# erthward/geonomics

Measured on AMD Instinct MI355X. Metric: individual-timesteps/sec, higher is better.
Workload: dtype u64

## Files before the change

### geonomics_amd/_native.py

```python
import ctypes as C
import os

import numpy as np

_HERE = os.path.dirname(os.path.abspath(__file__))
LIB_PATH = os.environ.get('GNX_LIB') or os.path.join(_HERE, 'libgnxhip.so')

DIST = {'lognormal': 0, 'wald': 1, 'levy': 2}
MATE_UNIFORM, MATE_NEAREST, MATE_INVERSE = 0, 1, 2
SURF_NONE, SURF_MIXTURE, SURF_UNIMODAL = 0, 1, 2
(F_X, F_Y, F_AGE, F_SEX, F_ID, F_E, F_Z, F_FIT, F_GROW, F_GENO) = range(10)
(R_N, R_NPAIRS, R_K, R_D, R_COUNTS) = range(5)
KERNELS = ['move', 'sort', 'permute', 'find_mates', 'pairs', 'offspring',
           'crossover', 'phenotype', 'density', 'death', 'compact', 'crossover_tail']

EXPORTS = [
    'gnx_create', 'gnx_destroy', 'gnx_last_error', 'gnx_words_per_hom', 'gnx_blocks_per_hom',
    'gnx_set_stream', 'gnx_synchronize', 'gnx_upload_rasters',
    'gnx_upload_layer', 'gnx_set_species_params', 'gnx_upload_population',
    'gnx_init_population', 'gnx_set_recomb_paths', 'gnx_set_trait',
    'gnx_set_dominance', 'gnx_set_deleterious', 'gnx_upload_genomes',
    'gnx_assign_genomes', 'gnx_set_z', 'gnx_age', 'gnx_move',
    'gnx_pop_dynamics', 'gnx_pop_dynamics_mate', 'gnx_pop_dynamics_die',
    'gnx_set_z_range', 'gnx_step', 'gnx_counts', 'gnx_step_index',
# ... 253 lines not shown
    def assign_genomes(self, n_per_site):
        n = _arr(n_per_site, np.int32)
        assert n.size == self.L
        self._chk(self.lib.gnx_assign_genomes(self.h, _ptr(n, C.c_int32)))

    def set_z(self):
        self._chk(self.lib.gnx_set_z(self.h))

    def age(self):
        self._chk(self.lib.gnx_age(self.h))

    def move(self):
        self._chk(self.lib.gnx_move(self.h))

    def pop_dynamics(self, burn, with_selection):
        self._chk(self.lib.gnx_pop_dynamics(self.h, int(bool(burn)),
                                            int(bool(with_selection))))

    def pop_dynamics_mate(self, burn):
        self._chk(self.lib.gnx_pop_dynamics_mate(self.h, int(bool(burn))))

    def pop_dynamics_die(self, burn, with_selection):
        self._chk(self.lib.gnx_pop_dynamics_die(self.h, int(bool(burn)),
                                                int(bool(with_selection))))

    def set_z_range(self, first, n):
        self._chk(self.lib.gnx_set_z_range(self.h, C.c_int64(first), C.c_int64(n)))

    def step(self, burn, with_selection):
        self._chk(self.lib.gnx_step(self.h, int(bool(burn)),
                                    int(bool(with_selection))))

    def walk(self, T, burn, with_selection):
        self._chk(self.lib.gnx_walk(self.h, C.c_int64(int(T)), int(bool(burn)),
                                    int(bool(with_selection))))

    def walk_history(self, max_steps=1 << 16):
        n = np.zeros(max_steps, np.int64)
        b = np.zeros(max_steps, np.int64)
        d = np.zeros(max_steps, np.int64)
        k = self.lib.gnx_walk_history(self.h, C.c_int64(max_steps), _ptr(n, C.c_int64),
                                      _ptr(b, C.c_int64), _ptr(d, C.c_int64))
        return n[:k], b[:k], d[:k]

    def comm_init_rccl(self, unique_id, rank, world):
        buf = (C.c_uint8 * 128).from_buffer_copy(bytes(unique_id))
        self._chk(self.lib.gnx_comm_init_rccl(self.h, buf, int(rank), int(world)))

    def comm_init_single(self):
        self._chk(self.lib.gnx_comm_init_single(self.h))

    def comm_local_join(self, group, rank):
        self._chk(self.lib.gnx_comm_local_join(self.h, group, int(rank)))

    def set_id_order(self, mode):
        self._chk(self.lib.gnx_set_id_order(self.h, int(mode)))
        self._id_order = int(mode)

    @property
    def id_order(self):
        return getattr(self, '_id_order', 0)

    def comm_selftest(self):
        self._chk(self.lib.gnx_comm_selftest(self.h))

    def comm_free(self):
        self._chk(self.lib.gnx_comm_free(self.h))

    @property
    def comm_bytes_sent(self):
        return int(self.lib.gnx_comm_bytes_sent(self.h))

    def comm_info(self):
        out = np.zeros(16, np.int64)
        self._chk(self.lib.gnx_comm_info(self.h, _ptr(out, C.c_int64)))
        steps = max(int(out[7]), 1)
        names = ('route_and_count_exchange', 'migrant_ghost_exchange_import',
                 'sort_pairs_second_count_exchange', 'births_gamete_service',
                 'allreduce_deaths')
        return {'transport': ('single', 'rccl', 'local')[int(out[0])], 'rank': int(out[1]),
                'world': int(out[2]), 'nccl_comm_count': int(out[3]),
                'nccl_comm_user_rank': int(out[4]), 'nccl_comm_device': int(out[5]),
                'hip_device': int(out[6]), 'tile_steps': int(out[7]),
                'phase_ms_per_step': {n: float(out[8 + k]) / 1e3 / steps
                                      for k, n in enumerate(names)},
                'bytes_sent': int(out[13]), 'gc_runs': int(out[14])}

    def tile_step_abort(self):
        self._chk(self.lib.gnx_tile_step_abort(self.h))

    def tile_step(self, burn, with_selection, exact=True):
        out = np.zeros(3, np.int64)
        self._chk(self.lib.gnx_tile_step(self.h, int(bool(burn)), int(bool(with_selection)),
                                         int(bool(exact)), _ptr(out, C.c_int64)))
        self._id_order = 1
        return int(out[0]), int(out[1]), int(out[2])

    def tile_walk(self, T, burn, with_selection, exact=True):
        out = np.zeros(5, np.int64)
        self._chk(self.lib.gnx_tile_walk(self.h, C.c_int64(int(T)), int(bool(burn)),
                                         int(bool(with_selection)), int(bool(exact)),
                                         _ptr(out, C.c_int64)))
        self._id_order = 1
        return (int(out[0]), int(out[1]), int(out[2])), int(out[3]), int(out[4])

    def tile_step_begin(self, burn):
        self._chk(self.lib.gnx_tile_step_begin(self.h, int(bool(burn))))
        self._id_order = 1
        a, b = C.c_int64(), C.c_int64()
        self._chk(self.lib.gnx_tile_step_births(self.h, C.byref(a), C.byref(b)))
        return int(a.value), int(b.value)

    def tile_step_end(self, burn, with_selection, exact=True):
        out = np.zeros(3, np.int64)
        self._chk(self.lib.gnx_tile_step_end(self.h, int(bool(burn)), int(bool(with_selection)),
                                             int(bool(exact)), _ptr(out, C.c_int64)))
        return int(out[0]), int(out[1]), int(out[2])

    def tile2_vt_counts(self):
        cnt = np.zeros(64, np.int64)
        self._chk(self.lib.gnx_tile2_vt_counts(self.h, _ptr(cnt, C.c_int64)))
        return cnt

    def tile2_vt_bases(self, bases):
        b = _arr(bases, np.int64)
        assert b.size == 64
        self._chk(self.lib.gnx_tile2_vt_bases(self.h, _ptr(b, C.c_int64)))

    def step_begin(self, burn):
        self._chk(self.lib.gnx_step_begin(self.h, int(bool(burn))))

    def step_mid(self, burn, with_selection):
        self._chk(self.lib.gnx_step_mid(self.h, int(bool(burn)), int(bool(with_selection))))

    def step_end(self, burn):
        self._chk(self.lib.gnx_step_end(self.h, int(bool(burn))))

    def counts(self):
        n, b, d = C.c_int64(), C.c_int64(), C.c_int64()
        self._chk(self.lib.gnx_counts(self.h, C.byref(n), C.byref(b), C.byref(d)))
        return n.value, b.value, d.value

    def totals(self):
        out = np.zeros(6, np.int64)
        self._chk(self.lib.gnx_totals(self.h, _ptr(out, C.c_int64)))
        return dict(zip(('steps', 'ind_steps', 'births', 'deaths', 'xo_births', 'dd_steps'),
                        (int(v) for v in out)))

    def reset_totals(self):
        self._chk(self.lib.gnx_reset_totals(self.h))

    PATH_COUNTS = ('lazy_mortalities', 'xo_launch_p2', 'xo_flush', 'jobs_lanes_256',
                   'jobs_lanes_512', 'sort_hist_gather', 'gc_with_pending_xo', 'make_dense',
                   'moves_ahead')

    def path_counts(self):
        out = np.zeros(len(self.PATH_COUNTS), np.int64)
        n = self.lib.gnx_path_counts(self.h, _ptr(out, C.c_int64), len(out))
        assert n == len(out), 'gnx_path_counts: the library has %d counters' % n
        return dict(zip(self.PATH_COUNTS, (int(v) for v in out)))

    def reset_path_counts(self):
        self._chk(self.lib.gnx_reset_path_counts(self.h))

    @property
    def N(self):
        return self.counts()[0]

    @property
    def step_index(self):
        return self.lib.gnx_step_index(self.h)

    @step_index.setter
    def step_index(self, v):
        self._chk(self.lib.gnx_set_step_index(self.h, C.c_int64(int(v))))

    def synchronize(self):
        self._chk(self.lib.gnx_synchronize(self.h))

    def set_defer_crossover(self, on):
        self._chk(self.lib.gnx_set_defer_crossover(self.h, int(bool(on))))

    def set_crossover_overlap(self, mode):
        self._chk(self.lib.gnx_set_crossover_overlap(self.h, int(mode)))

    def debug_halves(self):
        out = np.zeros(6, np.int64)
        self._chk(self.lib.gnx_debug_halves(self.h, _ptr(out, C.c_int64)))
        return out

    def genome_info(self):
        out = np.zeros(8, np.int64)
        self._chk(self.lib.gnx_genome_info(self.h, _ptr(out, C.c_int64)))
        return dict(zip(('NB', 'BW', 'gc_runs', 'row_spread', 'sparse', 'free_blocks_est',
                         'free_rows', 'deferred'), (int(v) for v in out)))

    def set_crossover_split(self, wide_per_1024):
        self._chk(self.lib.gnx_set_crossover_split(self.h, int(wide_per_1024)))

    def last_crossover_jobs(self):
        n = C.c_int64()
        self._chk(self.lib.gnx_last_crossover_jobs(self.h, None, 0, C.byref(n)))
        out = np.zeros((n.value, 4), np.int32)
        if n.value:
            self._chk(self.lib.gnx_last_crossover_jobs(self.h, _ptr(out, C.c_int32), n.value,
                                                       C.byref(n)))
        return out

    @property
    def last_crossover_births(self):
        return self.lib.gnx_last_crossover_births(self.h)

    def set_stream(self, stream_ptr):
        self._chk(self.lib.gnx_set_stream(self.h, C.c_void_p(stream_ptr)))

    def mutate(self, slots, loci, homs):
        slots = _arr(slots, np.int64)
        loci = _arr(loci, np.int32)
        homs = _arr(homs, np.uint8)
        self._chk(self.lib.gnx_mutate(self.h, int(slots.size),
                                      _ptr(slots, C.c_int64),
                                      _ptr(loci, C.c_int32),
                                      _ptr(homs, C.c_uint8)))

    _FIELD_DT = {F_X: np.float32, F_Y: np.float32, F_AGE: np.int32,
                 F_SEX: np.uint8, F_ID: np.int64, F_FIT: np.float32,
                 F_GROW: np.int32}

    def download(self, field):
        n = int(self.lib.gnx_n_slots(self.h))
        if field == F_E:
            out = np.empty((self.n_layers, n), dtype=np.float32)
        elif field == F_Z:
            out = np.empty((self.n_traits, n), dtype=np.float32)
        elif field == F_GENO:
            out = np.empty((n, 2, self.W64), dtype=np.uint64)
        else:
            out = np.empty(n, dtype=self._FIELD_DT[field])
        if out.size:
            self._chk(self.lib.gnx_download(self.h, field,
                                            out.ctypes.data_as(C.c_void_p),
                                            C.c_int64(out.nbytes)))
        return out

    def download_genomes(self, slots):
        slots = _arr(slots, np.int64)
        out = np.empty((slots.size, 2, self.W64), dtype=np.uint64)
        if slots.size:
            self._chk(self.lib.gnx_download_genomes(
                self.h, C.c_int64(slots.size), _ptr(slots, C.c_int64),
                _ptr(out, C.c_uint64)))
        return out

    def download_raster(self, which):
        out = np.empty((self.H, self.W), dtype=np.float64)
        self._chk(self.lib.gnx_download_raster(self.h, which, _ptr(out, C.c_double)))
        return out

    def spatial_diff_stats(self):
        m, s = C.c_double(), C.c_double()
        self._chk(self.lib.gnx_spatial_diff_stats(self.h, C.byref(m), C.byref(s)))
        return m.value, s.value

    def spatial_diff_sums(self):
        a, b = C.c_double(), C.c_double()
        self._chk(self.lib.gnx_spatial_diff_sums(self.h, C.byref(a), C.byref(b)))
        return a.value, b.value

    def op_move(self, theta, dist):
        t = _arr(theta, np.float32)
        d = _arr(dist, np.float32)
        assert t.size == self.N and d.size == self.N
        self._chk(self.lib.gnx_op_move(self.h, _ptr(t, C.c_float), _ptr(d, C.c_float)))

    def op_move_draws(self):
        n = self.N
        t = np.empty(n, np.float32)
        d = np.empty(n, np.float32)
        self._chk(self.lib.gnx_op_move_draws(self.h, _ptr(t, C.c_float),
                                             _ptr(d, C.c_float)))
        return t, d

    def op_find_pairs(self, keep=None):
        n = self.N
        k = None if keep is None else _arr(keep, np.uint8)
        mate = np.empty(n, np.int32)
        pairs = np.empty((max(n, 1), 2), np.int32)
        npairs = C.c_int64()
        self._chk(self.lib.gnx_op_find_pairs(self.h, _ptr(k, C.c_uint8),
                                             _ptr(mate, C.c_int32),
                                             _ptr(pairs, C.c_int32),
                                             C.byref(npairs)))
        return mate, pairs[:npairs.value].copy()

    def op_crossover(self, parent_slots, keys, start_homs):
        p = _arr(parent_slots, np.int32)
        k = _arr(keys, np.int32)
        s = _arr(start_homs, np.uint8)
        B = p.shape[0]
        assert p.shape == (B, 2) and k.shape == (B, 2) and s.shape == (B, 2)
        self._chk(self.lib.gnx_op_crossover(self.h, C.c_int64(B),
                                            _ptr(p, C.c_int32),
                                            _ptr(k, C.c_int32),
                                            _ptr(s, C.c_uint8)))

    def op_dispersal(self, mid_x, mid_y, theta, dist):
        mx = _arr(mid_x, np.float32)
# ... 963 lines not shown
```

### geonomics_amd/csrc/gnx_api.hip

```cpp
#include <cmath>
#include <cstdarg>
#include <algorithm>
#include <atomic>
#include <chrono>
#include "gnx_internal.h"
#include "gnx_rng.h"
#include "gnx_compact.h"

static thread_local char g_err[1024] = "";

void gnx_set_error(const char* fmt, ...) {
  va_list ap;
  va_start(ap, fmt);
  vsnprintf(g_err, sizeof(g_err), fmt, ap);
  va_end(ap);
}

extern "C" const char* gnx_last_error(void) { return g_err; }

extern "C" int gnx_words_per_hom(int32_t L) {
  int w = (L + 63) / 64;
  return ((w + 15) / 16) * 16;
}

// ... 255 lines not shown
      while (want > 1 && (lines % want || (!asked && lines / want < 2) ||
                          (double)h->cfg.cap_rows * 4 * 2.0 * want >= 2.0e9))
        --want;
      h->NB = want;
      h->BW = h->W64 / want;
      int bl = gnx_env_int("GNX_BLOCK_LINES", -1);
      if (bl < 0) bl = (!asked && lines >= 40) ? std::max(5, (lines + GNX_MAX_NB - 1) / GNX_MAX_NB) : 0;
      if (bl > 0 && (double)h->cfg.cap_rows * 4 * 2.0 * ((lines + bl - 1) / bl) >= 2.0e9) bl = 0;
      if (bl > 0 && (lines + bl - 1) / bl <= GNX_MAX_NB && (lines + bl - 1) / bl >= 1) {
        h->NB = (lines + bl - 1) / bl;
        h->BW = 16 * bl;
      }
      h->NB_alloc = h->NB;
      h->BW_alloc = h->BW;
    }
    {
      const size_t need = (size_t)h->cfg.cap_rows * 2 * std::max(h->W64, h->NB * h->BW) * 8;
      size_t free_b = 0, total_b = 0;
      (void)hipMemGetInfo(&free_b, &total_b);
      int want = gnx_env_int("GNX_ROW_SPREAD", 4);
      want = std::max(1, std::min(want, 8));
      while (want > 1 && ((double)need * want > 0.75 * (double)free_b ||
                          (double)h->cfg.cap_rows * want > 1.0e9))
        --want;
      for (; want >= 1; --want) {
        h->G = nullptr;
        const hipError_t e = hipMalloc((void**)&h->G, need * (size_t)want);
        if (e == hipSuccess) break;
        (void)hipGetLastError();
        if (want == 1) {
          gnx_set_error("hipMalloc of the genome table (%zu bytes) failed: %s", need,
                        hipGetErrorString(e));
          return 1;
        }
      }
      h->row_spread = want;
    }
    GNXCHK(dalloc(&h->free_rows, (size_t)h->cfg.cap_rows));
    const size_t halves = (size_t)h->cfg.cap_rows * h->row_spread * 2 * h->NB;
    GNXCHK(dalloc(&h->hmap, halves));
    GNXCHK(dalloc(&h->half_mark, halves));
    GNXCHK(dalloc(&h->half_free, (size_t)h->cfg.cap_rows * 2 * h->NB));
    GNXCHK(dalloc(&h->half_top, 1));
    HIPCHK(hipMalloc(&h->xo_plan, (size_t)cap * 40));
    GNXCHK(dalloc(&h->gc_cnt, (size_t)h->cfg.cap_rows * 2 * h->NB / GNX_CB + 2));
    GNXCHK(dalloc(&h->gc_off, (size_t)h->cfg.cap_rows * 2 * h->NB / GNX_CB + 2));
    HIPCHK(hipMemset(h->half_mark, 0, halves));
    HIPCHK(hipMalloc((void**)&h->xo_jobs_acc, 2 * sizeof(unsigned long long)));
    HIPCHK(hipMemset(h->xo_jobs_acc, 0, 2 * sizeof(unsigned long long)));
    HIPCHK(hipMemset(h->hmap, 0xff, halves * sizeof(int32_t)));
    HIPCHK(hipMemset(h->half_top, 0, sizeof(int32_t)));
    h->alias_xo = gnx_env_int("GNX_XO_ALIAS", 1) != 0;
  }
  for (int k = 0; k < 2; ++k) {
    GNXCHK(dalloc(&h->key[k], cap));
    GNXCHK(dalloc(&h->perm[k], cap));
  }
  GNXCHK(dalloc(&h->mate, cap));
  for (int k = 0; k < 2; ++k) {
    GNXCHK(dalloc(&h->ord[k], cap));
    GNXCHK(dalloc(&h->keyk[k], cap));
    GNXCHK(dalloc(&h->valk[k], cap));
  }
  GNXCHK(dalloc(&h->newslot, cap));
  GNXCHK(dalloc(&h->fill_cnt, 4));
  HIPCHK(hipEventCreateWithFlags(&h->ev_fill, gnx_order_event_flags()));
  HIPCHK(hipEventCreateWithFlags(&h->ev_alive, gnx_order_event_flags()));
  HIPCHK(hipEventCreateWithFlags(&h->ev_moved, gnx_order_event_flags()));
  HIPCHK(hipEventCreateWithFlags(&h->ev_perm_rest, gnx_order_event_flags()));
  {
    const size_t nb = std::max(gnx_os_scratch_bytes((size_t)cap, 24),
                               gnx_os_words_used64((size_t)cap, 64) * sizeof(unsigned int)) + 16;
    HIPCHK(hipMalloc(&h->os_scratch, nb));
    HIPCHK(hipMemset(h->os_scratch, 0, nb));
  }
  GNXCHK(dalloc(&h->os_ktmp, cap));
  GNXCHK(dalloc(&h->os_vtmp, cap));
  GNXCHK(dalloc(&h->cell32, cap));
  GNXCHK(dalloc(&h->ord_cnt, cap / GNX_CB + 2));
  GNXCHK(dalloc(&h->ord_off, cap / GNX_CB + 2));
  HIPCHK(hipEventCreateWithFlags(&h->ev_ord, gnx_order_event_flags()));
  HIPCHK(hipStreamCreate(&h->stream3));
  HIPCHK(hipEventCreateWithFlags(&h->ev_compact, gnx_order_event_flags()));
  h->ord_mode = gnx_env_int("GNX_ORD_SORT", 1) != 0;
  GNXCHK(dalloc(&h->tag, cap));
  HIPCHK(hipMalloc(&h->cand, (size_t)cap * 16));
  GNXCHK(dalloc(&h->flag, cap + 1));
  GNXCHK(dalloc(&h->flag2, cap + 1));
  GNXCHK(dalloc(&h->scan, cap + 1));
  GNXCHK(dalloc(&h->pairs, cap * 2));
  GNXCHK(dalloc(&h->nbirths, cap + 1));
  GNXCHK(dalloc(&h->boff, cap + 1));
  GNXCHK(dalloc(&h->off_pair, cap));
  GNXCHK(dalloc(&h->off_parent, cap * 2));
  GNXCHK(dalloc(&h->off_keys, cap * 2));
  GNXCHK(dalloc(&h->off_start, cap * 2));
  GNXCHK(dalloc(&h->keep_in, cap));
  GNXCHK(dalloc(&h->inj_a, cap * GNX_DISP_ATTEMPTS));
  GNXCHK(dalloc(&h->inj_b, cap * GNX_DISP_ATTEMPTS));
  GNXCHK(dalloc(&h->mid_x, cap));
  GNXCHK(dalloc(&h->mid_y, cap));
  GNXCHK(dalloc(&h->p_death, cap));
  GNXCHK(dalloc(&h->d_cell, cap));
  GNXCHK(dalloc(&h->dead_in, cap));
  GNXCHK(dalloc(&h->nmax_bits, 1));
  GNXCHK(dalloc(&h->red, 8));
  GNXCHK(gnx_prim_sort_bytes((size_t)cap, 32, &h->sort_tmp_bytes));
  HIPCHK(hipMalloc(&h->sort_tmp, std::max<size_t>(h->sort_tmp_bytes, 16)));
  GNXCHK(gnx_prim_scan_bytes((size_t)cap + 1, &h->scan_tmp_bytes));
  HIPCHK(hipMalloc(&h->scan_tmp, std::max<size_t>(h->scan_tmp_bytes, 16)));
  GNXCHK(gnx_prim_sort64_bytes((size_t)cap, &h->sort64_tmp_bytes));
  HIPCHK(hipMalloc(&h->sort64_tmp, std::max<size_t>(h->sort64_tmp_bytes, 16)));
  GNXCHK(dalloc(&h->key64[0], cap));
  GNXCHK(dalloc(&h->key64[1], cap));
  GNXCHK(dalloc(&h->pairs2, cap * 2));
  GNXCHK(dalloc(&h->pair_goff, cap));
  GNXCHK(dalloc(&h->req_pid, cap));
  GNXCHK(dalloc(&h->req_k, cap));
  GNXCHK(dalloc(&h->req_key, cap));
  GNXCHK(dalloc(&h->req_start, cap));
  GNXCHK(dalloc(&h->req_px, cap));
  GNXCHK(dalloc(&h->req_py, cap));
  GNXCHK(dalloc(&h->req_count, 1));
  h->blk_stride = (int)((cap + 1023) / 1024) + 2;
  GNXCHK(dalloc(&h->blk_cnt, (size_t)3 * h->blk_stride));
  GNXCHK(dalloc(&h->blk_off, (size_t)3 * h->blk_stride));
  GNXCHK(dalloc(&h->cnt_dev, 8));
  GNXCHK(dalloc(&h->tickets, 8));
  GNXCHK(dalloc(&h->nmax2, 2));
  HIPCHK(hipMemset(h->nmax2, 0, 2 * sizeof(unsigned long long)));
  HIPCHK(hipEventCreateWithFlags(&h->ev_pairs, gnx_order_event_flags()));
  HIPCHK(hipEventCreateWithFlags(&h->ev_latP, gnx_order_event_flags()));
  HIPCHK(hipEventCreateWithFlags(&h->ev_perm, gnx_order_event_flags()));
  HIPCHK(hipEventCreateWithFlags(&h->ev_binsN, gnx_order_event_flags()));
  HIPCHK(hipMemset(h->tickets, 0, 8 * sizeof(unsigned int)));
  HIPCHK(hipHostMalloc((void**)&h->h_pin, 32 * sizeof(int64_t),
                       hipHostMallocCoherent | hipHostMallocMapped));
  memset(h->h_pin, 0, 32 * sizeof(int64_t));
  HIPCHK(hipHostGetDevicePointer((void**)&h->h_pin_dev, h->h_pin, 0));
  if (cfg->L > 0) {
    for (int k = 0; k < 2; ++k) {
      HIPCHK(hipMalloc(&h->jobs[k], (size_t)cap * 2 * h->NB * 16));
      HIPCHK(hipMalloc(&h->jobs_bp[k], (size_t)cap * 2 * h->NB * 8));
      GNXCHK(dalloc(&h->n_jobs_dev[k], 1));
      HIPCHK(hipEventCreateWithFlags(&h->ev_xo_done[k], gnx_order_event_flags()));
      HIPCHK(hipEventCreateWithFlags(&h->ev_xo_wide[k], gnx_order_event_flags()));
    }
    HIPCHK(hipEventCreateWithFlags(&h->ev_jobs, gnx_order_event_flags()));
  }
  HIPCHK(hipEventCreateWithFlags(&h->ev_counts, hipEventDisableTiming));
  h->xo_launch_late = h->xo_launch_late_default = cap > gnx_dd_max_cap();
  h->compact_fill = gnx_env_int("GNX_COMPACT_FILL", 1) != 0;
  h->permute_split = gnx_env_int("GNX_PERMUTE_SPLIT", 1) != 0;
  *out = h;
  return 0;
}

extern "C" void gnx_destroy(gnx_state* h) {
  if (!h) return;
  host_marks_report();
  if (gnx_host_times() && g_host_steps > 0)
    fprintf(stderr, "[gnx host times] %lld steps: %.1f us/step in gnx_step, %.1f us of it waiting for counts\n",
            g_host_steps, 1e6 * g_host_step_s / g_host_steps, 1e6 * g_host_wait_s / g_host_steps);
  (void)gnx_xo_launch_pending(h);
  (void)hipStreamSynchronize(h->stream);
  gnx_dd_destroy(h);
  (void)gnx_comm_free(h);
  {
    void* vt[] = {h->vt_cls, h->vt_scls, h->vt_blk_nz, h->vt_rank, h->vt_pblk, h->vt_blk_cnt, h->vt_blk_off, h->vt_count, h->vt_base};
    for (void* q : vt)
      if (q) (void)hipFree(q);
  }
  if (h->stream2) (void)hipStreamSynchronize(h->stream2);
  if (h->stream3) (void)hipStreamSynchronize(h->stream3);
  for (int k = 0; k < 2; ++k) {
    (void)hipFree(h->jobs[k]);
    (void)hipFree(h->jobs_bp[k]);
    (void)hipFree(h->n_jobs_dev[k]);
    if (h->ev_xo_done[k]) (void)hipEventDestroy(h->ev_xo_done[k]);
    if (h->ev_xo_wide[k]) (void)hipEventDestroy(h->ev_xo_wide[k]);
  }
  if (h->ev_jobs) (void)hipEventDestroy(h->ev_jobs);
  if (h->ev_counts) (void)hipEventDestroy(h->ev_counts);
  for (int k = 0; k < 2; ++k) {
    free_soa(&h->soa[k]);
    (void)hipFree(h->key[k]);
    (void)hipFree(h->perm[k]);
    (void)hipFree(h->counts_rast[k]);
  }
  void* ptrs[] = {h->os_scratch, h->os_ktmp, h->os_vtmp, h->fill_cnt, h->ord[0], h->ord[1], h->keyk[0], h->keyk[1], h->valk[0], h->valk[1], h->newslot, h->cell32, h->ord_cnt, h->ord_off, h->route_geo_dev, h->xo_plan, h->gc_cnt, h->gc_off, h->half_mark, h->hmap, h->half_free, h->half_top, h->xo_jobs_acc, h->rast, h->G, h->free_rows, h->paths, h->bp_off, h->bp_loci, h->dom,
                  h->delet_loci, h->delet_s, h->cell_start, h->tag, h->cand, h->sort64_tmp, h->key64[0], h->key64[1], h->pairs2,
                  h->pair_goff, h->st_rec, h->st_z, h->st_geno, h->st_slots, h->req_pid, h->req_k, h->req_key, h->req_start, h->req_px, h->req_py,
                  h->req_count, h->sort_tmp, h->scan_tmp, h->mate,
                  h->flag, h->flag2, h->scan, h->pairs, h->nbirths, h->boff, h->off_pair,
                  h->off_parent, h->off_keys, h->off_start, h->keep_in, h->inj_a, h->inj_b,
                  h->mid_x, h->mid_y, h->p_death, h->d_cell, h->dead_in, h->nmax_bits, h->red,
                  h->sel_loci, h->path_sel, h->lat.areas, h->lat.cprime, h->spl_N.c, h->spl_P.c, h->bin_partials, h->nodes,
                  h->K_over, h->blk_cnt, h->blk_off, h->cnt_dev, h->tickets, h->nmax2, h->fb[0], h->gp_rec, h->gp_z, h->gp_slots, h->tile_counts, h->rq_sorted, h->rq_k, h->gam_out, h->gam_slot, h->chk,
                  h->lin_tab, h->lin_bt};
  for (void* p : ptrs) (void)hipFree(p);
  for (int t = 0; t < GNX_MAX_TRAITS; ++t) {
    (void)hipFree(h->traits[t].loci);
    (void)hipFree(h->traits[t].alpha);
    (void)hipFree(h->traits[t].phi_rast);
  }
  (void)hipHostFree(h->h_pin);
  if (h->h_route_pin) (void)hipHostFree(h->h_route_pin);
  (void)hipFree(h->gh_rec);
  (void)hipFree(h->route_cnt);
  if (h->h_stage) (void)hipHostFree(h->h_stage);
  for (int k = 0; k < GNX_K_COUNT; ++k) timers_resolve(h, k);
  for (hipEvent_t e : h->ev_free) (void)hipEventDestroy(e);
  if (h->own_stream) (void)hipStreamDestroy(h->stream);
  if (h->stream2) (void)hipStreamDestroy(h->stream2);
  h->stream2 = nullptr;
  if (h->stream3) {
    (void)hipStreamSynchronize(h->stream3);
    (void)hipStreamDestroy(h->stream3);
  }
  if (h->ev_ord) (void)hipEventDestroy(h->ev_ord);
  if (h->ev_compact) (void)hipEventDestroy(h->ev_compact);
  if (h->ev_fill) (void)hipEventDestroy(h->ev_fill);
  if (h->ev_alive) (void)hipEventDestroy(h->ev_alive);
  if (h->ev_moved) (void)hipEventDestroy(h->ev_moved);
  if (h->ev_perm_rest) (void)hipEventDestroy(h->ev_perm_rest);
  if (h->ev_pairs) (void)hipEventDestroy(h->ev_pairs);
  if (h->ev_latP) (void)hipEventDestroy(h->ev_latP);
  if (h->ev_perm) (void)hipEventDestroy(h->ev_perm);
  if (h->ev_binsN) (void)hipEventDestroy(h->ev_binsN);
  delete h;
}

extern "C" int gnx_set_stream(gnx_state* h, void* hip_stream) {
  GNXCHK(gnx_xo_join(h));
  HIPCHK(hipStreamSynchronize(h->stream));
  if (h->stream2) HIPCHK(hipStreamSynchronize(h->stream2));
  if (h->own_stream) (void)hipStreamDestroy(h->stream);
  if (h->stream2) (void)hipStreamDestroy(h->stream2);
  h->stream2 = nullptr;
  h->stream = (hipStream_t)hip_stream;
  h->own_stream = false;
  return 0;
}

extern "C" int gnx_synchronize(gnx_state* h) {
  GNXCHK(gnx_xo_launch_pending(h));
  if (h->stream3) HIPCHK(hipStreamSynchronize(h->stream3));
  HIPCHK(hipStreamSynchronize(h->stream));
  if (h->stream2) HIPCHK(hipStreamSynchronize(h->stream2));
  return 0;
}

extern "C" int gnx_upload_rasters(gnx_state* h, const float* rasts) {
  size_t n = (size_t)h->cfg.n_layers * h->cfg.W * h->cfg.H;
  HIPCHK(hipMemcpyAsync(h->rast, rasts, n * sizeof(float), hipMemcpyHostToDevice, h->stream));
  HIPCHK(hipStreamSynchronize(h->stream));
  return 0;
}

extern "C" int gnx_upload_layer(gnx_state* h, int32_t layer, const float* rast) {
  if (layer < 0 || layer >= h->cfg.n_layers) {
    gnx_set_error("gnx_upload_layer: bad layer %d", layer);
    return 1;
  }
  size_t n = (size_t)h->cfg.W * h->cfg.H;
  HIPCHK(hipMemcpyAsync(h->rast + layer * n, rast, n * sizeof(float), hipMemcpyHostToDevice,
                        h->stream));
  HIPCHK(hipStreamSynchronize(h->stream));
  return 0;
}

extern "C" int gnx_set_k_raster(gnx_state* h, const double* K) {
  h->cfg_epoch += 1;
  size_t n = (size_t)h->cfg.W * h->cfg.H;
  HIPCHK(hipStreamSynchronize(h->stream));
  if (!K) {
    (void)hipFree(h->K_over);
    h->K_over = nullptr;
    return 0;
  }
  if (!h->K_over) HIPCHK(hipMalloc((void**)&h->K_over, n * sizeof(double)));
  GNXCHK(gnx_h2d(h, h->K_over, K, n * sizeof(double)));
  return 0;
}

static int lattice_nodes(int dim, double ww) {
  double hww = ww / 2.0;
  double last_edge = 0, last_inner = 0;
  int ne = (int)ceil((dim + ww) / ww);
  last_edge = (ne - 1) * ww;
  int ni = (int)ceil(((dim + hww) - hww) / ww);
  last_inner = hww + (ni - 1) * ww;
  double last = std::max(last_edge, last_inner);
  return (int)llround(last / hww) + 1;
}

static int setup_lattice(gnx_state* h) {
  const gnx_config& c = h->cfg;
  double ww = h->sp.window_width;
  if (!(ww > 0)) ww = std::nearbyint(0.1 * std::max(c.W, c.H));
  if (!(ww > 0)) ww = 1;
  GnxLattice& L = h->lat;
  (void)hipFree(L.areas);
  (void)hipFree(L.cprime);
  (void)hipFree(h->spl_N.c);
  (void)hipFree(h->spl_P.c);
  (void)hipFree(h->bin_partials);
  (void)hipFree(h->nodes);
  L.hww = ww / 2.0;
  L.Jx = lattice_nodes(c.W, ww);
  L.Jy = lattice_nodes(c.H, ww);
  L.nbx = L.Jx;
  L.nby = L.Jy;
  const int64_t nn = (int64_t)L.Jx * L.Jy;
  std::vector<double> areas(nn);
  for (int i = 0; i < L.Jy; ++i)
    for (int j = 0; j < L.Jx; ++j) {
      double cx = j * L.hww, cy = i * L.hww;
      double ax = std::min(cx + L.hww, (double)c.W) - std::max(cx - L.hww, 0.0);
      double ay = std::min(cy + L.hww, (double)c.H) - std::max(cy - L.hww, 0.0);
      double a = std::max(ax, 0.0) * std::max(ay, 0.0);
      if (a == 0) a = 0.0001;
      areas[(int64_t)i * L.Jx + j] = a;
    }
  int Jm = std::max(L.Jx, L.Jy);
  std::vector<double> cp(Jm + 1, 0.0);
  if (Jm > 1) cp[1] = 0.25;
  for (int k = 2; k < Jm; ++k) cp[k] = 1.0 / (4.0 - cp[k - 1]);
  GNXCHK(dalloc(&L.areas, nn));
  GNXCHK(dalloc(&L.cprime, Jm + 1));
  GNXCHK(dalloc(&h->spl_N.c, 4 * nn));
  GNXCHK(dalloc(&h->spl_P.c, 4 * nn));
  GNXCHK(dalloc(&h->nodes, nn));
  size_t nb = (size_t)L.nbx * L.nby;
  GNXCHK(dalloc(&h->bin_partials, 2 * nb + 4));
  h->bins_P = h->bin_partials + nb;
  (void)hipFree(h->fb[0]);
  GNXCHK(dalloc(&h->fb[0], 3 * nb));
  h->fb[1] = h->fb[0] + nb;
  h->fb[2] = h->fb[0] + 2 * nb;
  HIPCHK(hipMemset(h->fb[0], 0, 3 * nb * sizeof(int32_t)));
  h->fb_zero[0] = h->fb_zero[1] = h->fb_zero[2] = true;
  h->fb_adults = false;
  h->nmax_ready = false;
  HIPCHK(hipMemcpy(L.areas, areas.data(), nn * sizeof(double), hipMemcpyHostToDevice));
  HIPCHK(hipMemcpy(L.cprime, cp.data(), (Jm + 1) * sizeof(double), hipMemcpyHostToDevice));
  h->spl_N.valid = h->spl_P.valid = false;
// ... 1003 lines not shown
```

### geonomics_amd/csrc/gnx_internal.h

```cpp
#pragma once
#include <cstring>
#include <cstdint>
#include <cstdio>
#include <cstdlib>
#include <string>
#include <vector>
#include <utility>
#include <hip/hip_runtime.h>
#include "../../include/gnx_hip.h"
#include "gnx_half.h"

#define GNX_MAX_TRAITS 16
#define GNX_MAX_LAYERS 16
#define GNX_DISP_ATTEMPTS 8
#define GNX_SPARSE_MAX_BP 24

void gnx_set_error(const char* fmt, ...);

static inline int gnx_env_int(const char* name, int dflt) {
  const char* v = getenv(name);
  return v ? atoi(v) : dflt;
}
static inline int64_t gnx_dd_max_cap() {
  static const int64_t v = getenv("GNX_DD_MAX_CAP") ? atoll(getenv("GNX_DD_MAX_CAP")) : 600000;
// ... 61 lines not shown
  float e[4], z[4];
  uint64_t tb[4];
};
#ifdef __HIPCC__
__device__ __forceinline__ GnxRec gnx_rec_load(const GnxSoA& a, int64_t i, int64_t cap, int nl,
                                               int nt, int tbw) {
  GnxRec r;
  r.x = a.x[i];
  r.y = a.y[i];
  r.age = a.age[i];
  r.sex = a.sex[i];
  r.id = a.id[i];
  r.fit = a.fit[i];
  r.grow = a.grow[i];
  r.ghost = a.ghost[i];
#pragma unroll
  for (int l = 0; l < 4; ++l) r.e[l] = l < nl ? a.e[(int64_t)l * cap + i] : 0.0f;
#pragma unroll
  for (int t = 0; t < 4; ++t) r.z[t] = t < nt ? a.z[(int64_t)t * cap + i] : 0.0f;
#pragma unroll
  for (int w = 0; w < 4; ++w) r.tb[w] = w < tbw ? a.tb[i * tbw + w] : 0ull;
  return r;
}
__device__ __forceinline__ void gnx_rec_store(const GnxSoA& b, int64_t k, int64_t cap, int nl, int nt,
                                              int tbw, const GnxRec& r) {
  b.x[k] = r.x;
  b.y[k] = r.y;
  b.age[k] = r.age;
  b.sex[k] = r.sex;
  b.id[k] = r.id;
  b.fit[k] = r.fit;
  b.grow[k] = r.grow;
  b.ghost[k] = r.ghost;
#pragma unroll
  for (int l = 0; l < 4; ++l)
    if (l < nl) b.e[(int64_t)l * cap + k] = r.e[l];
#pragma unroll
  for (int t = 0; t < 4; ++t)
    if (t < nt) b.z[(int64_t)t * cap + k] = r.z[t];
#pragma unroll
  for (int w = 0; w < 4; ++w)
    if (w < tbw) b.tb[k * tbw + w] = r.tb[w];
}
__device__ __forceinline__ void gnx_rec_rest(const GnxSoA& a, int64_t i, const GnxSoA& b, int64_t k,
                                             int64_t cap, int nl, int nt, int tbw) {
  for (int l = 4; l < nl; ++l) b.e[(int64_t)l * cap + k] = a.e[(int64_t)l * cap + i];
  for (int t = 4; t < nt; ++t) b.z[(int64_t)t * cap + k] = a.z[(int64_t)t * cap + i];
  for (int w = 4; w < tbw; ++w) b.tb[k * tbw + w] = a.tb[i * tbw + w];
}
#endif

struct GnxLattice {
  int Jx = 0, Jy = 0;
  int nbx = 0, nby = 0;
  double hww = 0;
  double* areas = nullptr;
  double* cprime = nullptr;
};

struct GnxSpline {
  double* c = nullptr;
  bool valid = false;
};

struct GnxKernelTimer {
  double ms = 0;
  int64_t launches = 0;
  double bytes = 0;
};

struct GnxDD {
  int32_t N;
  int32_t P;
  int32_t B;
  int32_t n_free;
  int32_t ord_n;
  int32_t err;
  int32_t seq;
  int32_t pad;
  int64_t max_id;
  int64_t step;
};
#define GNX_DD_ERR_SLOTS 1
#define GNX_DD_ERR_ROWS 2
#define GNX_DD_ERR_BLOCKS 4
struct GnxDDRec {
  int64_t seq;
  int32_t N0, P, B, S;
  int32_t xo, n_free, half_top, err;
  int64_t max_id, step;
  int64_t pad[2];
};
#define GNX_DD_RING 4096
#ifdef __HIPCC__
__device__ __forceinline__ int64_t gnx_dd_n(const GnxDD* dd, int64_t n) { return dd ? (int64_t)dd->N : n; }
__device__ __forceinline__ int64_t gnx_dd_nb(const GnxDD* dd, int64_t n) {
  return dd ? (int64_t)dd->N + dd->B : n;
}
__device__ __forceinline__ long long gnx_dd_step(const GnxDD* dd, long long s) {
  return dd ? (long long)dd->step : s;
}
__device__ __forceinline__ int gnx_tile_index(float v, int tw, int n) {
  int c = (int)(v / (float)tw);
  c = max(0, min(n - 1, c));
  while (c + 1 < n && (float)((c + 1) * tw) <= v) ++c;
  while (c > 0 && (float)(c * tw) > v) --c;
  return c;
}
#endif

#define GNX_MAX_TILES 4096
#define GNX_TILE_DIM 64
struct RouteGeo {
  int R, C, tw, th, me, ncx, ncy;
  double inv_cs;
  int cx0[GNX_TILE_DIM], cx1[GNX_TILE_DIM], cy0[GNX_TILE_DIM], cy1[GNX_TILE_DIM];
};
#ifdef __HIPCC__
__device__ __forceinline__ int gnx_route_append(int32_t* __restrict__ counts, int dest) {
  unsigned long long todo = __ballot(dest >= 0);
  const int lane = threadIdx.x & 63;
  int idx = -1;
  while (todo) {
    const int leader = __ffsll((long long)todo) - 1;
    const int d = __shfl(dest, leader);
    const unsigned long long same = __ballot(dest == d);
    int base = 0;
    if (lane == leader) base = atomicAdd(&counts[d], (int)__popcll(same));
    base = __shfl(base, leader);
    if (dest == d) idx = base + (int)__popcll(same & ((1ull << lane) - 1ull));
    todo &= ~same;
  }
  return idx;
}
__device__ __forceinline__ int gnx_route_dest(const RouteGeo& g, int k, int orow, int oc, int cx, int cy) {
  if (k == 4) return (orow * g.C + oc) != g.me ? orow * g.C + oc : -1;
  const int rr = orow + k / 3 - 1, cc = oc + k % 3 - 1;
  if (rr >= 0 && rr < g.R && cc >= 0 && cc < g.C && cx >= g.cx0[cc] && cx <= g.cx1[cc] &&
      cy >= g.cy0[rr] && cy <= g.cy1[rr])
    return rr * g.C + cc;
  return -1;
}
#endif
enum {
  GNX_PC_LAZY_MORT = 0,
  GNX_PC_XO_P2,
  GNX_PC_XO_FLUSH,
  GNX_PC_JOBS_256,
  GNX_PC_JOBS_512,
  GNX_PC_SORT_GATHER,
  GNX_PC_GC_PENDING_XO,
  GNX_PC_MAKE_DENSE,
  GNX_PC_MOVE_AHEAD,
  GNX_PC_COUNT
};

struct gnx_state {
  gnx_config cfg{};
  gnx_species_params sp{};
  bool have_sp = false;
  hipStream_t stream = nullptr;
  hipStream_t stream2 = nullptr;
  bool xo_pending = false;
  bool own_stream = false;
  int W64 = 0;
  int64_t N = 0;
  int64_t max_id = -1;
  int64_t step = 0;
  int64_t last_births = 0, last_deaths = 0;
  int64_t tot[6]{};
  int64_t pc[GNX_PC_COUNT]{};
  int64_t n_ghost = 0;

  GnxSoA soa[2]{};
  int cur = 0;

  uint64_t* G = nullptr;
  int row_spread = 1;
  int32_t* free_rows = nullptr;
  int64_t n_free = 0;
  int32_t* hmap = nullptr;
  uint8_t* half_mark = nullptr;
  int32_t* half_free = nullptr;
  int32_t* half_top = nullptr;
  int64_t half_free_est = 0;
  int64_t gc_runs = 0;
  void* xo_plan = nullptr;
  int32_t* gc_cnt = nullptr;
  int32_t* gc_off = nullptr;
  int NB = 1;
  int NB_alloc = 1;
  int BW = 0, BW_alloc = 0;
  hipStream_t stream3 = nullptr;
  hipEvent_t ev_compact = nullptr;
  bool alias_xo = true;
  unsigned long long* xo_jobs_acc = nullptr;
  bool genomes_assigned = false;

  float* rast = nullptr;

  int n_paths = 0;
  uint64_t* paths = nullptr;
  int32_t* bp_off = nullptr;
  int32_t* bp_loci = nullptr;
  bool sparse_paths = false;

  int32_t* lin_tab = nullptr;
  int32_t* lin_bt = nullptr;
  int64_t lin_rows = 0;
  uint64_t lin_sum = 0;
  int64_t lin_budget = 0;
  double lin_ms = 0.0;
  int64_t lin_launches = 0, lin_uploaded = 0;

  int64_t ld_budget = 0;
  double ld_ms = 0.0;
  int64_t ld_launches = 0, ld_blocks = 0;

  double tr_ms = 0.0;
  int64_t tr_launches = 0, tr_bytes = 0;

  double sw_ms = 0.0;
  int64_t sw_launches = 0, sw_steps = 0;

  int64_t cost_budget = 0;
  double cost_ms = 0.0;
  int64_t cost_launches = 0, cost_rounds = 0, cost_batches = 0;

  double admix_ms = 0.0;
  int64_t admix_launches = 0, admix_chunks = 0;
  int32_t admix_instance = 0;

  int64_t dm_tiles = 0, dm_chunks = 0, dm_launches = 0;

  GnxTrait traits[GNX_MAX_TRAITS];
  std::vector<int32_t> h_trait_loci[GNX_MAX_TRAITS];
  std::vector<int32_t> h_delet_loci;
  int n_tl = 0;
  int n_sel = 0, TW = 0;
  int32_t* sel_loci = nullptr;
  uint64_t* path_sel = nullptr;
  uint8_t* dom = nullptr;
  int n_delet = 0;
  int32_t* delet_loci = nullptr;
  double* delet_s = nullptr;

  bool defer_xo = true;
  bool xo_deferred = false;
  int64_t xo_first = 0, xo_B = 0;
  void* jobs[2]{};
  int32_t* n_jobs_dev[2]{};
  void* jobs_bp[2]{};
  bool jobs_inline[2]{};
  int jobs_cur = 0;
  hipEvent_t ev_jobs = nullptr, ev_xo_done[2]{};
  hipEvent_t ev_counts = nullptr;
  bool xo_inflight[2]{};
  hipEvent_t ev_xo_wide[2]{};
  bool xo_wide_inflight[2]{};
  int xo_split = 0;
  int xo_last_split = 0;
  bool xo_running = false;
  bool xo_launch_late = false;
  bool xo_launch_late_default = false;
  bool xo_sort_waits = true;
  int xo_wait_at = 1;
  int xo_ready_buf = -1;
  int64_t xo_ready_jobs = 0;
  int64_t last_xo_births = 0;

  double cs = 1, inv_cs = 1;
  int ncx = 1, ncy = 1, key_bits = 1;
  int cell_ref = 1;
  uint32_t* key[2]{};
  int32_t* perm[2]{};
  int32_t* cell_start = nullptr;
  void* cand = nullptr;
  uint32_t* tag = nullptr;
  void* sort_tmp = nullptr;
  size_t sort_tmp_bytes = 0;
  void* scan_tmp = nullptr;
  size_t scan_tmp_bytes = 0;
  void* sort64_tmp = nullptr;
  size_t sort64_tmp_bytes = 0;
  uint64_t* key64[2]{};
  int32_t* pairs2 = nullptr;
  int64_t* pair_goff = nullptr;
  bool pair_goff_local = false;
  int id_order = 0;
  bool pair_goff_ready = false;
  bool pair_goff_local_base = false;
  bool vt_fused = false;
  int64_t vt_mul = 1;
  bool vt_weighted = false;
  uint8_t* vt_cls = nullptr;
  uint8_t* vt_scls = nullptr;
  unsigned long long* vt_blk_nz = nullptr;
  int32_t *vt_rank = nullptr, *vt_pblk = nullptr, *vt_blk_cnt = nullptr, *vt_blk_off = nullptr,
          *vt_count = nullptr;
  int64_t* vt_base = nullptr;
  int64_t n_births_pending = 0;
  bool step_burn = false;
  int64_t* req_pid = nullptr;
  int32_t* req_k = nullptr;
  int32_t* req_key = nullptr;
  uint8_t* req_start = nullptr;
  float* req_px = nullptr;
  float* req_py = nullptr;
  int32_t* req_count = nullptr;
  bool tiled = false;
  int tile_R = 1, tile_C = 1, tile_r = 0, tile_c = 0;
  gnx_ind_rec* st_rec = nullptr;
  float* st_z = nullptr;
  uint64_t* st_geno = nullptr;
  int64_t* st_slots = nullptr;
  int64_t st_n = 0, st_cap = 0, st_geno_cap = 0;
  bool st_has_geno = false;
  int64_t birth_first_slot = 0;
  int64_t n_req = 0;
  gnx_ind_rec* gp_rec = nullptr;
  float* gp_z = nullptr;
  int64_t* gp_slots = nullptr;
  int64_t gp_n = 0, gp_cap = 0;
  int32_t* tile_counts = nullptr;
  void* rq_sorted = nullptr;
  int32_t* rq_k = nullptr;
  int64_t rq_cap = 0;
  uint64_t* gam_out = nullptr;
  int32_t* gam_slot = nullptr;
  int64_t gam_cap = 0;
  int64_t* chk = nullptr;
  int64_t tile_evict = 0;
  float evict_box[4]{};
  int64_t n_req_known = -1;
  gnx_ind_rec* gh_rec = nullptr;
  int64_t gh_cap = 0;
  int32_t* route_cnt = nullptr;
  int64_t route_n_mig = 0, route_n_gh = 0;
  int64_t prev_deaths = 0;
  int32_t* h_route_pin = nullptr;
  int32_t* h_route_pin_dev = nullptr;
  std::vector<int64_t> req_by_rank;
  bool rq_is2 = false;
  bool tile_req_on_device = false;
  bool tile2_mode = false;
  bool req_cnt_zeroed = false;
  bool tile_pairs_nowait = false;
  bool tile_births_settled = false;

  int32_t* mate = nullptr;
  int32_t* flag = nullptr;
  int32_t* flag2 = nullptr;
  int32_t* scan = nullptr;
  int32_t* pairs = nullptr;
  int32_t* nbirths = nullptr;
  int32_t* boff = nullptr;
  int32_t* off_pair = nullptr;
  int32_t* off_parent = nullptr;
  int32_t* off_keys = nullptr;
  uint8_t* off_start = nullptr;
  uint8_t* keep_in = nullptr;
  float* inj_a = nullptr;
  float* inj_b = nullptr;
  float* mid_x = nullptr;
  float* mid_y = nullptr;
  int64_t n_pairs = 0;
  bool pairs_wait = false;
  int64_t pairs_seq = 0;
  bool pairs_with_top = false, pairs_with_density = false;
  bool mort_wait = false;
  bool mort_xo = false, mort_fill = false, mort_ord_keep = false;
  int mort_has_rows = 0;
  int64_t mort_N = 0;

  GnxLattice lat;
  GnxSpline spl_N, spl_P;
  int32_t* bin_partials = nullptr;
  int32_t* bins_P = nullptr;
  bool bins_zeroed[2]{};
  bool nmax_zeroed = false;
  bool req_zeroed = false;
  int32_t* fb[3]{};
  bool fb_zero[3]{};
  int fb_cur = 0;
  bool fb_adults = false;
  int64_t fb_count = 0;
  unsigned long long* nmax2 = nullptr;
  const unsigned long long* nmax_cur = nullptr;
  bool nmax_ready = false;
  bool last_N_fused = false;
  hipEvent_t ev_pairs = nullptr, ev_latP = nullptr, ev_perm = nullptr, ev_binsN = nullptr;
  bool binsN_inflight = false;
  bool latP_inflight = false;
  bool ord_mode = true;
  bool ord_valid = false;
  int64_t ord_n = 0;
  int ord_cur = 0;
  int32_t* ord[2]{};
  int32_t* newslot = nullptr;
  bool compact_fill = true;
  bool jobs_self_scan = false;
  bool ord_covers_xo = false;
  bool permute_split = true;
  bool perm_rest_inflight = false;
  bool perm_rest_pending = false;
  GnxSoA perm_rest_a{}, perm_rest_b{};
  int64_t perm_rest_N = 0;
  hipEvent_t ev_perm_rest = nullptr;
  bool fb_pending = false;
  const float *fbp_x = nullptr, *fbp_y = nullptr;
  int64_t fbp_N = 0;
  hipEvent_t ev_alive = nullptr;
  int32_t* fill_cnt = nullptr;
  hipEvent_t ev_fill = nullptr;
  int64_t fill_guess = 0;
  uint32_t* cell32 = nullptr;
  uint32_t* keyk[2]{};
  int32_t* valk[2]{};
  void* os_scratch = nullptr;
  uint32_t* os_ktmp = nullptr;
  int32_t* os_vtmp = nullptr;
  int32_t* ord_cnt = nullptr;
  int32_t* ord_off = nullptr;
  hipEvent_t ev_ord = nullptr;
  bool ord_inflight = false;
  bool keys_ordmode = false;
  bool keys_fresh = false;
  bool hist_fresh = false;
  bool holes = false;
  int64_t holes_N = 0;
  RouteGeo* route_geo_dev = nullptr;
  uint64_t route_geo_epoch = 0;
  bool move_counts_routes = false;
  bool move_counted_routes = false;
  bool tile_lazy_ok = false;
  int64_t holes_flagged = 0;
  bool eager_move = false;
  bool move_ahead_ok = false;
  bool moved_ahead = false;
  hipEvent_t ev_moved = nullptr;
  bool move_writes_keys = false;
  int n_bin_blocks = 0;
  double* nodes = nullptr;
  double* K_over = nullptr;
  unsigned long long* nmax_bits = nullptr;
  double* p_death = nullptr;
  double* d_cell = nullptr;
  uint8_t* dead_in = nullptr;
  int32_t* counts_rast[2]{};
  int counts_cur = 0;
  bool counts_init = false;
  double* red = nullptr;

  int32_t* blk_cnt = nullptr;
  int32_t* blk_off = nullptr;
  int blk_stride = 0;
  int32_t* cnt_dev = nullptr;
  unsigned int* tickets = nullptr;

  int64_t* h_pin = nullptr;
  int64_t* h_pin_dev = nullptr;
  int64_t pin_seq = 0;
  void* h_stage = nullptr;
  size_t h_stage_bytes = 0;

  void* tile_comm = nullptr;
  GnxDD* dd = nullptr;
  GnxDDRec* dd_ring = nullptr;
  GnxDDRec* dd_ring_dev = nullptr;
  bool dd_active = false;
  int64_t dd_seq = 0;
  int64_t dd_seen = 0;
  int64_t dd_half_est = 0;
  int64_t dd_b_hi = 0;
  int64_t dd_use_hi = 0;
  int64_t dd_gc_seq = 0;
  int64_t dd_top_last = 0, dd_top_seq = 0;
  int64_t dd_est_seq = 0;
  int64_t dd_post_gc = 0;
  bool dd_gc_wait = false;
  void* dd_graph[1]{};
  int32_t dd_err = 0;
  std::vector<int64_t> dd_hist;
  bool dd_hist_closed = false;
  uint64_t cfg_epoch = 1;

  bool profiling = false;
  int profile_only = -1;
  GnxKernelTimer timers[GNX_K_COUNT];
  hipEvent_t ev_open = nullptr;
  std::vector<hipEvent_t> ev_free;
  std::vector<std::pair<hipEvent_t, hipEvent_t>> ev_pending[GNX_K_COUNT];
};

GnxTraitTab gnx_trait_tab(const gnx_state* h);

static inline GnxHalves gnx_halves(const gnx_state* h) {
  return GnxHalves{h->hmap, h->half_free, h->half_top, h->NB, h->BW > 0 ? h->BW : h->W64 / h->NB};
}
int gnx_half_reserve(gnx_state* h, int64_t blocks);
int gnx_gc(gnx_state* h);
static inline const int32_t* gnx_alias_bp(const gnx_state* h) {
  return (h->alias_xo && h->sparse_paths) ? h->bp_off : nullptr;
}
static inline const int32_t* gnx_alias_loci(const gnx_state* h) {
  return (h->alias_xo && h->sparse_paths) ? h->bp_loci : nullptr;
}

int gnx_publish(gnx_state* h, int slot, const int32_t* a, const int32_t* b = nullptr,
                const int32_t* c = nullptr, const int32_t* d = nullptr);

void gnx_time_begin(gnx_state* h, int kernel = -1);
void gnx_time_end(gnx_state* h, int kernel, double bytes);

int gnx_h2d(gnx_state* h, void* dst, const void* src, size_t bytes);
int gnx_d2h(gnx_state* h, void* dst, const void* src, size_t bytes);

int gnx_l_init_population(gnx_state* h, int64_t N);
int gnx_l_gather_e(gnx_state* h, int64_t first, int64_t n);
int gnx_l_age(gnx_state* h);
int gnx_l_move(gnx_state* h, bool inc_age, const float* inj_theta, const float* inj_dist,
               float* out_theta, float* out_dist, bool apply);
int gnx_l_move_ahead(gnx_state* h, int64_t N);
int gnx_move_ahead_join(gnx_state* h);
int gnx_l_sort_by_cell(gnx_state* h, bool split_rest = false);
int gnx_wait_permute_rest(gnx_state* h);
int gnx_permute_rest_launch(gnx_state* h);
int gnx_l_find_pairs(gnx_state* h, const uint8_t* d_keep, int64_t* n_pairs_out,
                     bool with_density = false);
int gnx_l_find_pairs_enqueue(gnx_state* h, const uint8_t* d_keep, bool with_density);
int gnx_l_find_pairs_finish(gnx_state* h, int64_t* n_pairs_out);
int gnx_l_births(gnx_state* h, int64_t* births_out);
int gnx_l_pair_cls(gnx_state* h, int64_t P, bool local);
int gnx_vt_buffers(gnx_state* h);
int gnx_l_mate(gnx_state* h, bool burn, bool inject, int64_t B_inject, int64_t* births_out,
               int64_t id_base = -1, bool tiled = false);
int gnx_l_dispersal_inject(gnx_state* h, int64_t B, int A, const float* d_mx, const float* d_my,
                           const float* d_theta, const float* d_dist, float* d_ox, float* d_oy,
                           int32_t* d_used);
int gnx_l_crossover_all(gnx_state* h, int64_t first_slot, int64_t B);
int gnx_l_crossover_requests(gnx_state* h, int64_t first_slot, int64_t n_req);
int gnx_l_crossover_pending(gnx_state* h, int64_t first_slot, int64_t B);
int gnx_l_crossover_survivors(gnx_state* h, int64_t first_slot, int64_t B, const int32_t* d_alive,
                              const int32_t* d_scan);
int gnx_xo_join(gnx_state* h);
int gnx_xo_flush_deferred(gnx_state* h);
int gnx_xo_launch_pending(gnx_state* h, int site = GNX_PC_XO_FLUSH);
int gnx_xo_wait_inflight(gnx_state* h);
int gnx_xo_prepare_jobs(gnx_state* h, int32_t** zero);
int gnx_xo_wait_wide(gnx_state* h);
double gnx_xo_bytes_per_birth(const gnx_state* h);
int gnx_l_rebuild_sel(gnx_state* h);
int gnx_l_path_sel(gnx_state* h);
int gnx_l_tb_from_rows(gnx_state* h, int64_t first, int64_t n, const int32_t* d_list,
                       const int64_t* d_slots, bool join = true);
// ... 165 lines not shown
```

### geonomics_amd/csrc/gnx_kernels_pop.hip

```cpp
#include "gnx_internal.h"
#include "gnx_rng.h"
#include "gnx_compact.h"
#include "gnx_tb.h"
#include "gnx_bins.h"

static int gnx_id_bits(const gnx_state* h) {
  int b = 1;
  while (b < 40 && (h->max_id >> b) != 0) ++b;
  return b;
}
static bool gnx_ord_sort(const gnx_state* h) {
  return h->ord_mode && h->ord_valid && !h->tiled;
}

__device__ __forceinline__ int wave_min_i(int v) {
#pragma unroll
  for (int m = 32; m >= 1; m >>= 1) v = min(v, __shfl_xor(v, m));
  return v;
}
__device__ __forceinline__ int wave_max_i(int v) {
#pragma unroll
  for (int m = 32; m >= 1; m >>= 1) v = max(v, __shfl_xor(v, m));
  return v;
}
// ... 432 lines not shown
  P.step = h->step;
  P.seed = c.seed;
  const bool with_keys = h->move_writes_keys && apply && !inj_theta;
  const bool ordm = with_keys && gnx_ord_sort(h);
  P.key = (with_keys && !ordm) ? h->key64[0] : nullptr;
  P.cell32 = ordm ? h->cell32 : nullptr;
  P.idx = h->perm[0];
  P.inv_cs = h->inv_cs;
  P.ncx = h->ncx;
  P.ncy = h->ncy;
  P.idbits = gnx_id_bits(h);
  GNXCHK(gnx_os_hist_discard(h));
  P.hist = nullptr;
  P.hist_rb = P.hist_places = 0;
  if (ordm && !ddm && gnx_move_hist(h, &P.hist_places, &P.hist_rb)) {
    P.hist = (uint32_t*)h->os_scratch;
    h->hist_fresh = true;
  }
  P.rg = nullptr;
  P.rcnt = nullptr;
  if (h->move_counts_routes && apply && !ddm && !inj_theta && h->route_geo_dev && h->route_cnt) {
    P.rg = h->route_geo_dev;
    P.rcnt = h->route_cnt;
    h->move_counted_routes = true;
  }
  h->keys_fresh = with_keys;
  if (with_keys) h->keys_ordmode = ordm;
  constexpr int GNX_MOVE_TILE_FLOATS = 2 * 2048;
  P.tile_floats = sp.move_surf != GNX_SURF_NONE ? GNX_MOVE_TILE_FLOATS : 0;
  gnx_time_begin(h);
  const int64_t n_grid = ddm ? (int64_t)c.cap_inds : (holes ? h->holes_N : h->N);
  hipLaunchKernelGGL(k_move<2>, dim3(gnx_grid(n_grid, 512)), dim3(256),
                     (size_t)P.tile_floats * sizeof(float), h->stream, P,
                     h->soa[h->cur], h->rast, inj_theta, inj_dist, out_theta, out_dist);
  gnx_time_end(h, GNX_K_MOVE,
               (double)h->N * (32.0 + 8.0 * c.n_layers + (sp.move_surf ? 36.0 : 0.0)));
  HIPCHK(hipGetLastError());
  return 0;
}

int gnx_l_move_ahead(gnx_state* h, int64_t N) {
  HIPCHK(hipStreamWaitEvent(h->stream2, h->ev_alive, 0));
  h->holes = true;
  h->holes_N = N;
  h->holes_flagged = N;
  hipStream_t main = h->stream;
  h->stream = h->stream2;
  h->step += 1;
  h->move_writes_keys = true;
  const int rc = gnx_l_move(h, true, nullptr, nullptr, nullptr, nullptr, true);
  h->move_writes_keys = false;
  h->step -= 1;
  h->stream = main;
  GNXCHK(rc);
  HIPCHK(hipEventRecord(h->ev_moved, h->stream2));
  h->moved_ahead = true;
  ++h->pc[GNX_PC_MOVE_AHEAD];
  return 0;
}

int gnx_move_ahead_join(gnx_state* h) {
  if (!h->moved_ahead) return 0;
  h->moved_ahead = false;
  HIPCHK(hipStreamWaitEvent(h->stream, h->ev_moved, 0));
  return 0;
}

__device__ __forceinline__ int gnx_cell_of(float x, float y, double inv_cs, int ncx, int ncy) {
  int cx = min(ncx - 1, (int)((double)x * inv_cs));
  int cy = min(ncy - 1, (int)((double)y * inv_cs));
  return cy * ncx + cx;
}

__global__ void k_keys(int64_t N, const float* x, const float* y, const int64_t* id,
                       double inv_cs, int ncx, int ncy, int idbits, uint64_t* key, int32_t* idx) {
  int64_t i = (int64_t)blockIdx.x * blockDim.x + threadIdx.x;
  if (i >= N) return;
  key[i] = ((uint64_t)gnx_cell_of(x[i], y[i], inv_cs, ncx, ncy) << idbits) | (uint64_t)id[i];
  idx[i] = (int32_t)i;
}

__global__ void k_keys_evict(int64_t N, const float* x, const float* y, const int64_t* id,
                             const uint8_t* ghost, float x0, float x1, float y0, float y1,
                             double inv_cs, int ncx, int ncy, int idbits, uint64_t* key,
                             int32_t* idx, const int32_t* __restrict__ alive, int64_t n_flagged) {
  int64_t i = (int64_t)blockIdx.x * blockDim.x + threadIdx.x;
  if (i >= N) return;
  const float xi = x[i], yi = y[i];
  const bool dead = alive != nullptr && i < n_flagged && (alive[i] & 1) == 0;
  const bool out = !ghost[i] && (xi < x0 || xi >= x1 || yi < y0 || yi >= y1);
  const uint64_t cell = dead ? (uint64_t)(ncx * ncy) + 1ull
                             : (out ? (uint64_t)(ncx * ncy) : (uint64_t)gnx_cell_of(xi, yi, inv_cs, ncx, ncy));
  key[i] = (cell << idbits) | (uint64_t)id[i];
  idx[i] = (int32_t)i;
}

__global__ void k_free_tail(int64_t N, int64_t n, const int32_t* grow, int32_t* free_rows,
                            int64_t n_free) {
  int64_t k = (int64_t)blockIdx.x * blockDim.x + threadIdx.x;
  if (k < n) free_rows[n_free + k] = grow[N + k];
}

__global__ void k_permute(int64_t N, int64_t cap, const int32_t* perm, GnxSoA a, GnxSoA b,
                          int n_layers, int n_traits, int tbw, unsigned long long pair_seed,
                          uint32_t* tag, uint4* cand, uint64_t* key, int idbits,
                          int32_t* cell_start, int ncells, const uint32_t* __restrict__ cellk,
                          const int32_t* __restrict__ ord, int64_t ord_n,
                          int32_t* __restrict__ ord_new, int32_t* __restrict__ perm_out,
                          uint4* __restrict__ wipe, int64_t wipe_n, int hot_only,
                          const GnxDD* __restrict__ dd, GnxBinP bins, int32_t* __restrict__ vt_zero) {
  int64_t i = (int64_t)blockIdx.x * blockDim.x + threadIdx.x;
  if (vt_zero && i < 64) vt_zero[i] = 0;
  if (dd) {
    N = dd->N;
    ord_n = dd->ord_n;
    pair_seed = gnx_pair_seed(pair_seed, dd->step);
  }
  for (int64_t w = i; w < wipe_n; w += (int64_t)gridDim.x * blockDim.x)
    wipe[w] = make_uint4(0u, 0u, 0u, 0u);
  if (i >= N) return;
  {
    const int k = cellk ? (int)cellk[i] : (int)(key[i] >> idbits);
    const int prev = (i == 0) ? -1 : (cellk ? (int)cellk[i - 1] : (int)(key[i - 1] >> idbits));
    for (int c = prev + 1; c <= k; ++c) cell_start[c] = (int32_t)i;
    if (i == N - 1)
      for (int c = k + 1; c <= ncells; ++c) cell_start[c] = (int32_t)N;
  }
  int64_t j = perm[i];
  if (cellk) {
    const int64_t kk = j;
    j = kk < ord_n ? ord[kk] : kk;
    ord_new[kk] = (int32_t)i;
    perm_out[i] = (int32_t)j;
  }
  const uint32_t ck = cellk ? cellk[i] : 0u;
  GnxRec r;
  if (hot_only) {
    r.x = a.x[j];
    r.y = a.y[j];
    r.age = a.age[j];
    r.sex = a.sex[j];
    r.id = a.id[j];
    r.ghost = a.ghost[j];
    b.x[i] = r.x;
    b.y[i] = r.y;
    b.age[i] = r.age;
    b.sex[i] = r.sex;
    b.id[i] = r.id;
    b.ghost[i] = r.ghost;
  } else {
    r = gnx_rec_load(a, j, cap, n_layers, n_traits, tbw);
    gnx_rec_store(b, i, cap, n_layers, n_traits, tbw, r);
  }
  if (cellk) key[i] = ((uint64_t)ck << idbits) | (uint64_t)r.id;
  const uint32_t tg = gnx_ind_tag(pair_seed, (unsigned long long)r.id);
  cand[i] = make_uint4(__float_as_uint(r.x), __float_as_uint(r.y), tg, (uint32_t)r.id);
  if (!hot_only) gnx_rec_rest(a, j, b, i, cap, n_layers, n_traits, tbw);
  if (bins.bins) gnx_bin_add(bins.bins, gnx_bin_of(bins, r.x, r.y), true);
}

__global__ void k_permute_rest(int64_t N, int64_t cap, const int32_t* __restrict__ perm, GnxSoA a,
                               GnxSoA b, int n_layers, int n_traits, int tbw) {
  const int64_t i = (int64_t)blockIdx.x * blockDim.x + threadIdx.x;
  if (i >= N) return;
  const int64_t j = perm[i];
  const float fit = a.fit[j];
  const int32_t grow = a.grow[j];
  float e[4], z[4];
  uint64_t tb[4];
#pragma unroll
  for (int l = 0; l < 4; ++l) e[l] = l < n_layers ? a.e[(int64_t)l * cap + j] : 0.0f;
#pragma unroll
  for (int t = 0; t < 4; ++t) z[t] = t < n_traits ? a.z[(int64_t)t * cap + j] : 0.0f;
#pragma unroll
  for (int w = 0; w < 4; ++w) tb[w] = w < tbw ? a.tb[j * tbw + w] : 0ull;
  b.fit[i] = fit;
  b.grow[i] = grow;
#pragma unroll
  for (int l = 0; l < 4; ++l)
    if (l < n_layers) b.e[(int64_t)l * cap + i] = e[l];
#pragma unroll
  for (int t = 0; t < 4; ++t)
    if (t < n_traits) b.z[(int64_t)t * cap + i] = z[t];
#pragma unroll
  for (int w = 0; w < 4; ++w)
    if (w < tbw) b.tb[i * tbw + w] = tb[w];
  gnx_rec_rest(a, j, b, i, cap, n_layers, n_traits, tbw);
}

__global__ void k_cells(int64_t N, const float* x, const float* y, double inv_cs, int ncx, int ncy,
                        uint32_t* cell32) {
  int64_t i = (int64_t)blockIdx.x * blockDim.x + threadIdx.x;
  if (i < N) cell32[i] = (uint32_t)gnx_cell_of(x[i], y[i], inv_cs, ncx, ncy);
}

__global__ void k_keys_ord(int64_t N, int64_t ord_n, const int32_t* __restrict__ ord,
                           const uint32_t* __restrict__ cell32, uint32_t* __restrict__ key,
                           int32_t* __restrict__ val) {
  int64_t k = (int64_t)blockIdx.x * blockDim.x + threadIdx.x;
  if (k >= N) return;
  const int64_t slot = k < ord_n ? ord[k] : k;
  key[k] = cell32[slot];
  val[k] = (int32_t)k;
}

__global__ void k_iota(int64_t N, int32_t* v) {
  int64_t i = (int64_t)blockIdx.x * blockDim.x + threadIdx.x;
  if (i < N) v[i] = (int32_t)i;
}

int gnx_permute_rest_launch(gnx_state* h) {
  if (!h->perm_rest_pending) return 0;
  h->perm_rest_pending = false;
  const gnx_config& c = h->cfg;
  HIPCHK(hipEventRecord(h->ev_perm, h->stream));
  HIPCHK(hipStreamWaitEvent(h->stream3, h->ev_perm, 0));
  hipLaunchKernelGGL(k_permute_rest, dim3(gnx_grid(h->perm_rest_N, 256)), dim3(256), 0, h->stream3,
                     h->perm_rest_N, c.cap_inds, h->perm[1], h->perm_rest_a, h->perm_rest_b,
                     c.n_layers, c.n_traits, h->perm_rest_a.tb ? 2 * h->TW : 0);
  HIPCHK(hipEventRecord(h->ev_perm_rest, h->stream3));
  HIPCHK(hipGetLastError());
  h->perm_rest_inflight = true;
  return 0;
}

int gnx_wait_permute_rest(gnx_state* h) {
  GNXCHK(gnx_permute_rest_launch(h));
  if (h->perm_rest_inflight) {
    HIPCHK(hipStreamWaitEvent(h->stream, h->ev_perm_rest, 0));
    h->perm_rest_inflight = false;
  }
  return 0;
}

__global__ void k_gather_ord(int64_t N, int64_t cap, const int32_t* __restrict__ ord, GnxSoA a,
                             GnxSoA b, int n_layers, int n_traits, int tbw,
                             int32_t* __restrict__ ord_new) {
  const int64_t i = (int64_t)blockIdx.x * blockDim.x + threadIdx.x;
  if (i >= N) return;
  const int64_t j = ord[i];
  const GnxRec r = gnx_rec_load(a, j, cap, n_layers, n_traits, tbw);
  gnx_rec_store(b, i, cap, n_layers, n_traits, tbw, r);
  gnx_rec_rest(a, j, b, i, cap, n_layers, n_traits, tbw);
  ord_new[i] = (int32_t)i;
}

int gnx_l_make_dense(gnx_state* h) {
  if (!h->holes) return 0;
  if (h->tile2_mode || h->mort_wait || h->pairs_wait || !h->ord_valid || h->ord_n != h->N) {
    gnx_set_error("internal: an uncompacted population that cannot be gathered (tile %d, step "
                  "open %d, index %d with %lld of %lld)", (int)h->tile2_mode,
                  (int)(h->mort_wait || h->pairs_wait), (int)h->ord_valid, (long long)h->ord_n,
                  (long long)h->N);
    return 1;
  }
  const int64_t N = h->N;
  gnx_bins_adults_drop(h);
  GNXCHK(gnx_wait_permute_rest(h));
  GNXCHK(gnx_xo_flush_deferred(h));
  GNXCHK(gnx_move_ahead_join(h));
  GNXCHK(gnx_os_hist_discard(h));
  h->keys_fresh = false;
  if (h->ord_inflight) {
    HIPCHK(hipStreamWaitEvent(h->stream, h->ev_ord, 0));
    h->ord_inflight = false;
  }
  const gnx_config& c = h->cfg;
  GnxSoA a = h->soa[h->cur], b = h->soa[h->cur ^ 1];
  hipLaunchKernelGGL(k_gather_ord, dim3(gnx_grid(N, 256)), dim3(256), 0, h->stream, N, c.cap_inds,
                     (const int32_t*)h->ord[h->ord_cur], a, b, c.n_layers, c.n_traits,
                     a.tb ? 2 * h->TW : 0, h->ord[h->ord_cur ^ 1]);
  HIPCHK(hipGetLastError());
  h->cur ^= 1;
  h->ord_cur ^= 1;
  h->holes = false;
  h->holes_N = 0;
  h->holes_flagged = 0;
  ++h->pc[GNX_PC_MAKE_DENSE];
  return 0;
}

int gnx_l_sort_by_cell(gnx_state* h, bool split_rest) {
  int64_t N = h->N;
  gnx_bins_adults_drop(h);
  GNXCHK(gnx_wait_permute_rest(h));
  if (N == 0) {
    h->holes = false;
    return gnx_move_ahead_join(h);
  }
  GNXCHK(gnx_xo_flush_deferred(h));
  const bool xo_covered = h->xo_sort_waits && h->ord_covers_xo && h->ord_inflight && h->tile_evict == 0 &&
                          (h->keys_fresh ? h->keys_ordmode : gnx_ord_sort(h));
  if (xo_covered) {
    for (int k = 0; k < 2; ++k) h->xo_inflight[k] = h->xo_wide_inflight[k] = false;
    h->ord_covers_xo = false;
  } else if (h->xo_sort_waits) {
    GNXCHK(gnx_xo_wait_wide(h));
  }
  const gnx_config& c = h->cfg;
  GnxSoA a = h->soa[h->cur], b = h->soa[h->cur ^ 1];
  const int idbits = gnx_id_bits(h);
  const bool alone = h->xo_sort_waits || !h->xo_running;
  const bool tile_holes = h->holes && h->tile2_mode;
  const int64_t n_sort = tile_holes ? h->holes_N : N;
  const bool ordm = (h->tile_evict > 0 || tile_holes) ? false
                                                      : (h->keys_fresh ? h->keys_ordmode : gnx_ord_sort(h));
  if (h->holes && !tile_holes && !(ordm && h->keys_fresh)) {
    gnx_set_error("internal: the cell sort of an uncompacted population needs the id-ordered index "
                  "and the movement's keys");
    return 1;
  }
  h->holes = false;
  gnx_time_begin(h);
  int64_t wipe_words = 0;
  if (ordm) {
    if (!h->keys_fresh)
      hipLaunchKernelGGL(k_cells, dim3(gnx_grid(N, 256)), dim3(256), 0, h->stream, N, a.x, a.y,
                         h->inv_cs, h->ncx, h->ncy, h->cell32);
    if (h->ord_inflight) {
      HIPCHK(hipStreamWaitEvent(h->stream, h->ev_ord, 0));
      h->ord_inflight = false;
    }
    if (h->keys_fresh && h->hist_fresh) {
      h->hist_fresh = false;
      ++h->pc[GNX_PC_SORT_GATHER];
      GNXCHK(gnx_os_sort32_gather(h->os_scratch, h->os_ktmp, h->os_vtmp, h->keyk[1], h->valk[1],
                                  (size_t)N, h->key_bits, h->ord[h->ord_cur], h->ord_n, h->cell32,
                                  h->stream));
      wipe_words = (int64_t)gnx_os_words_used((size_t)N, h->key_bits);
    } else if (h->key_bits <= 24) {
      GNXCHK(gnx_os_hist_discard(h));
      GNXCHK(gnx_os_keys_hist(h->os_scratch, h->tickets + 3, N, h->ord_n, h->ord[h->ord_cur],
                              h->cell32, h->keyk[0], h->valk[0], h->key_bits, h->stream));
      GNXCHK(gnx_os_sort32_ranked(h->os_scratch, h->os_ktmp, h->os_vtmp, h->keyk[0], h->keyk[1],
                                  h->valk[0], h->valk[1], (size_t)N, h->key_bits, h->stream));
      wipe_words = (int64_t)gnx_os_words_used((size_t)N, h->key_bits);
    } else {
      GNXCHK(gnx_os_hist_discard(h));
      hipLaunchKernelGGL(k_keys_ord, dim3(gnx_grid(N, 256)), dim3(256), 0, h->stream, N, h->ord_n,
                         h->ord[h->ord_cur], h->cell32, h->keyk[0], h->valk[0]);
      GNXCHK(gnx_prim_sort32_bits(h->sort64_tmp, h->sort64_tmp_bytes, h->keyk[0], h->keyk[1],
                                  h->valk[0], h->valk[1], (size_t)N, h->key_bits, h->stream, alone));
    }
  } else {
    GNXCHK(gnx_os_hist_discard(h));
    int cell_bits = h->key_bits;
    if (h->tile_evict > 0 || tile_holes) {
      while ((1ll << cell_bits) <= (int64_t)h->ncx * h->ncy + (tile_holes ? 1 : 0)) ++cell_bits;
      if (h->tile_evict == 0) {
        h->evict_box[0] = h->evict_box[2] = -1.0f;
        h->evict_box[1] = (float)c.W + 1.0f;
        h->evict_box[3] = (float)c.H + 1.0f;
      }
      hipLaunchKernelGGL(k_keys_evict, dim3(gnx_grid(n_sort, 256)), dim3(256), 0, h->stream, n_sort,
                         a.x, a.y, a.id, a.ghost, h->evict_box[0], h->evict_box[1], h->evict_box[2],
                         h->evict_box[3], h->inv_cs, h->ncx, h->ncy, idbits, h->key64[0],
                         h->perm[0], tile_holes ? (const int32_t*)h->flag : (const int32_t*)nullptr,
                         h->holes_flagged);
    } else if (!h->keys_fresh) {
      hipLaunchKernelGGL(k_keys, dim3(gnx_grid(N, 256)), dim3(256), 0, h->stream, N, a.x, a.y, a.id,
                         h->inv_cs, h->ncx, h->ncy, idbits, h->key64[0], h->perm[0]);
    }
    if (h->sort64_tmp_bytes >= (size_t)n_sort * 12 && h->os_scratch) {
      GNXCHK(gnx_os_sort64_clean(h->os_scratch, h->sort64_tmp, h->key64[0], h->key64[1], h->perm[0],
                                 h->perm[1], (size_t)n_sort, idbits + cell_bits, h->stream));
      wipe_words = (int64_t)gnx_os_words_used64((size_t)n_sort, idbits + cell_bits);
    } else {
      GNXCHK(gnx_prim_sort64_bits(h->sort64_tmp, h->sort64_tmp_bytes, h->key64[0], h->key64[1],
                                  h->perm[0], h->perm[1], (size_t)n_sort, idbits + cell_bits,
                                  h->stream, alone));
    }
  }
  h->keys_fresh = false;
  gnx_time_end(h, GNX_K_SORT, (double)N * 40.0);
  gnx_time_begin(h);
  static const bool tile_split = gnx_env_int("GNX_TILE_SPLIT", 0) != 0;
  const bool split = split_rest && h->permute_split && (ordm ? !h->tiled : (tile_split && h->tile2_mode)) &&
                     h->stream3 != nullptr;
  hipLaunchKernelGGL(k_permute, dim3(gnx_grid(N, 256)), dim3(256), 0, h->stream, N, c.cap_inds,
                     ordm ? h->valk[1] : h->perm[1], a, b, c.n_layers, c.n_traits,
                     a.tb ? 2 * h->TW : 0, gnx_pair_seed(c.seed, h->step), h->tag, (uint4*)h->cand,
                     h->key64[1], idbits, h->cell_start, h->ncx * h->ncy,
                     ordm ? h->keyk[1] : nullptr, h->ord[h->ord_cur], h->ord_n,
                     h->ord[h->ord_cur ^ 1], h->perm[1], (uint4*)h->os_scratch, (wipe_words + 3) / 4,
                     split ? 1 : 0, (const GnxDD*)nullptr, GnxBinP{nullptr, 0.0, 0, 0},
                     h->id_order == 1 ? h->vt_count : (int32_t*)nullptr);
  if (split) {
    h->perm_rest_a = a;
    h->perm_rest_b = b;
    h->perm_rest_N = N;
    h->perm_rest_pending = true;
    GNXCHK(gnx_permute_rest_launch(h));
  }
  gnx_time_end(h, GNX_K_PERMUTE,
               (double)N * 2.0 * (33.0 + 4.0 * c.n_layers + 4.0 * c.n_traits + 16.0 * h->TW));
  GNXCHK(gnx_l_bins_adults_async(h, b.x, b.y, N));
  if (ordm) {
    h->ord_cur ^= 1;
    h->ord_n = N;
  } else if (h->ord_mode && !h->tiled) {
    if (h->ord_inflight) {
      HIPCHK(hipStreamWaitEvent(h->stream, h->ev_ord, 0));
      h->ord_inflight = false;
    }
    hipLaunchKernelGGL(k_iota, dim3(gnx_grid(N, 256)), dim3(256), 0, h->stream, N, h->perm[0]);
    GNXCHK(gnx_prim_sort64_bits(h->sort64_tmp, h->sort64_tmp_bytes, (const uint64_t*)b.id,
                                h->key64[0], h->perm[0], h->ord[h->ord_cur], (size_t)N, idbits,
                                h->stream, alone));
    h->ord_valid = true;
    h->ord_n = N;
  } else {
    h->ord_valid = false;
  }
  HIPCHK(hipGetLastError());
  h->cur ^= 1;
  if (h->tile_evict > 0) {
    const int64_t n = h->tile_evict;
    h->tile_evict = 0;
    h->N -= n;
    if (h->genomes_assigned && c.L > 0) {
      hipStream_t fs = h->stream;
      if (split) {
        GNXCHK(gnx_permute_rest_launch(h));
        fs = h->stream3;
      }
      hipLaunchKernelGGL(k_free_tail, dim3(gnx_grid(n, 256)), dim3(256), 0, fs, h->N, n,
                         h->soa[h->cur].grow, h->free_rows, h->n_free);
      if (split) HIPCHK(hipEventRecord(h->ev_perm_rest, h->stream3));
      h->n_free += n;
    }
    h->ord_valid = false;
    h->fb_adults = false;
  }
  return 0;
}

#define FM_PER_BLOCK 1024
#define FM_LANES 4
#define FM_MIN_BLOCKS 8
#define FM_MAX_BLOCKS 2048

struct FocalP {
  int64_t N;
  const uint8_t* keep_in;
  float b;
  int sexed, ra_f;
  long long step;
  unsigned long long seed;
  const GnxDD* dd;
};

#define FM_ROWS 5
struct FmRanges {
  int st[FM_ROWS], len[FM_ROWS];
  unsigned int M;
  __device__ __forceinline__ int slot(int j) const {
    int s = st[0] + j;
    int acc = len[0];
#pragma unroll
    for (int q = 1; q < FM_ROWS; ++q) {
      s = j >= acc ? st[q] + (j - acc) : s;
      acc += len[q];
    }
    return s;
  }
};

__device__ __forceinline__ FmRanges fm_ranges(float fx, float fy, double inv_cs, int ncx, int ncy,
                                              const int32_t* __restrict__ cell_start, int ref) {
  FmRanges R;
  const int k = gnx_cell_of(fx, fy, inv_cs, ncx, ncy);
  const int cy = k / ncx;
  const int cx = k - cy * ncx;
  const int lo = max(cx - ref, 0), hi = min(cx + ref, ncx - 1);
  unsigned int M = 0;
#pragma unroll
  for (int q = 0; q < FM_ROWS; ++q) {
    const int ry = cy - ref + q;
    const bool in = q <= 2 * ref && ry >= 0 && ry < ncy;
    R.st[q] = in ? cell_start[ry * ncx + lo] : 0;
    R.len[q] = in ? cell_start[ry * ncx + hi + 1] - R.st[q] : 0;
    M += (unsigned int)R.len[q];
  }
  R.M = M;
  return R;
}

template <bool WT>
__device__ __forceinline__ int fm_blocks(unsigned int M) {
  return WT ? min(max((int)(M >> 2), 2 * FM_MIN_BLOCKS), 2 * FM_MAX_BLOCKS)
            : min(max((int)(M >> 3), FM_MIN_BLOCKS), FM_MAX_BLOCKS);
}

template <int MODE>
__global__ void __launch_bounds__(256)
k_find_mates(FocalP fp, GnxSoA s, const uint4* __restrict__ cand, double inv_cs,
             const int32_t* __restrict__ cell_start, int ncx, int ncy, int ref, float r, float r2,
             int easy_rounds, int32_t* __restrict__ mate) {
  __shared__ int32_t list[FM_PER_BLOCK];
  __shared__ int32_t hard[FM_PER_BLOCK];
  __shared__ int32_t wcnt[FM_PER_BLOCK / 256][4];
  __shared__ int32_t n_hard_s;
  const int tid = threadIdx.x, lane = tid & 63, wave = tid >> 6;
  const int64_t base = (int64_t)blockIdx.x * FM_PER_BLOCK;
  fp.N = gnx_dd_n(fp.dd, fp.N);
  fp.step = gnx_dd_step(fp.dd, fp.step);
  if (base >= fp.N) return;
  constexpr int ROUNDS = FM_PER_BLOCK / 256;
  bool okr[ROUNDS];
  unsigned long long balr[ROUNDS];
#pragma unroll
  for (int round = 0; round < ROUNDS; ++round) {
    const int64_t i = base + round * 256 + tid;
    bool ok = false;
    if (i < fp.N) {
      if (fp.keep_in) {
        ok = fp.keep_in[i] != 0;
      } else {
        uint4 rr = gnx_rand4(fp.seed, (unsigned long long)s.id[i], fp.step, OP_PAIR_KEEP, 0);
        ok = gnx_u01(rr.x) < fp.b;
      }
      if (fp.sexed) ok = ok && s.sex[i] == 0;
      ok = ok && s.age[i] >= fp.ra_f;
      if (!ok) mate[i] = -1;
    }
    okr[round] = ok;
    balr[round] = __ballot(ok);
    if (lane == 0) wcnt[round][wave] = __popcll(balr[round]);
  }
  if (tid == 0) n_hard_s = 0;
  __syncthreads();
  int n_list = 0;
#pragma unroll
  for (int round = 0; round < ROUNDS; ++round) {
    int off = n_list;
    for (int w = 0; w < wave; ++w) off += wcnt[round][w];
    if (okr[round])
      list[off + __popcll(balr[round] & ((1ull << lane) - 1ull))] =
          (int32_t)(base + round * 256 + tid);
    n_list += wcnt[round][0] + wcnt[round][1] + wcnt[round][2] + wcnt[round][3];
  }
  __syncthreads();
  if (MODE != GNX_MATE_NEAREST) {
    constexpr bool WT = MODE == GNX_MATE_INVERSE;
    constexpr int STEP = WT ? 2 : 1;
    for (int t = tid; t < n_list; t += 256) {
      const int i = list[t];
      const uint4 me = cand[i];
      const float fx = __uint_as_float(me.x), fy = __uint_as_float(me.y);
      const FmRanges R = fm_ranges(fx, fy, inv_cs, ncx, ncy, cell_start, min(ref, 2));
      const unsigned int M = R.M;
      const unsigned long long fid = (unsigned long long)s.id[i];
      int found = -1;
      bool open = false;
      if (M > 1) {
        const int early = min(fm_blocks<WT>(M), easy_rounds * STEP);
        for (int blk = 0; blk < early && found < 0; blk += STEP) {
          const uint4 w = gnx_rand4(fp.seed, fid, fp.step, OP_MATE_PICK, blk);
          const uint4 w2 = WT ? gnx_rand4(fp.seed, fid, fp.step, OP_MATE_PICK, blk + 1) : w;
          const unsigned int wi[4] = {w.x, WT ? w.z : w.y, WT ? w2.x : w.z, WT ? w2.z : w.w};
          const unsigned int wa[4] = {w.y, w.w, w2.y, w2.w};
          int slot[4];
          uint4 c[4];
#pragma unroll
          for (int q = 0; q < 4; ++q) {
            slot[q] = R.slot((int)__umulhi(wi[q], M));
            c[q] = cand[slot[q]];
          }
#pragma unroll
          for (int q = 0; q < 4; ++q) {
            const float dx = __uint_as_float(c[q].x) - fx, dy = __uint_as_float(c[q].y) - fy;
            const float d2 = dx * dx + dy * dy;
            bool ok = slot[q] != i && d2 <= r2;
            if (WT) ok = ok && d2 > 0.f && gnx_u01(wa[q]) * r < r - sqrtf(d2);
            if (ok && found < 0) found = slot[q];
          }
        }
        open = found < 0;
      }
      if (open)
        hard[atomicAdd(&n_hard_s, 1)] = i;
      else
        mate[i] = found;
    }
    __syncthreads();
    const int n_hard = n_hard_s;
    for (int hh = wave; hh < n_hard; hh += 4) {
      const int i = __builtin_amdgcn_readfirstlane(hard[hh]);
      const uint4 me = cand[i];
      const float fx = __uint_as_float(me.x), fy = __uint_as_float(me.y);
      const FmRanges R = fm_ranges(fx, fy, inv_cs, ncx, ncy, cell_start, min(ref, 2));
      const unsigned int M = R.M;
      const unsigned long long fid = (unsigned long long)s.id[i];
      const int blocks = fm_blocks<WT>(M);
      int found = -1;
      for (int b0 = easy_rounds * STEP; b0 < blocks && found < 0; b0 += 64) {
        const int blk = b0 + lane;
        const uint4 w = gnx_rand4(fp.seed, fid, fp.step, OP_MATE_PICK, blk);
        constexpr int NT = WT ? 2 : 4;
        const unsigned int wi[4] = {w.x, WT ? w.z : w.y, w.z, w.w};
        const unsigned int wa[2] = {w.y, w.w};
        int slot[NT];
        uint4 c[NT];
#pragma unroll
        for (int q = 0; q < NT; ++q) {
          slot[q] = R.slot((int)__umulhi(wi[q], M));
          c[q] = cand[slot[q]];
        }
        int mine = -1;
#pragma unroll
        for (int q = 0; q < NT; ++q) {
          const float dx = __uint_as_float(c[q].x) - fx, dy = __uint_as_float(c[q].y) - fy;
          const float d2 = dx * dx + dy * dy;
          bool ok = slot[q] != i && d2 <= r2;
          if (WT) ok = ok && d2 > 0.f && gnx_u01(wa[q]) * r < r - sqrtf(d2);
          if (ok && mine < 0) mine = slot[q];
        }
        const unsigned long long bal = __ballot(blk < blocks && mine >= 0);
        if (bal)
          found = __builtin_amdgcn_readlane(
              mine, __builtin_amdgcn_readfirstlane(__ffsll((long long)bal) - 1));
      }
      if (found < 0) {
        unsigned int m = 0;
        float wsum = 0.f;
        for (unsigned int j0 = 0; j0 < M; j0 += 256) {
          uint4 c[4];
          int sl[4];
#pragma unroll
          for (int q = 0; q < 4; ++q) {
            const unsigned int j = j0 + q * 64 + lane;
            sl[q] = j < M ? R.slot((int)j) : -1;
            if (sl[q] >= 0) c[q] = cand[sl[q]];
          }
#pragma unroll
          for (int q = 0; q < 4; ++q) {
            float wj = 0.f;
            bool in = false;
            if (sl[q] >= 0) {
              const float dx = __uint_as_float(c[q].x) - fx, dy = __uint_as_float(c[q].y) - fy;
              const float d2 = dx * dx + dy * dy;
              in = sl[q] != i && d2 <= r2 && (!WT || d2 > 0.f);
              if (WT && in) wj = r - sqrtf(d2);
            }
            unsigned long long bal = __ballot(in);
            m += (unsigned int)__popcll(bal);
            if (WT)
              while (bal) {
                const int k = __ffsll((long long)bal) - 1;
                bal &= bal - 1;
                wsum = wsum + __uint_as_float(__builtin_amdgcn_readlane(__float_as_uint(wj), k));
              }
          }
        }
        if (m > 0) {
          const uint4 w0 = gnx_rand4(fp.seed, fid, fp.step, OP_MATE_PICK, blocks);
          unsigned int want = __umulhi(w0.x, m);
          const float target = gnx_u01(w0.x) * wsum;
          float run = 0.f;
          int last = -1;
          for (unsigned int j0 = 0; j0 < M && found < 0; j0 += 256) {
            uint4 c[4];
            int sl[4];
#pragma unroll
            for (int q = 0; q < 4; ++q) {
              const unsigned int j = j0 + q * 64 + lane;
              sl[q] = j < M ? R.slot((int)j) : -1;
              if (sl[q] >= 0) c[q] = cand[sl[q]];
            }
#pragma unroll
            for (int q = 0; q < 4; ++q) {
              float wj = 0.f;
              bool in = false;
              if (sl[q] >= 0) {
                const float dx = __uint_as_float(c[q].x) - fx, dy = __uint_as_float(c[q].y) - fy;
                const float d2 = dx * dx + dy * dy;
                in = sl[q] != i && d2 <= r2 && (!WT || d2 > 0.f);
                if (WT && in) wj = r - sqrtf(d2);
              }
              unsigned long long bal = __ballot(in);
              if (found >= 0) continue;
              if (WT) {
                while (bal && found < 0) {
                  const int k = __ffsll((long long)bal) - 1;
                  bal &= bal - 1;
                  run = run + __uint_as_float(__builtin_amdgcn_readlane(__float_as_uint(wj), k));
                  last = __builtin_amdgcn_readlane(sl[q], k);
                  if (run > target) found = last;
                }
              } else {
                const unsigned int n_in = (unsigned int)__popcll(bal);
                if (want < n_in) {
                  const unsigned long long pick = __ballot(
                      in && (unsigned int)__popcll(bal & ((1ull << lane) - 1ull)) == want);
// ... 184 lines not shown
  if (n_dev) nb = (int)(((int64_t)*n_dev + GNX_CB - 1) / GNX_CB);
  if (dd) nb = (int)(((int64_t)dd->N + GNX_CB - 1) / GNX_CB);
  const int seg = (nb + 15) / 16;
  const int b0 = wave * seg, b1 = min(nb, b0 + seg);
  int run = 0;
  for (int b = b0; b < b1; ++b) run += blk_cnt[(int64_t)b * GNX_VTN + c];
  seg_tot[wave][c] = run;
  __syncthreads();
  int before = 0, total = 0;
  for (int w = 0; w < 16; ++w) {
    const int t = seg_tot[w][c];
    before += w < wave ? t : 0;
    total += t;
  }
  run = before;
  for (int b = b0; b < b1; ++b) {
    const int v = blk_cnt[(int64_t)b * GNX_VTN + c];
    blk_off[(int64_t)b * GNX_VTN + c] = run;
    run += v;
  }
  if (wave != 0) return;
  vt_count[c] = total;
  if (local) {
    int xs = total;
#pragma unroll
    for (int d = 1; d < 64; d <<= 1) {
      const int yv = __shfl_up(xs, d);
      if (c >= d) xs += yv;
    }
    vt_base[c] = (int64_t)(xs - total) * lam;
  }
}

struct GnxGoff {
  const int64_t* goff;
  const uint8_t* cls;
  const int32_t* rank;
  const int32_t* pblk;
  const int32_t* blk_off;
  const int64_t* vt_base;
  int64_t mul;
};

int gnx_vt_buffers(gnx_state* h) {
  if (h->vt_cls) return 0;
  const size_t cap = (size_t)h->cfg.cap_inds;
  const size_t nb = cap / GNX_CB + 2;
  HIPCHK(hipMalloc((void**)&h->vt_cls, cap));
  HIPCHK(hipMalloc((void**)&h->vt_scls, cap));
  HIPCHK(hipMalloc((void**)&h->vt_blk_nz, nb * sizeof(unsigned long long)));
  HIPCHK(hipMalloc((void**)&h->vt_rank, cap * sizeof(int32_t)));
  HIPCHK(hipMalloc((void**)&h->vt_pblk, cap * sizeof(int32_t)));
  HIPCHK(hipMalloc((void**)&h->vt_blk_cnt, nb * GNX_VTN * sizeof(int32_t)));
  HIPCHK(hipMalloc((void**)&h->vt_blk_off, nb * GNX_VTN * sizeof(int32_t)));
  HIPCHK(hipMalloc((void**)&h->vt_count, (GNX_VTN + GNX_MAX_TILES + 8) * sizeof(int32_t)));
  HIPCHK(hipMemset(h->vt_count, 0, (GNX_VTN + GNX_MAX_TILES + 8) * sizeof(int32_t)));
  HIPCHK(hipMalloc((void**)&h->vt_base, GNX_VTN * sizeof(int64_t)));
  return 0;
}

static GnxVtP gnx_vtp(const gnx_state* h) {
  const int vw = h->cfg.W / GNX_VT, vh = h->cfg.H / GNX_VT;
  return GnxVtP{vw, vh, 1.0f / (float)vw, 1.0f / (float)vh};
}

static int gnx_vt_out(gnx_state* h, GnxVtOut* out) {
  *out = GnxVtOut{nullptr, nullptr, nullptr, 0, nullptr, nullptr, nullptr, nullptr, 0, 1,
                  GnxVtP{1, 1, 1.f, 1.f}};
  h->vt_fused = false;
  if (h->id_order != 1 || !h->sp.n_births_fixed || h->sp.mating_radius < 0) return 0;
  GNXCHK(gnx_vt_buffers(h));
  *out = GnxVtOut{h->vt_scls, h->vt_blk_cnt, h->vt_blk_nz, (int)(h->cfg.cap_inds / GNX_CB + 2),
                  h->vt_count, h->vt_cls, h->vt_rank, h->vt_base,
                  h->tiled ? 0 : 1, (int64_t)h->sp.n_births_lambda, gnx_vtp(h)};
  h->vt_fused = true;
  return 0;
}

int gnx_l_pair_cls(gnx_state* h, int64_t P, bool local) {
  GNXCHK(gnx_vt_buffers(h));
  GnxSoA s = h->soa[h->cur];
  if (h->sp.n_births_fixed) {
    if (!h->vt_fused && h->N > 0 && P != 0) {
      gnx_set_error("tile-major offspring ids: the pair list was made without its classification");
      return 1;
    }
    if (local != !h->tiled) {
      gnx_set_error("tile-major offspring ids: the bases' owner does not match the tile grid");
      return 1;
    }
    h->vt_mul = (int64_t)h->sp.n_births_lambda;
    h->vt_weighted = false;
    if (h->N == 0 || P == 0)
      HIPCHK(hipMemsetAsync(h->vt_count, 0, GNX_VTN * sizeof(int32_t), h->stream));
    h->pair_goff_local_base = local;
    h->pair_goff_ready = true;
    return 0;
  }
  int nb;
  {
    h->vt_weighted = true;
    nb = (int)((P + GNX_CB - 1) / GNX_CB);
    h->vt_mul = 1;
    if (P > 0)
      hipLaunchKernelGGL(k_pair_cls, dim3(nb), dim3(256), 0, h->stream, P, (const int32_t*)nullptr,
                         (const int32_t*)h->pairs, (const float*)s.x, (const float*)s.y,
                         (const int32_t*)h->nbirths, gnx_vtp(h), h->vt_cls, h->vt_rank, h->vt_pblk,
                         h->vt_blk_cnt);
  }
  if (P == 0) nb = 0;
  hipLaunchKernelGGL(k_cls_scan, dim3(1), dim3(1024), 0, h->stream, nb, (const int32_t*)nullptr,
                     (const GnxDD*)nullptr, (const int32_t*)h->vt_blk_cnt, h->vt_blk_off,
                     h->vt_count, h->vt_base, local ? 1 : 0, h->vt_mul);
  HIPCHK(hipGetLastError());
  h->pair_goff_local_base = local;
  h->pair_goff_ready = true;
  return 0;
}

static GnxGoff gnx_goff_vt(const gnx_state* h) {
  if (!h->vt_weighted)
    return GnxGoff{nullptr, h->vt_cls, h->vt_rank, nullptr, nullptr, h->vt_base, h->vt_mul};
  return GnxGoff{nullptr, h->vt_cls, h->vt_rank, h->vt_pblk, h->vt_blk_off, h->vt_base, h->vt_mul};
}

struct PairP {
  int64_t N;
  const int32_t* focal;
  const int32_t* mate;
  const uint8_t* keep_in;
  float b;
  int sexed, ra_f, ra_m, dedup;
  long long step;
  unsigned long long seed;
  const GnxDD* dd;
};

__device__ __forceinline__ bool pair_ok(const PairP& P, const GnxSoA& s, int64_t i) {
  const int m = P.mate[i];
  if (m < 0) return false;
  const int fo = P.focal ? P.focal[i] : (int)i;
  bool keep;
  if (P.keep_in) {
    keep = P.keep_in[i] != 0;
  } else {
    uint4 r = gnx_rand4(P.seed, (unsigned long long)s.id[i], P.step, OP_PAIR_KEEP, 0);
    keep = gnx_u01(r.x) < P.b;
  }
  bool ok = keep;
  if (P.sexed) ok = ok && (s.sex[fo] == 0) && (s.sex[m] == 1);
  return ok && (s.age[fo] >= P.ra_f) && (s.age[m] >= P.ra_m);
}

__global__ void __launch_bounds__(256)
k_pair_flags(PairP P, GnxSoA s, int32_t* flag2, int32_t* cnt, GnxVtOut vt) {
  __shared__ int lds[16];
  __shared__ int vtot[GNX_VTN];
  if (vt.scls && threadIdx.x < GNX_VTN) vtot[threadIdx.x] = 0;
  const int64_t base = (int64_t)blockIdx.x * GNX_CB;
  P.N = gnx_dd_n(P.dd, P.N);
  P.step = gnx_dd_step(P.dd, P.step);
  bool f[4];
  float px[4] = {0.f, 0.f, 0.f, 0.f}, py[4] = {0.f, 0.f, 0.f, 0.f};
  if (vt.scls) {
#pragma unroll
    for (int r = 0; r < 4; ++r) {
      const int64_t i = base + r * 256 + threadIdx.x;
      if (i < P.N) {
        px[r] = s.x[i];
        py[r] = s.y[i];
      }
    }
  }
#pragma unroll
  for (int r = 0; r < 4; ++r) {
    const int64_t i = base + r * 256 + threadIdx.x;
    f[r] = false;
    if (i < P.N) {
      bool ok = pair_ok(P, s, i);
      if (ok && P.dedup) {
        const int m = P.mate[i];
        if (P.mate[m] == (int32_t)i && s.id[m] < s.id[i] && pair_ok(P, s, m)) ok = false;
      }
      if (s.ghost[P.focal ? P.focal[i] : (int)i]) ok = false;
      f[r] = ok;
      flag2[i] = ok ? 1 : 0;
    }
  }
  int rank[4], tot;
  gnx_block_ranks(f, rank, tot, lds);
  if (threadIdx.x == 0) cnt[blockIdx.x] = tot;
  if (!vt.scls) return;
  const int lane = threadIdx.x & 63;
#pragma unroll
  for (int r = 0; r < 4; ++r) {
    const int64_t i = base + r * 256 + threadIdx.x;
    int c = GNX_VTN;
    if (f[r]) {
      c = gnx_vt_of(vt.V, px[r], py[r]);
      vt.scls[i] = (uint8_t)c;
    }
    unsigned long long todo = __ballot(f[r]);
    while (todo) {
      const int leader = __ffsll((long long)todo) - 1;
      const int lc = __shfl(c, leader);
      const unsigned long long same = __ballot(f[r] && c == lc);
      if (lane == leader) atomicAdd(&vtot[lc], __popcll(same));
      todo &= ~same;
    }
  }
  __syncthreads();
  if (threadIdx.x < GNX_VTN) {
    const int t = vtot[threadIdx.x];
    vt.blk_cnt[(int64_t)threadIdx.x * vt.stride + blockIdx.x] = t;
    if (t) atomicAdd(&vt.total[threadIdx.x], t);
    const unsigned long long nz = __ballot(t != 0);
    if (threadIdx.x == 0) vt.blk_nz[blockIdx.x] = nz;
  }
}

__global__ void __launch_bounds__(256)
k_pair_compact(int64_t N, const int32_t* focal, const int32_t* mate, const int32_t* flag2,
               const int32_t* blk_off, const float* x, const float* y, const uint64_t* popkey,
               int idbits, int32_t* pairs, float* mid_x, float* mid_y, uint64_t* key,
               const int32_t* __restrict__ cnt, int32_t* __restrict__ total_dev,
               int64_t* __restrict__ host, long long seq, const int32_t* __restrict__ extra,
               GnxDD* __restrict__ dd, int dd_births, int64_t dd_cap, GnxBinP bins, GnxVtOut vt) {
  __shared__ int lds[16];
  __shared__ int psum[4];
  __shared__ int vcnt[16][GNX_VTN];
  __shared__ int vpre[GNX_VTN];
  if (dd) N = dd->N;
  if (vt.cls) {
    for (int k = threadIdx.x; k < 16 * GNX_VTN; k += 256) (&vcnt[0][0])[k] = 0;
    const int lane = threadIdx.x & 63, wave = threadIdx.x >> 6;
    unsigned long long nz = vt.blk_nz[blockIdx.x];
    for (int k = 0; nz; ++k) {
      const int c = __ffsll((long long)nz) - 1;
      nz &= nz - 1;
      if ((k & 3) != wave) continue;
      const int32_t* row = vt.blk_cnt + (int64_t)c * vt.stride;
      int part = 0;
      for (int b2 = lane; b2 < (int)blockIdx.x; b2 += 64) part += row[b2];
#pragma unroll
      for (int d = 32; d > 0; d >>= 1) part += __shfl_xor(part, d);
      if (lane == 0) vpre[c] = part;
    }
    if (vt.local && blockIdx.x == 0 && wave == 3) {
      const int tot = vt.total[lane];
      int xs = tot;
#pragma unroll
      for (int d = 1; d < 64; d <<= 1) {
        const int yv = __shfl_up(xs, d);
        if (lane >= d) xs += yv;
      }
      vt.base[lane] = (int64_t)(xs - tot) * vt.lam;
    }
  }
  int self_off = 0;
  if (cnt) {
    const int lane = threadIdx.x & 63, wave = threadIdx.x >> 6;
    const int upto = blockIdx.x == 0 ? (int)gridDim.x : (int)blockIdx.x;
    int part = 0;
    for (int i = threadIdx.x; i < upto; i += 256) part += cnt[i];
#pragma unroll
    for (int d = 32; d > 0; d >>= 1) part += __shfl_xor(part, d);
    if (lane == 0) psum[wave] = part;
    __syncthreads();
    const int sum = psum[0] + psum[1] + psum[2] + psum[3];
    self_off = blockIdx.x == 0 ? 0 : sum;
    if (blockIdx.x == 0 && threadIdx.x == 0) {
      *total_dev = sum;
      if (dd) {
        int64_t births = (int64_t)sum * dd_births;
        if ((int64_t)dd->N + births > dd_cap) {
          dd->err |= GNX_DD_ERR_SLOTS;
          births = 0;
        }
        dd->P = sum;
        dd->B = (int32_t)births;
      }
      if (host) {
        __hip_atomic_store(&host[0], (int64_t)sum, __ATOMIC_RELAXED, __HIP_MEMORY_SCOPE_SYSTEM);
        if (extra)
          __hip_atomic_store(&host[12], (int64_t)*extra, __ATOMIC_RELAXED, __HIP_MEMORY_SCOPE_SYSTEM);
        asm volatile("s_waitcnt vmcnt(0)" ::: "memory");
        if (seq)
          __hip_atomic_store(&host[3], (int64_t)seq, __ATOMIC_RELAXED, __HIP_MEMORY_SCOPE_SYSTEM);
      }
    }
  }
  const int64_t base = (int64_t)blockIdx.x * GNX_CB;
  bool f[4];
  int sc[4] = {0, 0, 0, 0};
#pragma unroll
  for (int r = 0; r < 4; ++r) {
    const int64_t i = base + r * 256 + threadIdx.x;
    f[r] = i < N && flag2[i] != 0;
    if (vt.cls && i < N) sc[r] = vt.scls[i];
  }
  int rank[4], tot;
  gnx_block_ranks(f, rank, tot, lds);
  int vc[4] = {0, 0, 0, 0}, vrw[4] = {0, 0, 0, 0};
  float fx[4], fy[4];
  int fo4[4];
#pragma unroll
  for (int r = 0; r < 4; ++r) {
    const int64_t i = base + r * 256 + threadIdx.x;
    fo4[r] = f[r] ? (focal ? focal[i] : (int)i) : 0;
    fx[r] = f[r] ? x[fo4[r]] : 0.f;
    fy[r] = f[r] ? y[fo4[r]] : 0.f;
  }
  if (vt.cls) {
    const int lane = threadIdx.x & 63, wave = threadIdx.x >> 6;
#pragma unroll
    for (int r = 0; r < 4; ++r) {
      vc[r] = f[r] ? sc[r] : GNX_VTN;
      gnx_vt_wave_ranks<false>(f[r], vc[r], 1, lane, vcnt[r * 4 + wave], vrw[r]);
    }
    __syncthreads();
  }
  const int32_t bo = cnt ? self_off : blk_off[blockIdx.x];
#pragma unroll
  for (int r = 0; r < 4; ++r) {
    const int64_t i = base + r * 256 + threadIdx.x;
    int bin = 0;
    if (f[r]) {
      const int p = bo + rank[r];
      const int m = mate[i];
      const int fo = fo4[r];
      pairs[2 * p] = fo;
      pairs[2 * p + 1] = m;
      const float mx = (fx[r] + x[m]) / 2.0f, my = (fy[r] + y[m]) / 2.0f;
      mid_x[p] = mx;
      mid_y[p] = my;
      const uint64_t k = popkey[i];
      key[p] = ((k >> idbits) << 40) | (k & ((1ull << idbits) - 1ull));
      if (bins.bins) bin = gnx_bin_of(bins, mx, my);
      if (vt.cls) {
        const int wave = threadIdx.x >> 6;
        int before = vpre[vc[r]];
        for (int j = 0; j < r * 4 + wave; ++j) before += vcnt[j][vc[r]];
        vt.cls[p] = (uint8_t)vc[r];
        vt.rank[p] = before + vrw[r];
      }
    }
    if (bins.bins) gnx_bin_add(bins.bins, bin, f[r]);
  }
}

__global__ void k_panmixia(int64_t N, const int64_t* id, long long step, unsigned long long seed,
                           int32_t* focal, int32_t* mate) {
  int64_t i = (int64_t)blockIdx.x * blockDim.x + threadIdx.x;
  if (i >= N) return;
  uint4 r = gnx_rand4(seed, (unsigned long long)id[i], step, OP_PAIR_KEEP, 1);
  int f = (int)(((unsigned long long)r.x * (unsigned long long)N) >> 32);
  int m = (int)(((unsigned long long)r.y * (unsigned long long)N) >> 32);
  focal[i] = f;
  mate[i] = (m == f) ? -1 : m;
}

int gnx_l_find_pairs(gnx_state* h, const uint8_t* d_keep, int64_t* n_pairs_out, bool with_density) {
  int rc = gnx_l_find_pairs_enqueue(h, d_keep, with_density);
  if (rc) {
    *n_pairs_out = 0;
    return rc;
  }
  return gnx_l_find_pairs_finish(h, n_pairs_out);
}

constexpr int GNX_FM_EASY_ROUNDS = 2;

int gnx_l_find_pairs_enqueue(gnx_state* h, const uint8_t* d_keep, bool with_density) {
  int64_t N = h->N;
  h->n_pairs = 0;
  h->pairs_wait = false;
  if (N == 0) return 0;
  const gnx_species_params& sp = h->sp;
  GnxSoA s = h->soa[h->cur];
  int sexed = sp.sexed;
  const int32_t* focal = nullptr;
  gnx_time_begin(h);
  if (sp.mating_radius < 0) {
    focal = h->off_pair;
    hipLaunchKernelGGL(k_panmixia, dim3(gnx_grid(N, 256)), dim3(256), 0, h->stream, N, s.id,
                       h->step, h->cfg.seed, h->off_pair, h->mate);
  } else {
    float r = (float)sp.mating_radius;
    float r2 = r * r;
    FocalP fp{N, d_keep, (float)sp.b, sexed, sp.repro_age[0], h->step, h->cfg.seed};
    dim3 grid(gnx_grid(N, FM_PER_BLOCK)), blk(256);
    const uint4* cd = (const uint4*)h->cand;
    if (sp.mate_mode == GNX_MATE_NEAREST)
      hipLaunchKernelGGL(k_find_mates<GNX_MATE_NEAREST>, grid, blk, 0, h->stream, fp, s, cd,
                         h->inv_cs, h->cell_start, h->ncx, h->ncy, h->cell_ref, r, r2, GNX_FM_EASY_ROUNDS, h->mate);
    else if (sp.mate_mode == GNX_MATE_INVERSE)
      hipLaunchKernelGGL(k_find_mates<GNX_MATE_INVERSE>, grid, blk, 0, h->stream, fp, s, cd,
                         h->inv_cs, h->cell_start, h->ncx, h->ncy, h->cell_ref, r, r2, GNX_FM_EASY_ROUNDS, h->mate);
    else
      hipLaunchKernelGGL(k_find_mates<GNX_MATE_UNIFORM>, grid, blk, 0, h->stream, fp, s, cd,
                         h->inv_cs, h->cell_start, h->ncx, h->ncy, h->cell_ref, r, r2, GNX_FM_EASY_ROUNDS, h->mate);
  }
  gnx_time_end(h, GNX_K_FIND_MATES, (double)N * 16.0);
  GNXCHK(gnx_permute_rest_launch(h));
  gnx_time_begin(h);
  const int nb = (int)((N + GNX_CB - 1) / GNX_CB);
  PairP pp{N, focal, h->mate, d_keep, (float)sp.b, sexed, sp.repro_age[0], sp.repro_age[1],
           (sexed || sp.mating_radius < 0) ? 0 : 1,
           h->step, h->cfg.seed};
  GnxVtOut vto;
  GNXCHK(gnx_vt_out(h, &vto));
  hipLaunchKernelGGL(k_pair_flags, dim3(nb), dim3(256), 0, h->stream, pp, s, h->flag2, h->blk_cnt, vto);
  const int64_t seq = ++h->pin_seq;
  const bool with_top = h->half_top && h->genomes_assigned;
  hipLaunchKernelGGL(k_pair_compact, dim3(nb), dim3(256), 0, h->stream, N, focal, h->mate,
                     h->flag2, h->blk_off, s.x, s.y, h->key64[1], gnx_id_bits(h), h->pairs,
                     h->mid_x, h->mid_y, h->key64[0],
                     (const int32_t*)h->blk_cnt, h->cnt_dev,
                     h->h_pin_dev + 4, (long long)seq,
                     with_top ? (const int32_t*)h->half_top : (const int32_t*)nullptr,
                     (GnxDD*)nullptr, 0, (int64_t)0, GnxBinP{nullptr, 0.0, 0, 0}, vto);
  gnx_time_end(h, GNX_K_PAIRS, (double)N * 40.0);
  HIPCHK(hipGetLastError());
  if (with_density && gnx_fused_bins(h)) {
    GNXCHK(gnx_l_lattice_P_async(h, N));
  } else if (with_density) {
    const bool lds_bins = (size_t)h->lat.nbx * h->lat.nby * sizeof(int32_t) <= 48 * 1024;
    if (lds_bins)
      GNXCHK(gnx_l_density(h, N, h->mid_x, h->mid_y, &h->spl_P, nullptr, h->cnt_dev));
    else
      with_density = false;
  }
  h->pairs_wait = true;
  h->pairs_seq = seq;
  h->pairs_with_top = with_top;
  h->pairs_with_density = with_density;
  return 0;
}

int gnx_l_find_pairs_finish(gnx_state* h, int64_t* n_pairs_out) {
  *n_pairs_out = 0;
  if (!h->pairs_wait) return 0;
  h->pairs_wait = false;
  GNXCHK(gnx_wait_published(h, 4, h->pairs_seq));
  h->n_pairs = h->h_pin[4];
  if (h->pairs_with_top) h->half_free_est = h->h_pin[16];
  *n_pairs_out = h->n_pairs;
  if (!h->pairs_with_density) h->spl_P.valid = false;
  else if (h->n_pairs == 0) h->spl_P.valid = false;
  if (h->xo_launch_late) GNXCHK(gnx_xo_launch_pending(h, GNX_PC_XO_P2));
  return 0;
}

__global__ void k_births(int64_t P, const int32_t* pairs, const int64_t* id, float thr,
                         long long step, unsigned long long seed, int32_t* nb) {
  int64_t p = (int64_t)blockIdx.x * blockDim.x + threadIdx.x;
  if (p >= P) return;
  GnxStream st(seed, (unsigned long long)id[pairs[2 * p]], step, OP_BIRTHS);
  int k = 0;
  float prod = 1.0f;
  for (int j = 0; j < 64; ++j) {
    prod = prod * gnx_u01(st.next());
    if (!(prod > thr)) break;
    k++;
  }
  nb[p] = max(k, 1);
}

__global__ void k_expand_births(int64_t P, const int32_t* nb, const int32_t* boff,
                                int32_t* off_pair) {
  int64_t p = (int64_t)blockIdx.x * blockDim.x + threadIdx.x;
  if (p >= P) return;
  int o = boff[p];
  for (int q = 0; q < nb[p]; ++q) off_pair[o + q] = (int32_t)p;
}

struct OffP {
  int64_t N, B, cap;
  int W, H, n_layers;
  float xmax, ymax, rrx, rry;
  int distr;
  float p1, p2;
  int surf, surf_layer;
  float surf_kappa;
  int sexed;
  float p_male;
  int fixed_nb;
  int genomes;
  int n_paths;
  int64_t id_base, n_free;
  long long step;
  unsigned long long seed;
  int fuse_tb, TW;
  const uint64_t* path_sel;
  const uint8_t* dom;
  GnxBinP bins;
  const GnxDD* dd;
  const uint64_t* ptb;
  const int32_t* pmap;
  const int32_t* P_dev;
};

struct GnxReq {
  int64_t* pid;
  int32_t* k;
  int32_t* key;
  uint8_t* start;
  float* px;
  float* py;
  int32_t* count;
};

__device__ __forceinline__ bool disperse_once(float mx, float my, float theta, float dist,
                                              float rrx, float rry, float xmax, float ymax,
                                              float& ox, float& oy) {
  float dx = cosf(theta) * dist;
  float dy = sinf(theta) * dist;
  if (rrx != 1.0f) dx *= rrx;
  if (rry != 1.0f) dy *= rry;
  ox = fminf(fmaxf(mx + dx, 0.0f), xmax);
  oy = fminf(fmaxf(my + dy, 0.0f), ymax);
  return ox > 0.0f && oy > 0.0f;
}

__global__ void __launch_bounds__(256)
k_offspring(OffP P, GnxSoA s, const float* rast, const int32_t* pairs, const int32_t* off_pair,
            const int32_t* boff, GnxGoff gf,
            int32_t* off_parent, int32_t* off_keys, uint8_t* off_start, GnxReq rq, GnxTraitTab T,
            int32_t* __restrict__ ord_tail) {
  int64_t k = (int64_t)blockIdx.x * blockDim.x + threadIdx.x;
  if (P.dd) {
    P.N = P.dd->N;
    P.B = P.dd->B;
    P.id_base = P.dd->max_id + 1;
    P.step = P.dd->step;
  }
  if (P.P_dev) {
    P.B = (int64_t)*P.P_dev * P.fixed_nb;
    if (P.N + P.B > P.cap || (P.genomes && P.B > P.n_free)) return;
  }
  if (k >= P.B) return;
  int64_t p, ord;
  if (P.fixed_nb > 0) {
    p = k / P.fixed_nb;
    ord = k - p * P.fixed_nb;
  } else {
    p = off_pair[k];
    ord = k - boff[p];
  }
  int64_t gk = k;
  if (gf.cls) {
    const int c = gf.cls[p];
    int64_t rk = gf.rank[p];
    if (gf.pblk) rk += gf.blk_off[(int64_t)gf.pblk[p] * GNX_VTN + c];
    gk = gf.vt_base[c] + rk * gf.mul + ord;
  } else if (gf.goff) {
    gk = gf.goff[p] + ord;
  }
  int i = pairs[2 * p], m = pairs[2 * p + 1];
  int64_t slot = P.N + k;
  unsigned long long oid = (unsigned long long)(P.id_base + gk);
  if (ord_tail) ord_tail[(P.dd ? P.N : 0) + gk] = (int32_t)slot;
  float mx = (s.x[i] + s.x[m]) / 2.0f;
  float my = (s.y[i] + s.y[m]) / 2.0f;
  const uint4 r = gnx_rand4(P.seed, oid, P.step, OP_OFFSPRING, 0);
  const uint8_t st0 = (uint8_t)(r.x & 1u), st1 = (uint8_t)((r.x >> 1) & 1u);
  const int32_t k0 = (int32_t)(((unsigned long long)r.y * (unsigned long long)P.n_paths) >> 32);
  const int32_t k1 = (int32_t)(((unsigned long long)r.z * (unsigned long long)P.n_paths) >> 32);
  const bool tb_regs = P.genomes && P.fuse_tb && P.TW > 0 && P.TW <= 2;
  uint64_t pi[4] = {0, 0, 0, 0}, pm[4] = {0, 0, 0, 0}, ps0[2] = {0, 0}, ps1[2] = {0, 0};
// ... 148 lines not shown
  Q.B = B;
  Q.cap = c.cap_inds;
  Q.W = c.W;
  Q.H = c.H;
  Q.n_layers = c.n_layers;
  Q.xmax = (float)(c.W - 0.001);
  Q.ymax = (float)(c.H - 0.001);
  Q.rrx = (float)sp.res_ratio[0];
  Q.rry = (float)sp.res_ratio[1];
  Q.distr = sp.disp_distr;
  Q.p1 = (float)sp.disp_p1;
  Q.p2 = (float)sp.disp_p2;
  Q.surf = sp.disp_surf;
  Q.surf_layer = sp.disp_surf_layer;
  Q.surf_kappa = (float)sp.disp_surf_kappa;
  Q.sexed = sp.sexed;
  Q.p_male = (float)sp.p_male;
  Q.fixed_nb = sp.n_births_fixed ? (int)sp.n_births_lambda : 0;
  Q.genomes = genomes ? 1 : 0;
  Q.n_paths = h->n_paths;
  Q.id_base = id_base >= 0 ? id_base : h->max_id + 1;
  Q.n_free = h->n_free;
  Q.step = h->step;
  Q.seed = c.seed;
  Q.fuse_tb = genomes ? 1 : 0;
  Q.TW = h->TW;
  Q.path_sel = h->path_sel;
  Q.dom = h->dom;
  Q.bins = GnxBinP{nullptr, 1.0 / h->lat.hww, h->lat.nbx, h->lat.nby};
  Q.P_dev = nullptr;
  Q.ptb = h->soa[h->cur].tb;
  Q.pmap = nullptr;
  return Q;
}

int gnx_l_mate(gnx_state* h, bool burn, bool inject, int64_t B_inject, int64_t* births_out,
               int64_t id_base, bool tiled) {
  const gnx_config& c = h->cfg;
  GnxSoA s = h->soa[h->cur];
  *births_out = 0;
  int64_t B = 0;
  bool ord_tail_used = false;
  GNXCHK(gnx_xo_flush_deferred(h));
  bool genomes = !burn && c.L > 0 && h->genomes_assigned;
  if (inject) {
    B = B_inject;
    if (B == 0) return 0;
    if (h->N + B > c.cap_inds || B > h->n_free) {
      gnx_set_error("capacity exceeded: N=%lld + B=%lld > cap_inds=%lld or free rows %lld",
                    (long long)h->N, (long long)B, (long long)c.cap_inds, (long long)h->n_free);
      return 2;
    }
    hipLaunchKernelGGL(k_offspring_inject, dim3(gnx_grid(B, 256)), dim3(256), 0, h->stream, h->N,
                       B, c.cap_inds, s, h->rast, c.n_layers, c.W, c.H, h->off_parent, h->max_id);
  } else {
    if (!tiled) {
      GNXCHK(gnx_l_births(h, &B));
      if (h->id_order == 1 && h->n_pairs > 0 && h->sp.mating_radius >= 0)
        GNXCHK(gnx_l_pair_cls(h, h->n_pairs, true));
    }
    B = h->n_births_pending;
    if (B == 0) {
      h->pair_goff_ready = false;
      return 0;
    }
    if (h->N + B > c.cap_inds || (genomes && B > h->n_free)) {
      gnx_set_error("capacity exceeded: N=%lld + births=%lld > cap_inds=%lld (free rows %lld)",
                    (long long)h->N, (long long)B, (long long)c.cap_inds, (long long)h->n_free);
      return 2;
    }
    OffP Q = gnx_make_offp(h, genomes, tiled, id_base, B);
    if (gnx_fused_bins(h) && h->fb_adults && h->fb_count == h->N) {
      Q.bins.bins = h->fb[h->fb_cur];
      h->fb_count += B;
    } else {
      h->fb_adults = false;
    }
    GnxReq rq{};
    if (tiled && genomes) {
      rq.pid = h->req_pid;
      rq.k = h->req_k;
      rq.key = h->req_key;
      rq.start = h->req_start;
      rq.px = h->req_px;
      rq.py = h->req_py;
      rq.count = h->req_count;
      if (!h->req_zeroed) HIPCHK(hipMemsetAsync(h->req_count, 0, sizeof(int32_t), h->stream));
      h->req_zeroed = false;
    }
    int32_t* ord_tail = nullptr;
    if (h->pair_goff_ready && h->pair_goff_local_base && h->ord_mode && h->ord_valid && !h->tiled &&
        h->ord_n == h->N)
      ord_tail = h->ord[h->ord_cur] + h->ord_n;
    ord_tail_used = ord_tail != nullptr;
    GnxGoff gf{};
    if (h->pair_goff_ready) gf = gnx_goff_vt(h);
    else if (tiled && !h->pair_goff_local) gf.goff = h->pair_goff;
    gnx_time_begin(h);
    hipLaunchKernelGGL(k_offspring, dim3(gnx_grid(B, 256)), dim3(256), 0, h->stream, Q, s, h->rast,
                       h->pairs, h->off_pair, h->boff, gf,
                       h->off_parent, h->off_keys, h->off_start, rq, gnx_trait_tab(h), ord_tail);
    gnx_time_end(h, GNX_K_OFFSPRING, (double)B * (60.0 + 8.0 * c.n_layers + 48.0 * h->TW +
                                                  4.0 * c.n_traits));
    if (tiled && genomes) {
      if (h->n_req_known >= 0) {
        h->n_req = h->n_req_known;
      } else {
        GNXCHK(gnx_publish(h, 0, h->req_count));
        HIPCHK(hipStreamSynchronize(h->stream));
        h->n_req = h->h_pin[0];
      }
    }
  }
  HIPCHK(hipGetLastError());
  if (genomes || inject) {
    const bool fused = !inject;
    if (!fused) GNXCHK(gnx_l_newborn_tb(h, h->N, B));
    const bool defer = h->defer_xo && !inject && h->stream2 != nullptr;
    if (defer) {
      if (tiled) GNXCHK(gnx_l_crossover_requests(h, h->N, h->n_req));
      h->xo_deferred = true;
      h->xo_first = h->N;
      h->xo_B = B;
    } else {
      GNXCHK(gnx_l_crossover_all(h, h->N, B));
    }
    if (c.n_traits > 0 && !tiled && !fused) GNXCHK(gnx_l_phenotype(h, h->N, B));
  }
  h->N += B;
  if (!tiled) h->max_id += B;
  if (h->pair_goff_ready) {
    h->pair_goff_ready = false;
    if (ord_tail_used)
      h->ord_n += B;
    else
      h->ord_valid = false;
  }
  *births_out = B;
  return 0;
}

int gnx_dd_l_sort(gnx_state* h, int32_t* d_bins, hipStream_t st) {
  const gnx_config& c = h->cfg;
  const int64_t n_fixed = c.cap_inds;
  GnxSoA a = h->soa[h->cur], b = h->soa[h->cur ^ 1];
  const int front_geometry = n_fixed <= (1 << 21) ? 1 : 0;
  GNXCHK(gnx_os_keys_hist(h->os_scratch, h->tickets + 3, n_fixed, 0, h->ord[h->ord_cur], h->cell32,
                          h->keyk[0], h->valk[0], h->key_bits, st, h->dd, front_geometry));
  GNXCHK(gnx_os_sort32_ranked(h->os_scratch, h->os_ktmp, h->os_vtmp, h->keyk[0], h->keyk[1],
                              h->valk[0], h->valk[1], (size_t)n_fixed, h->key_bits, st));
  const int64_t wipe_words = (int64_t)gnx_os_words_used((size_t)n_fixed, h->key_bits);
  hipLaunchKernelGGL(k_permute, dim3(gnx_grid(n_fixed, 256)), dim3(256), 0, st, n_fixed, c.cap_inds,
                     h->valk[1], a, b, c.n_layers, c.n_traits, a.tb ? 2 * h->TW : 0,
                     (unsigned long long)c.seed, h->tag, (uint4*)h->cand, h->key64[1], 40,
                     h->cell_start, h->ncx * h->ncy, h->keyk[1], h->ord[h->ord_cur], (int64_t)0,
                     h->ord[h->ord_cur ^ 1], h->perm[1], (uint4*)h->os_scratch, (wipe_words + 3) / 4,
                     0, (const GnxDD*)h->dd,
                     GnxBinP{d_bins, 1.0 / h->lat.hww, h->lat.nbx, h->lat.nby},
                     h->id_order == 1 ? h->vt_count : (int32_t*)nullptr);
  HIPCHK(hipGetLastError());
  h->ord_cur ^= 1;
  h->cur ^= 1;
  return 0;
}

int gnx_dd_l_pairs(gnx_state* h, int32_t* d_bins, hipStream_t st) {
  const gnx_species_params& sp = h->sp;
  const int64_t cap = h->cfg.cap_inds;
  GnxSoA s = h->soa[h->cur];
  const float r = (float)sp.mating_radius, r2 = r * r;
  FocalP fp{cap, nullptr, (float)sp.b, sp.sexed, sp.repro_age[0], 0, h->cfg.seed, h->dd};
  dim3 grid(gnx_grid(cap, FM_PER_BLOCK)), blk(256);
  const uint4* cd = (const uint4*)h->cand;
  if (sp.mate_mode == GNX_MATE_NEAREST)
    hipLaunchKernelGGL(k_find_mates<GNX_MATE_NEAREST>, grid, blk, 0, st, fp, s, cd, h->inv_cs,
                       h->cell_start, h->ncx, h->ncy, h->cell_ref, r, r2, GNX_FM_EASY_ROUNDS, h->mate);
  else if (sp.mate_mode == GNX_MATE_INVERSE)
    hipLaunchKernelGGL(k_find_mates<GNX_MATE_INVERSE>, grid, blk, 0, st, fp, s, cd, h->inv_cs,
                       h->cell_start, h->ncx, h->ncy, h->cell_ref, r, r2, GNX_FM_EASY_ROUNDS, h->mate);
  else
    hipLaunchKernelGGL(k_find_mates<GNX_MATE_UNIFORM>, grid, blk, 0, st, fp, s, cd, h->inv_cs,
                       h->cell_start, h->ncx, h->ncy, h->cell_ref, r, r2, GNX_FM_EASY_ROUNDS, h->mate);
  const int nb = (int)((cap + GNX_CB - 1) / GNX_CB);
  PairP pp{cap, nullptr, h->mate, nullptr, (float)sp.b, sp.sexed, sp.repro_age[0], sp.repro_age[1],
           sp.sexed ? 0 : 1, 0, h->cfg.seed, h->dd};
  GnxVtOut vto;
  GNXCHK(gnx_vt_out(h, &vto));
  hipLaunchKernelGGL(k_pair_flags, dim3(nb), dim3(256), 0, st, pp, s, h->flag2, h->blk_cnt, vto);
  hipLaunchKernelGGL(k_pair_compact, dim3(nb), dim3(256), 0, st, cap, (const int32_t*)nullptr,
                     h->mate, h->flag2, h->blk_off, s.x, s.y, h->key64[1], 40, h->pairs, h->mid_x,
                     h->mid_y, h->key64[0], (const int32_t*)h->blk_cnt, h->cnt_dev,
                     (int64_t*)nullptr, 0ll, (const int32_t*)nullptr, h->dd,
                     (int)sp.n_births_lambda, (int64_t)cap,
                     GnxBinP{d_bins, 1.0 / h->lat.hww, h->lat.nbx, h->lat.nby}, vto);
  if (vto.cls) {
    h->vt_mul = (int64_t)sp.n_births_lambda;
    h->vt_weighted = false;
  }
  HIPCHK(hipGetLastError());
  return 0;
}

int gnx_dd_l_offspring(gnx_state* h, bool genomes, int32_t* d_bins, hipStream_t st) {
  OffP Q = gnx_make_offp(h, genomes, false, 0, 0);
  Q.dd = h->dd;
  Q.bins.bins = d_bins;
  const bool vt = h->vt_fused && h->id_order == 1;
  hipLaunchKernelGGL(k_offspring, dim3(gnx_grid(h->cfg.cap_inds, 256)), dim3(256), 0, st, Q,
                     h->soa[h->cur], h->rast, h->pairs, h->off_pair, h->boff,
                     vt ? gnx_goff_vt(h) : GnxGoff{}, h->off_parent, h->off_keys, h->off_start,
                     GnxReq{}, gnx_trait_tab(h), vt ? h->ord[h->ord_cur] : (int32_t*)nullptr);
  HIPCHK(hipGetLastError());
  return 0;
}

__global__ void k_dispersal_inject(int64_t B, int A, const float* mx, const float* my,
                                   const float* theta, const float* dist, float rrx, float rry,
                                   float xmax, float ymax, float* ox, float* oy, int32_t* used) {
  int64_t k = (int64_t)blockIdx.x * blockDim.x + threadIdx.x;
  if (k >= B) return;
  float x = 0.f, y = 0.f;
  int u = A - 1;
  for (int a = 0; a < A; ++a) {
    if (disperse_once(mx[k], my[k], theta[(int64_t)a * B + k], dist[(int64_t)a * B + k], rrx, rry,
                      xmax, ymax, x, y)) {
      u = a;
      break;
    }
  }
  ox[k] = x;
  oy[k] = y;
  used[k] = u;
}

int gnx_l_dispersal_inject(gnx_state* h, int64_t B, int A, const float* d_mx, const float* d_my,
                           const float* d_theta, const float* d_dist, float* d_ox, float* d_oy,
                           int32_t* d_used) {
  const gnx_config& c = h->cfg;
  hipLaunchKernelGGL(k_dispersal_inject, dim3(gnx_grid(B, 256)), dim3(256), 0, h->stream, B, A,
                     d_mx, d_my, d_theta, d_dist, (float)h->sp.res_ratio[0],
                     (float)h->sp.res_ratio[1], (float)(c.W - 0.001), (float)(c.H - 0.001), d_ox,
                     d_oy, d_used);
  HIPCHK(hipGetLastError());
  return 0;
}
```

### geonomics_amd/csrc/gnx_tile.hip

```cpp
#include <algorithm>
#include <atomic>
#include "gnx_internal.h"
#include "gnx_rng.h"

#include "gnx_xo.h"

struct TileBox {
  float x0, y0, x1, y1;
  int r, c, R, C;
};

static TileBox tile_box(const gnx_state* h) {
  TileBox t;
  float tw = (float)h->cfg.W / h->tile_C, th = (float)h->cfg.H / h->tile_R;
  t.x0 = h->tile_c * tw;
  t.x1 = (h->tile_c + 1) * tw;
  t.y0 = h->tile_r * th;
  t.y1 = (h->tile_r + 1) * th;
  t.r = h->tile_r;
  t.c = h->tile_c;
  t.R = h->tile_R;
  t.C = h->tile_C;
  return t;
}

extern "C" int gnx_tile_set(gnx_state* h, int32_t R, int32_t C, int32_t r, int32_t c) {
  if (R < 1 || C < 1 || r < 0 || r >= R || c < 0 || c >= C || h->cfg.W % C || h->cfg.H % R) {
    gnx_set_error("gnx_tile_set: bad tile grid %dx%d (%d,%d) for a %dx%d landscape", R, C, r, c,
                  h->cfg.W, h->cfg.H);
    return 1;
  }
  h->route_geo_epoch = 0;
  h->tile_R = R;
  h->tile_C = C;
  h->tile_r = r;
  h->tile_c = c;
  h->tiled = R * C > 1;
  return 0;
}

__global__ void k_mark_out(int64_t N, const float* x, const float* y, TileBox t, int32_t* flag,
                           uint8_t* dead) {
  int64_t i = (int64_t)blockIdx.x * blockDim.x + threadIdx.x;
  if (i >= N) return;
  bool out = x[i] < t.x0 || x[i] >= t.x1 || y[i] < t.y0 || y[i] >= t.y1;
  flag[i] = out ? 1 : 0;
  dead[i] = out ? 1 : 0;
}

struct HaloSpans {
  int cx0[3], cx1[3], cy0[3], cy1[3];
  int okx[3], oky[3];
};

__global__ void k_mark_halo(int64_t N, const float* x, const float* y, const uint8_t* ghost,
                            HaloSpans sp, double inv_cs, int ncx, int ncy, int32_t* flag,
                            int32_t* mask) {
  int64_t i = (int64_t)blockIdx.x * blockDim.x + threadIdx.x;
  if (i >= N) return;
  int m = 0;
  if (!ghost[i]) {
    const int cx = min(ncx - 1, (int)((double)x[i] * inv_cs));
    const int cy = min(ncy - 1, (int)((double)y[i] * inv_cs));
    for (int dy = 0; dy < 3; ++dy)
      for (int dx = 0; dx < 3; ++dx) {
        if (dx == 1 && dy == 1) continue;
        if (sp.okx[dx] && sp.oky[dy] && cx >= sp.cx0[dx] && cx <= sp.cx1[dx] &&
            cy >= sp.cy0[dy] && cy <= sp.cy1[dy])
          m |= 1 << (dy * 3 + dx);
      }
  }
  mask[i] = m;
  flag[i] = m ? 1 : 0;
}

__global__ void k_mark_everybody(int64_t N, const uint8_t* ghost, int32_t* flag, int32_t* mask) {
  int64_t i = (int64_t)blockIdx.x * blockDim.x + threadIdx.x;
  if (i >= N) return;
  const int m = ghost[i] ? 0 : 0x1EF;
  mask[i] = m;
  flag[i] = m ? 1 : 0;
}

static HaloSpans halo_spans(const gnx_state* h) {
  HaloSpans sp;
  const int tw = h->cfg.W / h->tile_C, th = h->cfg.H / h->tile_R;
  for (int d = 0; d < 3; ++d) {
    const int cc = h->tile_c + d - 1, rr = h->tile_r + d - 1;
    sp.okx[d] = cc >= 0 && cc < h->tile_C;
    sp.oky[d] = rr >= 0 && rr < h->tile_R;
    const float x0 = (float)(cc * tw), x1 = nextafterf((float)((cc + 1) * tw), 0.f);
    const float y0 = (float)(rr * th), y1 = nextafterf((float)((rr + 1) * th), 0.f);
    const int ring = 2 * h->cell_ref;
    sp.cx0[d] = std::min(h->ncx - 1, (int)((double)x0 * h->inv_cs)) - ring;
    sp.cx1[d] = std::min(h->ncx - 1, (int)((double)x1 * h->inv_cs)) + ring;
    sp.cy0[d] = std::min(h->ncy - 1, (int)((double)y0 * h->inv_cs)) - ring;
    sp.cy1[d] = std::min(h->ncy - 1, (int)((double)y1 * h->inv_cs)) + ring;
  }
  return sp;
}

__global__ void k_pack(int64_t N, int64_t cap, const int32_t* flag, const int32_t* scan,
                       const int32_t* mask, GnxSoA s, int n_traits, gnx_ind_rec* rec, float* zrec,
                       int64_t* slots) {
  int64_t i = (int64_t)blockIdx.x * blockDim.x + threadIdx.x;
  if (i >= N || !flag[i]) return;
  int64_t q = scan[i];
  gnx_ind_rec r;
  r.x = s.x[i];
  r.y = s.y[i];
  r.age = s.age[i];
  r.sex = s.sex[i];
  r.id = s.id[i];
  r.fit = s.fit[i];
  r.nbr_mask = mask ? mask[i] : 0;
  rec[q] = r;
  if (zrec)
    for (int t = 0; t < n_traits; ++t) zrec[q * n_traits + t] = s.z[(int64_t)t * cap + i];
  if (slots) slots[q] = i;
}

__global__ void k_unpack(int64_t N, int64_t n, int64_t cap, GnxSoA s, const gnx_ind_rec* rec,
                         const float* zrec, int n_traits, int n_layers, const float* rast, int W,
                         int H, const int32_t* free_rows, int64_t n_free, int has_rows, int ghost,
                         GnxHalves Hv) {
  int64_t k = (int64_t)blockIdx.x * blockDim.x + threadIdx.x;
  if (k >= n) return;
  int64_t slot = N + k;
  gnx_ind_rec r = rec[k];
  s.x[slot] = r.x;
  s.y[slot] = r.y;
  s.age[slot] = r.age;
  s.sex[slot] = (uint8_t)r.sex;
  s.id[slot] = r.id;
  s.fit[slot] = r.fit;
  s.ghost[slot] = (uint8_t)ghost;
  s.grow[slot] = (has_rows && !ghost) ? free_rows[n_free - 1 - k] : -1;
  if (has_rows && !ghost)
    for (int q = 0; q < 2 * Hv.NB; ++q)
      gnx_half_new(Hv, (int64_t)s.grow[slot] * 2 * Hv.NB + q, true);
  for (int t = 0; t < n_traits; ++t)
    s.z[(int64_t)t * cap + slot] = zrec ? zrec[k * n_traits + t] : 0.f;
  int cx = (int)r.x, cy = (int)r.y;
  for (int l = 0; l < n_layers; ++l)
    s.e[(int64_t)l * cap + slot] = rast[((int64_t)l * H + cy) * W + cx];
}

template <typename T>
static int dalloc_t(T** p, size_t n) {
  *p = nullptr;
  HIPCHK(hipMalloc((void**)p, std::max<size_t>(n, 1) * sizeof(T)));
  return 0;
}

static bool has_rows(const gnx_state* h) { return h->genomes_assigned && h->cfg.L > 0; }

static int stage_selection(gnx_state* h, const int32_t* d_mask, bool with_z, bool with_geno,
                           int64_t* n_out) {
  int64_t N = h->N;
  GnxSoA s = h->soa[h->cur];
  HIPCHK(hipMemsetAsync(h->flag + N, 0, sizeof(int32_t), h->stream));
  GNXCHK(gnx_prim_scan(h->scan_tmp, h->scan_tmp_bytes, h->flag, h->scan, (size_t)N + 1,
                       h->stream));
  GNXCHK(gnx_publish(h, 0, h->scan + N));
  HIPCHK(hipStreamSynchronize(h->stream));
  int64_t n = h->h_pin[0];
  *n_out = n;
  h->st_n = n;
  h->st_has_geno = false;
  if (n == 0) return 0;
  if (n > h->st_cap) {
    (void)hipFree(h->st_rec);
    (void)hipFree(h->st_z);
    (void)hipFree(h->st_slots);
    h->st_cap = n + n / 4 + 1024;
    GNXCHK(dalloc_t(&h->st_rec, (size_t)h->st_cap));
    GNXCHK(dalloc_t(&h->st_z, (size_t)h->st_cap * std::max(h->cfg.n_traits, 1)));
    GNXCHK(dalloc_t(&h->st_slots, (size_t)h->st_cap));
  }
  hipLaunchKernelGGL(k_pack, dim3(gnx_grid(N, 256)), dim3(256), 0, h->stream, N, h->cfg.cap_inds,
                     h->flag, h->scan, d_mask, s, h->cfg.n_traits, h->st_rec,
                     (with_z && h->cfg.n_traits) ? h->st_z : nullptr, h->st_slots);
  if (with_geno && has_rows(h)) {
    if (n > h->st_geno_cap) {
      (void)hipFree(h->st_geno);
      h->st_geno_cap = n + n / 4 + 64;
      GNXCHK(dalloc_t(&h->st_geno, (size_t)h->st_geno_cap * 2 * h->W64));
    }
    GNXCHK(gnx_l_gather_genomes(h, n, h->st_slots, h->st_geno));
    h->st_has_geno = true;
  }
  HIPCHK(hipGetLastError());
  return 0;
}

extern "C" int gnx_tile_export_migrants(gnx_state* h, int64_t* n_out) {
  *n_out = 0;
  if (h->n_ghost) {
    gnx_set_error("gnx_tile_export_migrants: ghosts are resident");
    return 1;
  }
  int64_t N = h->N;
  if (N == 0) return 0;
  GnxSoA s = h->soa[h->cur];
  hipLaunchKernelGGL(k_mark_out, dim3(gnx_grid(N, 256)), dim3(256), 0, h->stream, N, s.x, s.y,
                     tile_box(h), h->flag, h->dead_in);
  GNXCHK(stage_selection(h, nullptr, true, true, n_out));
  if (*n_out > 0) {
    int64_t D = 0;
    GNXCHK(gnx_l_mortality(h, h->dead_in, &D));
    HIPCHK(hipStreamSynchronize(h->stream));
  }
  return 0;
}

extern "C" int gnx_tile_export_halo(gnx_state* h, int64_t* n_out) {
  *n_out = 0;
  int64_t N = h->N;
  if (N == 0) return 0;
  GnxSoA s = h->soa[h->cur];
  if (h->have_sp && h->sp.mating_radius < 0)
    hipLaunchKernelGGL(k_mark_everybody, dim3(gnx_grid(N, 256)), dim3(256), 0, h->stream, N, s.ghost,
                       h->flag, h->mate);
  else
    hipLaunchKernelGGL(k_mark_halo, dim3(gnx_grid(N, 256)), dim3(256), 0, h->stream, N, s.x, s.y,
                       s.ghost, halo_spans(h), h->inv_cs, h->ncx, h->ncy, h->flag, h->mate);
  return stage_selection(h, h->mate, false, false, n_out);
}

extern "C" int gnx_tile_get_staged(gnx_state* h, gnx_ind_rec* rec, float* z, uint64_t* geno) {
  int64_t n = h->st_n;
  if (n == 0) return 0;
  if (rec) GNXCHK(gnx_d2h(h, rec, h->st_rec, n * sizeof(gnx_ind_rec)));
  if (z && h->st_z && h->cfg.n_traits)
    GNXCHK(gnx_d2h(h, z, h->st_z, n * h->cfg.n_traits * sizeof(float)));
  if (geno && h->st_has_geno)
    GNXCHK(gnx_d2h(h, geno, h->st_geno, (size_t)n * 2 * h->W64 * 8));
  return 0;
}

static int import_common(gnx_state* h, int64_t n, const gnx_ind_rec* rec, const float* z,
                         const uint64_t* geno, int ghost) {
  if (n == 0) return 0;
  const gnx_config& c = h->cfg;
  const bool rows = has_rows(h) && !ghost;
  if (h->N + n > c.cap_inds || (rows && n > h->n_free)) {
    gnx_set_error("capacity exceeded importing %lld individuals (N=%lld cap=%lld free rows %lld)",
                  (long long)n, (long long)h->N, (long long)c.cap_inds, (long long)h->n_free);
    return 2;
  }
  for (int64_t k = 0; k < n; ++k)
    if (!(rec[k].x >= 0 && rec[k].x < c.W && rec[k].y >= 0 && rec[k].y < c.H)) {
      gnx_set_error("import: record %lld is off the landscape", (long long)k);
      return 1;
    }
  gnx_ind_rec* d_rec = nullptr;
  float* d_z = nullptr;
  u64* d_g = nullptr;
  GNXCHK(dalloc_t(&d_rec, (size_t)n));
  GNXCHK(gnx_h2d(h, d_rec, rec, n * sizeof(gnx_ind_rec)));
  if (z && c.n_traits) {
    GNXCHK(dalloc_t(&d_z, (size_t)n * c.n_traits));
    GNXCHK(gnx_h2d(h, d_z, z, n * c.n_traits * sizeof(float)));
  }
  GnxSoA s = h->soa[h->cur];
  if (rows && !ghost) GNXCHK(gnx_half_reserve(h, 2 * (int64_t)h->NB * n));
  hipLaunchKernelGGL(k_unpack, dim3(gnx_grid(n, 256)), dim3(256), 0, h->stream, h->N, n,
                     c.cap_inds, s, d_rec, d_z, c.n_traits, c.n_layers, h->rast, c.W, c.H,
                     h->free_rows, h->n_free, rows ? 1 : 0, ghost,
                     gnx_halves(h));
  if (rows) {
    if (!geno) {
      gnx_set_error("import: genomes are assigned on this tile but none were sent");
      return 1;
    }
    GNXCHK(dalloc_t(&d_g, (size_t)n * 2 * h->W64));
    GNXCHK(gnx_h2d(h, d_g, geno, (size_t)n * 2 * h->W64 * 8));
    GNXCHK(gnx_l_scatter_genomes(h, n, (const uint64_t*)d_g, h->N));
    h->n_free -= n;
    GNXCHK(gnx_l_tb_from_rows(h, h->N, n, nullptr, nullptr));
  }
  HIPCHK(hipStreamSynchronize(h->stream));
  (void)hipFree(d_rec);
  (void)hipFree(d_z);
  (void)hipFree(d_g);
  h->N += n;
  h->ord_valid = false;
  if (ghost) h->n_ghost += n;
  for (int64_t k = 0; k < n; ++k) h->max_id = std::max<int64_t>(h->max_id, rec[k].id);
  HIPCHK(hipGetLastError());
  return 0;
}

extern "C" int gnx_tile_import(gnx_state* h, int64_t n, const gnx_ind_rec* rec, const float* z,
                               const uint64_t* geno) {
  return import_common(h, n, rec, z, geno, 0);
}

extern "C" int gnx_tile_import_ghosts(gnx_state* h, int64_t n, const gnx_ind_rec* rec) {
  return import_common(h, n, rec, nullptr, nullptr, 1);
}

extern "C" int gnx_tile_pairs(gnx_state* h, int32_t burn, int64_t* n_pairs, int64_t* n_births) {
  if (!h->have_sp) {
    gnx_set_error("species parameters not set");
    return 1;
  }
  int64_t P = 0, B = 0;
  GNXCHK(gnx_l_sort_by_cell(h));
  GNXCHK(gnx_l_find_pairs(h, nullptr, &P));
  GNXCHK(gnx_l_bins(h, P, h->mid_x, h->mid_y, nullptr, h->bins_P));
  GNXCHK(gnx_l_births(h, &B));
  *n_pairs = P;
  *n_births = B;
  return 0;
}

extern "C" int gnx_tile_pair_info(gnx_state* h, int64_t* focal_ids, int32_t* n_births) {
  int64_t P = h->n_pairs;
  if (P == 0) return 0;
  GNXCHK(gnx_d2h(h, focal_ids, h->key64[0], P * sizeof(int64_t)));
  if (h->sp.n_births_fixed)
    for (int64_t p = 0; p < P; ++p) n_births[p] = (int32_t)h->sp.n_births_lambda;
  else
    GNXCHK(gnx_d2h(h, n_births, h->nbirths, P * sizeof(int32_t)));
  return 0;
}

extern "C" int gnx_get_bins(gnx_state* h, int32_t which, int32_t* out) {
  size_t nb = (size_t)h->lat.nbx * h->lat.nby;
  HIPCHK(hipStreamSynchronize(h->stream));
  const int32_t* src = which ? h->bins_P : (h->last_N_fused ? h->fb[h->fb_cur ^ 1] : h->bin_partials);
  GNXCHK(gnx_d2h(h, out, src, nb * sizeof(int32_t)));
  return 0;
}

extern "C" int gnx_set_bins(gnx_state* h, int32_t which, const int32_t* in) {
  size_t nb = (size_t)h->lat.nbx * h->lat.nby;
  GNXCHK(gnx_h2d(h, which ? h->bins_P : h->bin_partials, in, nb * sizeof(int32_t)));
  h->bins_zeroed[which ? 1 : 0] = false;
  if (!which) h->last_N_fused = false;
  return 0;
}

extern "C" int gnx_density_bin_count(gnx_state* h) { return h->lat.nbx * h->lat.nby; }

struct SideStream {
  gnx_state* h;
  hipStream_t saved;
  explicit SideStream(gnx_state* hh) : h(hh), saved(hh->stream) {
    if (h->xo_pending && h->stream2) h->stream = h->stream2;
  }
  ~SideStream() { h->stream = saved; }
};

extern "C" int gnx_tile_offspring(gnx_state* h, int32_t burn, int64_t id_base,
                                  const int64_t* pair_goff, int64_t* n_requests) {
  *n_requests = 0;
  int64_t P = h->n_pairs, B = 0;
  h->birth_first_slot = h->N;
  h->n_req = 0;
  h->tile_births_settled = false;
  if (P > 0 && pair_goff)
    GNXCHK(gnx_h2d(h, h->pair_goff, pair_goff, P * sizeof(int64_t)));
  GNXCHK(gnx_l_mate(h, burn != 0, false, 0, &B, id_base, true));
  h->last_births = B;
  if (B == 0) h->n_req = 0;
  *n_requests = h->n_req;
  h->xo_pending = B > 0 && !burn && has_rows(h);
  return 0;
}

static int serve_wait_crossover(gnx_state* h, hipStream_t main_stream) {
  if (h->stream == h->stream2 && h->stream2 != nullptr) {
    hipStream_t cur = h->stream;
    h->stream = main_stream;
    int rc = gnx_xo_launch_pending(h);
    h->stream = cur;
    return rc;
  }
  GNXCHK(gnx_xo_launch_pending(h));
  return gnx_xo_wait_inflight(h);
}

extern "C" int gnx_tile_get_requests(gnx_state* h, int64_t* pid, int32_t* child_k, int32_t* key,
                                     uint8_t* start, float* px, float* py) {
  SideStream side(h);
  int64_t n = h->n_req;
  if (n == 0) return 0;
  GNXCHK(gnx_d2h(h, pid, h->req_pid, n * 8));
  GNXCHK(gnx_d2h(h, child_k, h->req_k, n * 4));
  GNXCHK(gnx_d2h(h, key, h->req_key, n * 4));
  GNXCHK(gnx_d2h(h, start, h->req_start, n));
  GNXCHK(gnx_d2h(h, px, h->req_px, n * 4));
  GNXCHK(gnx_d2h(h, py, h->req_py, n * 4));
  return 0;
}

__global__ void k_id_keys(int64_t N, const int64_t* id, uint64_t* key, int32_t* slot) {
  int64_t i = (int64_t)blockIdx.x * blockDim.x + threadIdx.x;
  if (i >= N) return;
  key[i] = (uint64_t)id[i];
  slot[i] = (int32_t)i;
}

__global__ void k_lookup(int64_t n, const int64_t* want, int64_t N, const uint64_t* sorted_ids,
                         const int32_t* sorted_slots, int32_t* out_slot, int32_t* n_missing) {
  int64_t q = (int64_t)blockIdx.x * blockDim.x + threadIdx.x;
  if (q >= n) return;
  uint64_t w = (uint64_t)want[q];
  int64_t lo = 0, hi = N;
  while (lo < hi) {
    int64_t mid = (lo + hi) >> 1;
    if (sorted_ids[mid] < w) lo = mid + 1; else hi = mid;
  }
  if (lo < N && sorted_ids[lo] == w) {
    out_slot[q] = sorted_slots[lo];
  } else {
    out_slot[q] = -1;
    atomicAdd(n_missing, 1);
  }
}

__global__ void __launch_bounds__(256)
k_make_gametes(int64_t n, int W16, const u64x2* __restrict__ G, const int32_t* __restrict__ grow,
               GnxHalves H, const int32_t* __restrict__ slot, const int32_t* __restrict__ keys,
               const uint8_t* __restrict__ starts, const u64x2* __restrict__ paths,
               u64x2* __restrict__ out) {
  const int lane = threadIdx.x & 63;
  const int64_t q = ((int64_t)blockIdx.x * blockDim.x + threadIdx.x) >> 6;
  if (q >= n) return;
  const int prow = grow[slot[q]];
  const u64 s = starts[q] ? ~0ull : 0ull;
  const int64_t lh0 = (int64_t)prow * 2;
  const u64x2* pm = paths + (int64_t)keys[q] * W16;
  for (int c = lane; c < W16; c += 64) {
    u64x2 m = pm[c];
    m.a ^= s;
    m.b ^= s;
    const u64x2 a = G[gnx_chunk_at(H, lh0, c)], b = G[gnx_chunk_at(H, lh0 + 1, c)];
    u64x2 o;
    o.a = (a.a & ~m.a) | (b.a & m.a);
    o.b = (a.b & ~m.b) | (b.b & m.b);
    out[q * W16 + c] = o;
  }
}

extern "C" int gnx_tile_serve_gametes(gnx_state* h, int64_t n, const int64_t* parent_ids,
                                      const int32_t* keys, const uint8_t* starts,
                                      uint64_t* out) {
  SideStream side(h);
  if (n == 0) return 0;
  if (!has_rows(h) || h->n_paths == 0) {
    gnx_set_error("gnx_tile_serve_gametes: genomes / paths not set");
    return 1;
  }
  for (int64_t q = 0; q < n; ++q)
    if (keys[q] < 0 || keys[q] >= h->n_paths || starts[q] > 1) {
      gnx_set_error("gnx_tile_serve_gametes: request %lld out of range", (long long)q);
      return 1;
    }
  int64_t N = h->N;
  GnxSoA s = h->soa[h->cur];
  GNXCHK(serve_wait_crossover(h, side.saved));
  hipLaunchKernelGGL(k_id_keys, dim3(gnx_grid(N, 256)), dim3(256), 0, h->stream, N, s.id,
                     h->key64[0], h->perm[0]);
  GNXCHK(gnx_prim_sort64(h->sort64_tmp, h->sort64_tmp_bytes, h->key64[0], h->key64[1], h->perm[0],
                         h->perm[1], (size_t)N, h->stream));
  int64_t* d_ids = nullptr;
  int32_t *d_keys = nullptr, *d_slot = nullptr, *d_miss = nullptr;
  uint8_t* d_st = nullptr;
  u64* d_out = nullptr;
  GNXCHK(dalloc_t(&d_ids, (size_t)n));
// ... 254 lines not shown
              int C, int32_t* __restrict__ counts, const int32_t* __restrict__ offs,
              gnx_ind_rec* __restrict__ out) {
  const int64_t i = (int64_t)blockIdx.x * blockDim.x + threadIdx.x;
  const int lane = threadIdx.x & 63;
  int m = 0;
  if (i < N && !s.ghost[i]) m = halo_mask_of(s.x[i], s.y[i], sp, inv_cs, ncx, ncy);
  if (__ballot(m != 0) == 0ull) return;
  for (int k = 0; k < 9; ++k) {
    if (k == 4) continue;
    const unsigned long long b = __ballot((m >> k) & 1);
    if (b == 0ull) continue;
    const int rank = (tr + k / 3 - 1) * C + (tc + k % 3 - 1);
    int base = 0;
    if (lane == __ffsll((long long)b) - 1) base = atomicAdd(&counts[rank], __popcll(b));
    if (WRITE) {
      base = __shfl(base, __ffsll((long long)b) - 1);
      if ((m >> k) & 1) {
        gnx_ind_rec r;
        r.x = s.x[i];
        r.y = s.y[i];
        r.age = s.age[i];
        r.sex = s.sex[i];
        r.id = s.id[i];
        r.fit = s.fit[i];
        r.nbr_mask = m;
        out[offs[rank] + base + __popcll(b & ((1ull << lane) - 1ull))] = r;
      }
    }
  }
}

extern "C" int gnx_tile_export_halo_dev(gnx_state* h, int64_t* counts) {
  GNXCHK(check_tiles(h, "gnx_tile_export_halo_dev"));
  const int nt = n_tiles(h);
  for (int p = 0; p < nt; ++p) counts[p] = 0;
  h->gp_n = 0;
  h->st_has_geno = false;
  const int64_t N = h->N;
  if (N == 0) return 0;
  if (!h->tile_counts) GNXCHK(dalloc_t(&h->tile_counts, (size_t)GNX_MAX_TILES * 2));
  GnxSoA s = h->soa[h->cur];
  const HaloSpans sp = halo_spans(h);
  int32_t* cnt = h->tile_counts;
  int32_t* off = h->tile_counts + GNX_MAX_TILES;
  HIPCHK(hipMemsetAsync(cnt, 0, nt * sizeof(int32_t), h->stream));
  hipLaunchKernelGGL(k_halo_direct<false>, dim3(gnx_grid(N, 256)), dim3(256), 0, h->stream, N, s,
                     sp, h->inv_cs, h->ncx, h->ncy, h->tile_r, h->tile_c, h->tile_C, cnt, nullptr,
                     nullptr);
  std::vector<int32_t> c(nt), o(nt);
  GNXCHK(gnx_d2h(h, c.data(), cnt, nt * sizeof(int32_t)));
  int64_t m = 0;
  for (int p = 0; p < nt; ++p) {
    o[p] = (int32_t)m;
    counts[p] = c[p];
    m += c[p];
  }
  if (m == 0) return 0;
  if (m > h->gp_cap) {
    (void)hipFree(h->gp_rec);
    (void)hipFree(h->gp_z);
    (void)hipFree(h->gp_slots);
    h->gp_cap = m + m / 4 + 1024;
    GNXCHK(dalloc_t(&h->gp_rec, (size_t)h->gp_cap));
    GNXCHK(dalloc_t(&h->gp_z, (size_t)h->gp_cap * std::max(h->cfg.n_traits, 1)));
    GNXCHK(dalloc_t(&h->gp_slots, (size_t)h->gp_cap));
  }
  GNXCHK(gnx_h2d(h, off, o.data(), nt * sizeof(int32_t)));
  HIPCHK(hipMemsetAsync(cnt, 0, nt * sizeof(int32_t), h->stream));
  hipLaunchKernelGGL(k_halo_direct<true>, dim3(gnx_grid(N, 256)), dim3(256), 0, h->stream, N, s,
                     sp, h->inv_cs, h->ncx, h->ncy, h->tile_r, h->tile_c, h->tile_C, cnt, off,
                     h->gp_rec);
  HIPCHK(hipGetLastError());
  h->gp_n = m;
  return 0;
}

extern "C" int gnx_tile_staged_ptrs(gnx_state* h, void** rec, void** z, void** geno) {
  HIPCHK(hipStreamSynchronize(h->stream));
  *rec = h->gp_n ? (void*)h->gp_rec : nullptr;
  *z = (h->gp_n && h->cfg.n_traits) ? (void*)h->gp_z : nullptr;
  *geno = (h->gp_n && h->st_has_geno) ? (void*)h->st_geno : nullptr;
  return 0;
}

__global__ void k_check_rec(int64_t n, const gnx_ind_rec* rec, int W, int H, int64_t* chk) {
  int64_t k = (int64_t)blockIdx.x * blockDim.x + threadIdx.x;
  if (k >= n) return;
  gnx_ind_rec r = rec[k];
  if (!(r.x >= 0 && r.x < W && r.y >= 0 && r.y < H)) atomicAdd((unsigned long long*)&chk[0], 1ull);
  atomicMax((long long*)&chk[1], (long long)r.id);
}

static int import_device(gnx_state* h, int64_t n, const gnx_ind_rec* d_rec, const float* d_z,
                         const uint64_t* d_g, int ghost) {
  if (n == 0) return 0;
  const gnx_config& c = h->cfg;
  const bool rows = has_rows(h) && !ghost;
  if (h->N + n > c.cap_inds || (rows && n > h->n_free)) {
    gnx_set_error("capacity exceeded importing %lld individuals (N=%lld cap=%lld free rows %lld)",
                  (long long)n, (long long)h->N, (long long)c.cap_inds, (long long)h->n_free);
    return 2;
  }
  if (rows && !d_g) {
    gnx_set_error("import: genomes are assigned on this tile but none were sent");
    return 1;
  }
  if (!h->chk) GNXCHK(dalloc_t(&h->chk, 2));
  int64_t init[2] = {0, h->max_id};
  GNXCHK(gnx_h2d(h, h->chk, init, sizeof(init)));
  hipLaunchKernelGGL(k_check_rec, dim3(gnx_grid(n, 256)), dim3(256), 0, h->stream, n, d_rec, c.W,
                     c.H, h->chk);
  int64_t res[2];
  GNXCHK(gnx_d2h(h, res, h->chk, sizeof(res)));
  if (res[0]) {
    gnx_set_error("import: %lld records are off the landscape", (long long)res[0]);
    return 1;
  }
  GnxSoA s = h->soa[h->cur];
  if (rows && !ghost) GNXCHK(gnx_half_reserve(h, 2 * (int64_t)h->NB * n));
  hipLaunchKernelGGL(k_unpack, dim3(gnx_grid(n, 256)), dim3(256), 0, h->stream, h->N, n,
                     c.cap_inds, s, d_rec, (d_z && c.n_traits) ? d_z : nullptr, c.n_traits,
                     c.n_layers, h->rast, c.W, c.H, h->free_rows, h->n_free, rows ? 1 : 0, ghost,
                     gnx_halves(h));
  if (rows) {
    GNXCHK(gnx_l_scatter_genomes(h, n, (const uint64_t*)d_g, h->N));
    h->n_free -= n;
    GNXCHK(gnx_l_tb_from_rows(h, h->N, n, nullptr, nullptr));
  }
  HIPCHK(hipStreamSynchronize(h->stream));
  h->N += n;
  h->ord_valid = false;
  if (ghost) h->n_ghost += n;
  h->max_id = std::max(h->max_id, res[1]);
  HIPCHK(hipGetLastError());
  return 0;
}

extern "C" int gnx_tile_import_dev(gnx_state* h, int64_t n, const void* rec, const void* z,
                                   const void* geno) {
  return import_device(h, n, (const gnx_ind_rec*)rec, (const float*)z, (const uint64_t*)geno, 0);
}

extern "C" int gnx_tile_import_ghosts_dev(gnx_state* h, int64_t n, const void* rec) {
  return import_device(h, n, (const gnx_ind_rec*)rec, nullptr, nullptr, 1);
}

extern "C" int gnx_tile_pair_ptrs(gnx_state* h, int64_t* n_pairs, void** focal_ids,
                                  void** n_births) {
  const int64_t P = h->n_pairs;
  *n_pairs = P;
  *focal_ids = nullptr;
  *n_births = nullptr;
  if (P == 0) return 0;
  HIPCHK(hipStreamSynchronize(h->stream));
  *focal_ids = h->key64[0];
  if (!h->sp.n_births_fixed) *n_births = h->nbirths;
  return 0;
}

extern "C" int gnx_tile_offspring_dev(gnx_state* h, int32_t burn, int64_t id_base,
                                      const void* pair_goff_dev, int64_t* n_requests) {
  *n_requests = 0;
  int64_t P = h->n_pairs, B = 0;
  h->birth_first_slot = h->N;
  h->n_req = 0;
  h->tile_births_settled = false;
  if (P > 0 && pair_goff_dev) {
    HIPCHK(hipMemcpyAsync(h->pair_goff, pair_goff_dev, P * sizeof(int64_t),
                          hipMemcpyDeviceToDevice, h->stream));
    HIPCHK(hipStreamSynchronize(h->stream));
  }
  GNXCHK(gnx_l_mate(h, burn != 0, false, 0, &B, id_base, true));
  h->last_births = B;
  if (B == 0) h->n_req = 0;
  *n_requests = h->n_req;
  h->xo_pending = B > 0 && !burn && has_rows(h);
  return 0;
}

__global__ void k_pack_requests(int64_t n, const int32_t* idx, const int64_t* pid,
                                const int32_t* key, const uint8_t* start, const int32_t* child_k,
                                gnx_gamete_req* out, int32_t* k_out) {
  int64_t q = (int64_t)blockIdx.x * blockDim.x + threadIdx.x;
  if (q >= n) return;
  int i = idx[q];
  gnx_gamete_req r;
  r.parent_id = pid[i];
  r.key = key[i];
  r.start = start[i];
  out[q] = r;
  k_out[q] = child_k[i];
}

extern "C" int gnx_tile_group_requests(gnx_state* h, int64_t* counts, void** req_dev) {
  SideStream side(h);
  GNXCHK(check_tiles(h, "gnx_tile_group_requests"));
  for (int p = 0; p < n_tiles(h); ++p) counts[p] = 0;
  *req_dev = nullptr;
  const int64_t n = h->n_req;
  if (n == 0) return 0;
  if (n > h->rq_cap) {
    (void)hipFree(h->rq_sorted);
    (void)hipFree(h->rq_k);
    h->rq_cap = n + n / 4 + 1024;
    gnx_gamete_req* p = nullptr;
    GNXCHK(dalloc_t(&p, (size_t)h->rq_cap));
    h->rq_sorted = p;
    GNXCHK(dalloc_t(&h->rq_k, (size_t)h->rq_cap));
  }
  hipLaunchKernelGGL(k_req_owner, dim3(gnx_grid(n, 256)), dim3(256), 0, h->stream, n, h->req_px,
                     h->req_py, h->cfg.W / h->tile_C, h->cfg.H / h->tile_R, h->tile_R, h->tile_C,
                     h->key[0], h->perm[0]);
  GNXCHK(group_by_key(h, n, counts));
  hipLaunchKernelGGL(k_pack_requests, dim3(gnx_grid(n, 256)), dim3(256), 0, h->stream, n,
                     h->perm[1], h->req_pid, h->req_key, h->req_start, h->req_k,
                     (gnx_gamete_req*)h->rq_sorted, h->rq_k);
  HIPCHK(hipStreamSynchronize(h->stream));
  HIPCHK(hipGetLastError());
  *req_dev = h->rq_sorted;
  return 0;
}

__global__ void k_lookup_req(int64_t n, const gnx_gamete_req* req, int64_t N, int n_paths,
                             const uint64_t* sorted_ids, const int32_t* sorted_slots,
                             int32_t* out_slot, int32_t* n_bad) {
  int64_t q = (int64_t)blockIdx.x * blockDim.x + threadIdx.x;
  if (q >= n) return;
  const gnx_gamete_req r = req[q];
  uint64_t w = (uint64_t)r.parent_id;
  int64_t lo = 0, hi = N;
  while (lo < hi) {
    int64_t mid = (lo + hi) >> 1;
    if (sorted_ids[mid] < w) lo = mid + 1; else hi = mid;
  }
  const bool ok = lo < N && sorted_ids[lo] == w && r.key >= 0 && r.key < n_paths &&
                  (r.start == 0 || r.start == 1);
  out_slot[q] = ok ? sorted_slots[lo] : -1;
  if (!ok) atomicAdd(n_bad, 1);
}

__global__ void __launch_bounds__(256)
k_make_gametes_req(int64_t n, int W16, const u64x2* __restrict__ G,
                   const int32_t* __restrict__ grow, GnxHalves H,
                   const int32_t* __restrict__ slot, const gnx_gamete_req* __restrict__ req, const u64x2* __restrict__ paths,
                   u64x2* __restrict__ out) {
  const int lane = threadIdx.x & 63;
  const int64_t q = ((int64_t)blockIdx.x * blockDim.x + threadIdx.x) >> 6;
  if (q >= n) return;
  const int prow = grow[slot[q]];
  const gnx_gamete_req r = req[q];
  const u64 s = r.start ? ~0ull : 0ull;
  const int64_t lh0 = (int64_t)prow * 2;
  const u64x2* pm = paths + (int64_t)r.key * W16;
  for (int c = lane; c < W16; c += 64) {
    u64x2 m = pm[c];
    m.a ^= s;
    m.b ^= s;
    const u64x2 a = G[gnx_chunk_at(H, lh0, c)], b = G[gnx_chunk_at(H, lh0 + 1, c)];
    u64x2 o;
    o.a = (a.a & ~m.a) | (b.a & m.a);
    o.b = (a.b & ~m.b) | (b.b & m.b);
    out[q * W16 + c] = o;
  }
}

extern "C" int gnx_tile_serve_gametes_dev(gnx_state* h, int64_t n, const void* req_dev,
                                          void** out_dev) {
  SideStream side(h);
  *out_dev = nullptr;
  if (n == 0) return 0;
  if (!has_rows(h) || h->n_paths == 0) {
    gnx_set_error("gnx_tile_serve_gametes_dev: genomes / paths not set");
    return 1;
  }
  if (n > h->gam_cap) {
    (void)hipFree(h->gam_out);
    (void)hipFree(h->gam_slot);
    h->gam_cap = n + n / 4 + 256;
    GNXCHK(dalloc_t(&h->gam_out, (size_t)h->gam_cap * h->W64));
    GNXCHK(dalloc_t(&h->gam_slot, (size_t)h->gam_cap + 1));
  }
  const int64_t N = h->N;
  GnxSoA s = h->soa[h->cur];
  GNXCHK(serve_wait_crossover(h, side.saved));
  hipLaunchKernelGGL(k_id_keys, dim3(gnx_grid(N, 256)), dim3(256), 0, h->stream, N, s.id,
                     h->key64[0], h->perm[0]);
  GNXCHK(gnx_prim_sort64(h->sort64_tmp, h->sort64_tmp_bytes, h->key64[0], h->key64[1], h->perm[0],
                         h->perm[1], (size_t)N, h->stream));
  int32_t* d_bad = h->gam_slot + h->gam_cap;
  HIPCHK(hipMemsetAsync(d_bad, 0, 4, h->stream));
  hipLaunchKernelGGL(k_lookup_req, dim3(gnx_grid(n, 256)), dim3(256), 0, h->stream, n,
                     (const gnx_gamete_req*)req_dev, N, h->n_paths, h->key64[1], h->perm[1],
                     h->gam_slot, d_bad);
  int bad = 0;
  GNXCHK(gnx_d2h(h, &bad, d_bad, 4));
  if (bad) {
    gnx_set_error("gnx_tile_serve_gametes_dev: %d requests name a parent that does not live on "
                  "this tile, or a path / start out of range", bad);
    return 1;
  }
  const int W16 = h->W64 / 2;
  hipLaunchKernelGGL(k_make_gametes_req, dim3(gnx_grid(n * 64, 256)), dim3(256), 0, h->stream, n,
                     W16, (const u64x2*)h->G, s.grow, gnx_halves(h), h->gam_slot,
                     (const gnx_gamete_req*)req_dev,
                     (const u64x2*)h->paths, (u64x2*)h->gam_out);
  HIPCHK(hipStreamSynchronize(h->stream));
// ... 20 lines not shown
}

extern "C" int gnx_tile_bins_ptr(gnx_state* h, void** bins, int64_t* n_total) {
  HIPCHK(hipStreamSynchronize(h->stream));
  *bins = h->bin_partials;
  *n_total = 2 * (int64_t)h->lat.nbx * h->lat.nby;
  return 0;
}

static int route_geo(const gnx_state* h, RouteGeo* g) {
  if (h->tile_R > GNX_TILE_DIM || h->tile_C > GNX_TILE_DIM) {
    gnx_set_error("tile2: at most %d tiles per axis", GNX_TILE_DIM);
    return 1;
  }
  g->R = h->tile_R;
  g->C = h->tile_C;
  g->tw = h->cfg.W / h->tile_C;
  g->th = h->cfg.H / h->tile_R;
  g->me = h->tile_r * h->tile_C + h->tile_c;
  g->ncx = h->ncx;
  g->ncy = h->ncy;
  g->inv_cs = h->inv_cs;
  const int ring = 2 * h->cell_ref;
  for (int c = 0; c < g->C; ++c) {
    const float x0 = (float)(c * g->tw), x1 = nextafterf((float)((c + 1) * g->tw), 0.f);
    g->cx0[c] = std::min(h->ncx - 1, (int)((double)x0 * h->inv_cs)) - ring;
    g->cx1[c] = std::min(h->ncx - 1, (int)((double)x1 * h->inv_cs)) + ring;
  }
  for (int r = 0; r < g->R; ++r) {
    const float y0 = (float)(r * g->th), y1 = nextafterf((float)((r + 1) * g->th), 0.f);
    g->cy0[r] = std::min(h->ncy - 1, (int)((double)y0 * h->inv_cs)) - ring;
    g->cy1[r] = std::min(h->ncy - 1, (int)((double)y1 * h->inv_cs)) + ring;
  }
  return 0;
}

template <bool WRITE>
__global__ void __launch_bounds__(256)
k_route(int64_t N, int64_t cap, GnxSoA s, RouteGeo g, int n_traits, int32_t* __restrict__ cnt,
        const int32_t* __restrict__ offs, gnx_ind_rec* __restrict__ mig_rec,
        float* __restrict__ mig_z, int64_t* __restrict__ mig_slot,
        gnx_ind_rec* __restrict__ gh_rec, int64_t mig_cap, int64_t gh_cap,
        const int32_t* __restrict__ alive) {
  const int64_t i = (int64_t)blockIdx.x * blockDim.x + threadIdx.x;
  const bool act = i < N && !s.ghost[i] && (!alive || (alive[i] & 1) != 0);
  const int T = g.R * g.C;
  float x = 0.f, y = 0.f;
  int oc = 0, orow = 0, cx = 0, cy = 0;
  if (act) {
    x = s.x[i];
    y = s.y[i];
    oc = tile_index(x, g.tw, g.C);
    orow = tile_index(y, g.th, g.R);
    cx = min(g.ncx - 1, (int)((double)x * g.inv_cs));
    cy = min(g.ncy - 1, (int)((double)y * g.inv_cs));
  }
  const int owner = orow * g.C + oc;
  gnx_ind_rec r;
  if (WRITE && act) {
    r.x = x;
    r.y = y;
    r.age = s.age[i];
    r.sex = s.sex[i];
    r.id = s.id[i];
    r.fit = s.fit[i];
    r.nbr_mask = 0;
  }
  for (int k = 0; k < 9; ++k) {
    int dest = -1;
    if (act) {
      if (k == 4) {
        if (owner != g.me) dest = owner;
      } else {
        const int rr = orow + k / 3 - 1, cc = oc + k % 3 - 1;
        if (rr >= 0 && rr < g.R && cc >= 0 && cc < g.C && cx >= g.cx0[cc] && cx <= g.cx1[cc] &&
            cy >= g.cy0[rr] && cy <= g.cy1[rr])
          dest = rr * g.C + cc;
      }
    }
    if (__ballot(dest >= 0) == 0ull) continue;
    const int grp = (k == 4) ? 0 : T;
    const int idx = gnx_route_append(cnt + grp, dest);
    if (WRITE && dest >= 0) {
      const int64_t q = (int64_t)offs[grp + dest] + idx;
      if (k == 4) {
        if (q < mig_cap) {
          mig_rec[q] = r;
          mig_slot[q] = i;
          if (mig_z)
            for (int t = 0; t < n_traits; ++t) mig_z[q * n_traits + t] = s.z[(int64_t)t * cap + i];
        }
      } else if (q < gh_cap) {
        gh_rec[q] = r;
      }
    }
  }
}

__global__ void k_route_offsets(int T, int32_t* cnt ,
                                int32_t* host, int n_extra, int seq, int zero_counts) {
  if (threadIdx.x != 0 || blockIdx.x != 0) return;
  for (int grp = 0; grp < 2; ++grp) {
    int run = 0;
    for (int p = 0; p < T; ++p) {
      const int v = cnt[grp * T + p];
      cnt[2 * T + grp * T + p] = run;
      run += v;
      if (zero_counts) cnt[grp * T + p] = 0;
    }
    cnt[4 * T + grp] = run;
  }
  if (!host) return;
  for (int p = 0; p < 2 * T + n_extra; ++p)
    __hip_atomic_store(&host[p], cnt[p < 2 * T ? p : 4 * T + (p - 2 * T)], __ATOMIC_RELAXED,
                       __HIP_MEMORY_SCOPE_SYSTEM);
  __builtin_amdgcn_fence(__ATOMIC_RELEASE, "workgroup");
  asm volatile("s_waitcnt vmcnt(0)" ::: "memory");
  __hip_atomic_store(&host[2 * GNX_MAX_TILES + 7], seq, __ATOMIC_RELAXED, __HIP_MEMORY_SCOPE_SYSTEM);
}

__global__ void k_publish_words(int n, const int32_t* src, int32_t* host, int seq) {
  if (threadIdx.x != 0 || blockIdx.x != 0) return;
  for (int p = 0; p < n; ++p)
    __hip_atomic_store(&host[p], src[p], __ATOMIC_RELAXED, __HIP_MEMORY_SCOPE_SYSTEM);
  __builtin_amdgcn_fence(__ATOMIC_RELEASE, "workgroup");
  asm volatile("s_waitcnt vmcnt(0)" ::: "memory");
  __hip_atomic_store(&host[2 * GNX_MAX_TILES + 7], seq, __ATOMIC_RELAXED, __HIP_MEMORY_SCOPE_SYSTEM);
}

__global__ void k_tile2_zero(int32_t* p0, int n0, int32_t* p1, int n1, int32_t* p2, int n2,
                             int32_t* p3, int n3, int32_t* p4, int n4) {
  const int stride = gridDim.x * blockDim.x;
  for (int i = blockIdx.x * blockDim.x + threadIdx.x; i < n1; i += stride) p1[i] = 0;
  for (int i = blockIdx.x * blockDim.x + threadIdx.x; i < n4; i += stride) p4[i] = 0;
  if (blockIdx.x == 0) {
    if ((int)threadIdx.x < n0) p0[threadIdx.x] = 0;
    if ((int)threadIdx.x < n2) p2[threadIdx.x] = 0;
    if ((int)threadIdx.x < n3) p3[threadIdx.x] = 0;
  }
}

__global__ void k_publish_words2(int n1, const int32_t* src1, int32_t* host1, int n2,
                                 const int32_t* src2, int32_t* host2) {
  if (threadIdx.x != 0 || blockIdx.x != 0) return;
  for (int p = 0; p < n1; ++p)
    __hip_atomic_store(&host1[p], src1[p], __ATOMIC_RELAXED, __HIP_MEMORY_SCOPE_SYSTEM);
  for (int p = 0; p < n2; ++p)
    __hip_atomic_store(&host2[p], src2[p], __ATOMIC_RELAXED, __HIP_MEMORY_SCOPE_SYSTEM);
}

#define GNX_REQ_CNT(h) ((h)->route_cnt + 4 * n_tiles(h) + 8)
static int tile2_buffers(gnx_state* h) {
  h->tile2_mode = true;
  if (!h->route_cnt) {
    GNXCHK(dalloc_t(&h->route_cnt, (size_t)5 * GNX_MAX_TILES + 8));
    HIPCHK(hipMemset(h->route_cnt, 0, ((size_t)5 * GNX_MAX_TILES + 8) * sizeof(int32_t)));
    HIPCHK(hipHostMalloc((void**)&h->h_route_pin, (2 * GNX_MAX_TILES + 8) * sizeof(int32_t),
                         hipHostMallocCoherent | hipHostMallocMapped));
    memset(h->h_route_pin, 0, (2 * GNX_MAX_TILES + 8) * sizeof(int32_t));
    HIPCHK(hipHostGetDevicePointer((void**)&h->h_route_pin_dev, h->h_route_pin, 0));
  }
  if (!h->chk) GNXCHK(dalloc_t(&h->chk, 2));
  return 0;
}

static int tile2_wait(gnx_state* h, int seq) {
  volatile int32_t* word = h->h_route_pin + 2 * GNX_MAX_TILES + 7;
  for (long spin = 0;; ++spin) {
    if (*word == seq) break;
    if (spin > 2000000) {
      HIPCHK(hipStreamSynchronize(h->stream));
      if (*word != seq) {
        gnx_set_error("tile2: the device counters never arrived");
        return 1;
      }
      break;
    }
    __builtin_ia32_pause();
  }
  std::atomic_thread_fence(std::memory_order_acquire);
  return 0;
}

extern "C" int gnx_stream_ptr(gnx_state* h, void** stream) {
  *stream = (void*)h->stream;
  return 0;
}

extern "C" int gnx_tile2_route_begin(gnx_state* h, int32_t move, void** counts_dev) {
  GNXCHK(check_tiles(h, "gnx_tile2_move_route"));
  const int T = n_tiles(h);
  *counts_dev = nullptr;
  h->route_n_mig = h->route_n_gh = 0;
  h->st_has_geno = false;
  if (h->n_ghost) {
    gnx_set_error("gnx_tile2_move_route: ghosts are resident");
    return 1;
  }
  GNXCHK(tile2_buffers(h));
  {
    const int nb = h->lat.nbx * h->lat.nby;
    const bool bins = h->have_sp && h->bin_partials != nullptr;
    const int T0 = n_tiles(h);
    hipLaunchKernelGGL(k_tile2_zero, dim3(8), dim3(256), 0, h->stream, (int32_t*)h->chk, 4,
                       bins ? h->bin_partials : nullptr, bins ? 2 * nb + 4 : 0,
                       (int32_t*)h->nmax_bits, h->nmax_bits ? 2 : 0, h->req_count,
                       h->req_count ? 1 : 0, h->route_cnt, 5 * T0 + 8);
    if (bins) h->bins_zeroed[0] = h->bins_zeroed[1] = true;
    h->req_cnt_zeroed = true;
    if (h->nmax_bits) h->nmax_zeroed = true;
    h->req_zeroed = h->req_count != nullptr;
  }
  h->move_counted_routes = false;
  if (move && h->sp.move) {
    h->move_writes_keys = T == 1 && h->sp.mating_radius >= 0;
    if (T > 1 && h->N > 0) {
      if (!h->route_geo_dev) HIPCHK(hipMalloc((void**)&h->route_geo_dev, sizeof(RouteGeo)));
      if (h->route_geo_epoch != h->cfg_epoch) {
        RouteGeo g;
        GNXCHK(route_geo(h, &g));
        HIPCHK(hipMemcpyAsync(h->route_geo_dev, &g, sizeof(g), hipMemcpyHostToDevice, h->stream));
        HIPCHK(hipStreamSynchronize(h->stream));
        h->route_geo_epoch = h->cfg_epoch;
      }
      h->move_counts_routes = true;
    }
    const int rc_move = gnx_l_move(h, true, nullptr, nullptr, nullptr, nullptr, true);
    h->move_writes_keys = false;
    h->move_counts_routes = false;
    GNXCHK(rc_move);
  } else {
    GNXCHK(gnx_l_age(h));
  }
  const int64_t N = gnx_extent(h);
  *counts_dev = h->route_cnt;
  if (h->N == 0 || T == 1) return 0;
  RouteGeo g;
  GNXCHK(route_geo(h, &g));
  GnxSoA s = h->soa[h->cur];
  const int nt = h->cfg.n_traits;
  if (h->move_counted_routes) return 0;
  hipLaunchKernelGGL(k_route<false>, dim3(gnx_grid(N, 256)), dim3(256), 0, h->stream, N,
                     h->cfg.cap_inds, s, g, nt, h->route_cnt, (const int32_t*)nullptr,
                     (gnx_ind_rec*)nullptr, (float*)nullptr, (int64_t*)nullptr,
                     (gnx_ind_rec*)nullptr, (int64_t)0, (int64_t)0,
                     h->holes ? (const int32_t*)h->flag : (const int32_t*)nullptr);
  HIPCHK(hipGetLastError());
  return 0;
}

extern "C" int gnx_tile2_route_finish(gnx_state* h, const int64_t* counts) {
  const int T = n_tiles(h);
  const int64_t N = gnx_extent(h);
  if (h->N == 0 || T == 1) return 0;
  RouteGeo g;
  GNXCHK(route_geo(h, &g));
  GnxSoA s = h->soa[h->cur];
  const int nt = h->cfg.n_traits;
  int64_t n_mig = 0, n_gh = 0;
  for (int p = 0; p < T; ++p) {
    n_mig += counts[p];
    n_gh += counts[T + p];
  }
  if (counts[g.me] != 0) {
    gnx_set_error("tile2: %lld migrants routed to their own tile", (long long)counts[g.me]);
    return 1;
  }
  h->route_n_mig = n_mig;
  h->route_n_gh = n_gh;
  if (n_mig == 0 && n_gh == 0) return 0;
  if (n_mig > h->gp_cap) {
    (void)hipFree(h->gp_rec);
    (void)hipFree(h->gp_z);
    (void)hipFree(h->gp_slots);
    h->gp_cap = n_mig + n_mig / 4 + 1024;
    GNXCHK(dalloc_t(&h->gp_rec, (size_t)h->gp_cap));
    GNXCHK(dalloc_t(&h->gp_z, (size_t)h->gp_cap * std::max(nt, 1)));
    GNXCHK(dalloc_t(&h->gp_slots, (size_t)h->gp_cap));
  }
  if (n_gh > h->gh_cap) {
    (void)hipFree(h->gh_rec);
    h->gh_cap = n_gh + n_gh / 4 + 4096;
    GNXCHK(dalloc_t(&h->gh_rec, (size_t)h->gh_cap));
  }
  hipLaunchKernelGGL(k_route_offsets, dim3(1), dim3(64), 0, h->stream, T, h->route_cnt,
                     (int32_t*)nullptr, 0, 0, 1);
  hipLaunchKernelGGL(k_route<true>, dim3(gnx_grid(N, 256)), dim3(256), 0, h->stream, N,
                     h->cfg.cap_inds, s, g, nt, h->route_cnt,
                     (const int32_t*)(h->route_cnt + 2 * T), h->gp_rec, nt ? h->gp_z : nullptr,
                     h->gp_slots, h->gh_rec, h->gp_cap, h->gh_cap,
                     h->holes ? (const int32_t*)h->flag : (const int32_t*)nullptr);
  if (n_mig > 0 && has_rows(h)) {
    if (n_mig > h->st_geno_cap) {
      (void)hipFree(h->st_geno);
      h->st_geno_cap = n_mig + n_mig / 4 + 64;
      GNXCHK(dalloc_t(&h->st_geno, (size_t)h->st_geno_cap * 2 * h->W64));
    }
    GNXCHK(gnx_l_gather_genomes(h, n_mig, h->gp_slots, h->st_geno));
    h->st_has_geno = true;
  }
  HIPCHK(hipGetLastError());
  h->tile_evict = n_mig;
  const TileBox tb = tile_box(h);
  h->evict_box[0] = tb.x0;
  h->evict_box[1] = tb.x1;
  h->evict_box[2] = tb.y0;
// ... 299 lines not shown
__global__ void k_lookup_req2(int64_t n, const gnx_gamete_req2* __restrict__ req, int n_paths,
                              double inv_cs, int ncx, int ncy,
                              const int32_t* __restrict__ cell_start,
                              const int64_t* __restrict__ id, const uint8_t* __restrict__ ghost,
                              int32_t* __restrict__ out_slot, int64_t* __restrict__ chk) {
  int64_t q = (int64_t)blockIdx.x * blockDim.x + threadIdx.x;
  if (q >= n) return;
  const gnx_gamete_req2 r = req[q];
  const int cx = min(ncx - 1, max(0, (int)((double)r.px * inv_cs)));
  const int cy = min(ncy - 1, max(0, (int)((double)r.py * inv_cs)));
  const int c = cy * ncx + cx;
  int lo = cell_start[c], hi = cell_start[c + 1];
  const int end = hi;
  while (lo < hi) {
    const int mid = (lo + hi) >> 1;
    if (id[mid] < r.parent_id) lo = mid + 1; else hi = mid;
  }
  const bool ok = lo < end && id[lo] == r.parent_id && !ghost[lo] && r.key >= 0 &&
                  r.key < n_paths && (r.start == 0 || r.start == 1);
  out_slot[q] = ok ? lo : 0;
  if (!ok) atomicAdd((unsigned long long*)&chk[1], 1ull);
}

__global__ void __launch_bounds__(256)
k_make_gametes_req2(int64_t n, int W16, const u64x2* __restrict__ G,
                    const int32_t* __restrict__ grow, GnxHalves H,
                    const int32_t* __restrict__ slot, const gnx_gamete_req2* __restrict__ req,
                    const u64x2* __restrict__ paths, u64x2* __restrict__ out) {
  const int lane = threadIdx.x & 63;
  const int64_t q = ((int64_t)blockIdx.x * blockDim.x + threadIdx.x) >> 6;
  if (q >= n) return;
  const int prow = grow[slot[q]];
  const gnx_gamete_req2 r = req[q];
  const u64 s = r.start ? ~0ull : 0ull;
  const int64_t lh0 = (int64_t)max(prow, 0) * 2;
  const int key = min(max(r.key, 0), 0x7fffffff);
  const u64x2* pm = paths + (int64_t)key * W16;
  for (int c = lane; c < W16; c += 64) {
    u64x2 m = pm[c];
    m.a ^= s;
    m.b ^= s;
    const u64x2 a = G[gnx_chunk_at(H, lh0, c)], b = G[gnx_chunk_at(H, lh0 + 1, c)];
    u64x2 o;
    o.a = (a.a & ~m.a) | (b.a & m.a);
    o.b = (a.b & ~m.b) | (b.b & m.b);
    out[q * W16 + c] = o;
  }
}

extern "C" int gnx_tile2_serve(gnx_state* h, int64_t n, const void* req_dev, void** out_dev) {
  *out_dev = nullptr;
  if (n == 0) return 0;
  if (!has_rows(h) || h->n_paths == 0) {
    gnx_set_error("gnx_tile2_serve: genomes / paths not set");
    return 1;
  }
  GNXCHK(tile2_buffers(h));
  if (n > h->gam_cap) {
    (void)hipFree(h->gam_out);
    (void)hipFree(h->gam_slot);
    h->gam_cap = n + n / 4 + 256;
    GNXCHK(dalloc_t(&h->gam_out, (size_t)h->gam_cap * h->W64));
    GNXCHK(dalloc_t(&h->gam_slot, (size_t)h->gam_cap + 1));
  }
  GNXCHK(gnx_xo_launch_pending(h));
  GNXCHK(gnx_xo_wait_inflight(h));
  GnxSoA s = h->soa[h->cur];
  hipLaunchKernelGGL(k_lookup_req2, dim3(gnx_grid(n, 256)), dim3(256), 0, h->stream, n,
                     (const gnx_gamete_req2*)req_dev, h->n_paths, h->inv_cs, h->ncx, h->ncy,
                     h->cell_start, s.id, s.ghost, h->gam_slot, h->chk);
  const int W16 = h->W64 / 2;
  hipLaunchKernelGGL(k_make_gametes_req2, dim3(gnx_grid(n * 64, 256)), dim3(256), 0, h->stream, n,
                     W16, (const u64x2*)h->G, s.grow, gnx_halves(h), h->gam_slot,
                     (const gnx_gamete_req2*)req_dev, (const u64x2*)h->paths, (u64x2*)h->gam_out);
  HIPCHK(hipGetLastError());
  *out_dev = h->gam_out;
  return 0;
}

extern "C" int gnx_tile2_put(gnx_state* h, int64_t n, const void* data_dev) {
  if (n == 0) return 0;
  if (n != h->n_req) {
    gnx_set_error("gnx_tile2_put: %lld gametes for %lld requests", (long long)n,
                  (long long)h->n_req);
    return 1;
  }
  const int W16 = h->W64 / 2;
  hipLaunchKernelGGL(k_put_gametes, dim3(gnx_grid(n * W16, 256, 256 * 32)), dim3(256), 0, h->stream,
                     n, W16, (const u64x2*)data_dev, (u64x2*)h->G, h->soa[h->cur].grow,
                     gnx_halves(h), h->birth_first_slot, h->rq_k);
  HIPCHK(hipGetLastError());
  return 0;
}

extern "C" int gnx_tile2_finish_births(gnx_state* h, int32_t burn, void** reduce_dev,
                                       int64_t* n_words) {
  const int64_t nb = (int64_t)h->lat.nbx * h->lat.nby;
  GnxSetWords sw;
  sw.dst = h->bin_partials + 2 * nb;
  sw.v[0] = (int32_t)(h->N - h->n_ghost);
  sw.v[1] = (int32_t)h->last_births;
  sw.v[2] = (int32_t)h->prev_deaths;
  sw.v[3] = 0;
  GNXCHK(tile_finish_births(h, burn, &sw));
  *reduce_dev = h->bin_partials;
  *n_words = 2 * nb + 4;
  return 0;
}

extern "C" int gnx_tile2_die(gnx_state* h, int32_t burn, int32_t with_selection,
                             int32_t have_pairs, int64_t* totals) {
  GNXCHK(tile2_buffers(h));
  const int64_t nb = (int64_t)h->lat.nbx * h->lat.nby;
  GnxPubWords pub;
  pub.n1 = 4;
  pub.src1 = h->bin_partials + 2 * nb;
  pub.host1 = h->h_route_pin_dev;
  pub.n2 = 4;
  pub.src2 = (const int32_t*)h->chk;
  pub.host2 = h->h_route_pin_dev + 8;
  if (!gnx_l_lattices_tiled(h, have_pairs != 0, pub)) {
    hipLaunchKernelGGL(k_publish_words2, dim3(1), dim3(64), 0, h->stream, 4,
                       (const int32_t*)(h->bin_partials + 2 * nb), h->h_route_pin_dev, 4,
                       (const int32_t*)h->chk, h->h_route_pin_dev + 8);
    if (have_pairs)
      GNXCHK(gnx_l_spline(h, h->bins_P, &h->spl_P, nullptr));
    else
      h->spl_P.valid = false;
    GNXCHK(gnx_l_spline(h, h->bin_partials, &h->spl_N, nullptr));
  }
  GNXCHK(gnx_l_death_probs(h, with_selection != 0 && !burn));
  const int64_t N_before = h->N;
  int64_t D = 0;
  GNXCHK(gnx_l_mortality(h, nullptr, &D));
  h->last_deaths = D;
  h->prev_deaths = D;
  if (N_before == 0) HIPCHK(hipStreamSynchronize(h->stream));
  std::atomic_thread_fence(std::memory_order_acquire);
  for (int k = 0; k < 3; ++k) totals[k] = h->h_route_pin[k];
  const int64_t bad_rec = (int64_t)(uint32_t)h->h_route_pin[8] | ((int64_t)h->h_route_pin[9] << 32);
  const int64_t bad_req = (int64_t)(uint32_t)h->h_route_pin[10] | ((int64_t)h->h_route_pin[11] << 32);
  if (bad_rec || bad_req) {
    gnx_set_error("tile2: %lld imported records off the landscape, %lld gamete requests for a "
                  "parent that does not live on this tile (or a path / start out of range)",
                  (long long)bad_rec, (long long)bad_req);
    return 1;
  }
  return 0;
}

extern "C" int gnx_tile_pair_ptrs_nosync(gnx_state* h, int64_t* n_pairs, void** focal_ids,
                                         void** n_births) {
  const int64_t P = h->n_pairs;
  *n_pairs = P;
  *focal_ids = P ? (void*)h->key64[0] : nullptr;
  *n_births = (P && !h->sp.n_births_fixed) ? (void*)h->nbirths : nullptr;
  return 0;
}
```

Measured before the change: 2.540 billion.

## Pass mate-search candidate lists into pair flagging and compaction, skip unused pair keys

The mate-search kernel now writes each block's compacted list of eligible focal individuals and a per-block count. The pair-flag and pair-compact kernels read those lists so they only visit candidates, and the flag array carries the mate index so the compaction skips re-reading mate. Population and pair sort keys are written only when the tile protocol needs them, with checks added on tile entry points. This saves scattered memory traffic in pairing but ties the kernels to matching block sizes and adds an extra per-block count buffer.

```diff
diff --git a/geonomics_amd/_native.py b/geonomics_amd/_native.py
--- a/geonomics_amd/_native.py
+++ b/geonomics_amd/_native.py
@@ -429,7 +429,7 @@
 
     PATH_COUNTS = ('lazy_mortalities', 'xo_launch_p2', 'xo_flush', 'jobs_lanes_256',
                    'jobs_lanes_512', 'sort_hist_gather', 'gc_with_pending_xo', 'make_dense',
-                   'moves_ahead')
+                   'moves_ahead', 'pair_lists')
 
     def path_counts(self):
         out = np.zeros(len(self.PATH_COUNTS), np.int64)
diff --git a/geonomics_amd/csrc/gnx_api.hip b/geonomics_amd/csrc/gnx_api.hip
--- a/geonomics_amd/csrc/gnx_api.hip
+++ b/geonomics_amd/csrc/gnx_api.hip
@@ -431,6 +431,8 @@
   h->xo_launch_late = h->xo_launch_late_default = cap > gnx_dd_max_cap();
   h->compact_fill = gnx_env_int("GNX_COMPACT_FILL", 1) != 0;
   h->permute_split = gnx_env_int("GNX_PERMUTE_SPLIT", 1) != 0;
+  h->pair_lists = gnx_env_int("GNX_PAIR_LISTS", 1) != 0;
+  GNXCHK(dalloc(&h->kcnt, cap / 1024 + 1));
   *out = h;
   return 0;
 }
@@ -471,7 +473,7 @@
                   h->delet_loci, h->delet_s, h->cell_start, h->tag, h->cand, h->sort64_tmp, h->key64[0], h->key64[1], h->pairs2,
                   h->pair_goff, h->st_rec, h->st_z, h->st_geno, h->st_slots, h->req_pid, h->req_k, h->req_key, h->req_start, h->req_px, h->req_py,
                   h->req_count, h->sort_tmp, h->scan_tmp, h->mate,
-                  h->flag, h->flag2, h->scan, h->pairs, h->nbirths, h->boff, h->off_pair,
+                  h->flag, h->flag2, h->kcnt, h->scan, h->pairs, h->nbirths, h->boff, h->off_pair,
                   h->off_parent, h->off_keys, h->off_start, h->keep_in, h->inj_a, h->inj_b,
                   h->mid_x, h->mid_y, h->p_death, h->d_cell, h->dead_in, h->nmax_bits, h->red,
                   h->sel_loci, h->path_sel, h->lat.areas, h->lat.cprime, h->spl_N.c, h->spl_P.c, h->bin_partials, h->nodes,
diff --git a/geonomics_amd/csrc/gnx_internal.h b/geonomics_amd/csrc/gnx_internal.h
--- a/geonomics_amd/csrc/gnx_internal.h
+++ b/geonomics_amd/csrc/gnx_internal.h
@@ -237,6 +237,7 @@
   GNX_PC_GC_PENDING_XO,
   GNX_PC_MAKE_DENSE,
   GNX_PC_MOVE_AHEAD,
+  GNX_PC_PAIR_LISTS,
   GNX_PC_COUNT
 };
 
@@ -436,6 +437,7 @@
   int32_t* mate = nullptr;
   int32_t* flag = nullptr;
   int32_t* flag2 = nullptr;
+  int32_t* kcnt = nullptr;
   int32_t* scan = nullptr;
   int32_t* pairs = nullptr;
   int32_t* nbirths = nullptr;
@@ -486,6 +488,8 @@
   bool compact_fill = true;
   bool jobs_self_scan = false;
   bool ord_covers_xo = false;
+  bool pair_keys = false, pairs_keyed = false;
+  bool pair_lists = true;
   bool permute_split = true;
   bool perm_rest_inflight = false;
   bool perm_rest_pending = false;
diff --git a/geonomics_amd/csrc/gnx_kernels_pop.hip b/geonomics_amd/csrc/gnx_kernels_pop.hip
--- a/geonomics_amd/csrc/gnx_kernels_pop.hip
+++ b/geonomics_amd/csrc/gnx_kernels_pop.hip
@@ -608,7 +608,7 @@
     r = gnx_rec_load(a, j, cap, n_layers, n_traits, tbw);
     gnx_rec_store(b, i, cap, n_layers, n_traits, tbw, r);
   }
-  if (cellk) key[i] = ((uint64_t)ck << idbits) | (uint64_t)r.id;
+  if (cellk && key) key[i] = ((uint64_t)ck << idbits) | (uint64_t)r.id;
   const uint32_t tg = gnx_ind_tag(pair_seed, (unsigned long long)r.id);
   cand[i] = make_uint4(__float_as_uint(r.x), __float_as_uint(r.y), tg, (uint32_t)r.id);
   if (!hot_only) gnx_rec_rest(a, j, b, i, cap, n_layers, n_traits, tbw);
@@ -836,8 +836,8 @@
   hipLaunchKernelGGL(k_permute, dim3(gnx_grid(N, 256)), dim3(256), 0, h->stream, N, c.cap_inds,
                      ordm ? h->valk[1] : h->perm[1], a, b, c.n_layers, c.n_traits,
                      a.tb ? 2 * h->TW : 0, gnx_pair_seed(c.seed, h->step), h->tag, (uint4*)h->cand,
-                     h->key64[1], idbits, h->cell_start, h->ncx * h->ncy,
-                     ordm ? h->keyk[1] : nullptr, h->ord[h->ord_cur], h->ord_n,
+                     (ordm && !h->pair_keys) ? (uint64_t*)nullptr : h->key64[1], idbits, h->cell_start,
+                     h->ncx * h->ncy, ordm ? h->keyk[1] : nullptr, h->ord[h->ord_cur], h->ord_n,
                      h->ord[h->ord_cur ^ 1], h->perm[1], (uint4*)h->os_scratch, (wipe_words + 3) / 4,
                      split ? 1 : 0, (const GnxDD*)nullptr, GnxBinP{nullptr, 0.0, 0, 0},
                      h->id_order == 1 ? h->vt_count : (int32_t*)nullptr);
@@ -895,6 +895,7 @@
 #define FM_LANES 4
 #define FM_MIN_BLOCKS 8
 #define FM_MAX_BLOCKS 2048
+static_assert(FM_PER_BLOCK == GNX_CB, "the pair list reads the mate search's lists block by block");
 
 struct FocalP {
   int64_t N;
@@ -952,7 +953,8 @@
 __global__ void __launch_bounds__(256)
 k_find_mates(FocalP fp, GnxSoA s, const uint4* __restrict__ cand, double inv_cs,
              const int32_t* __restrict__ cell_start, int ncx, int ncy, int ref, float r, float r2,
-             int easy_rounds, int32_t* __restrict__ mate) {
+             int easy_rounds, int32_t* __restrict__ mate, int32_t* __restrict__ klist,
+             int32_t* __restrict__ kcnt) {
   __shared__ int32_t list[FM_PER_BLOCK];
   __shared__ int32_t hard[FM_PER_BLOCK];
   __shared__ int32_t wcnt[FM_PER_BLOCK / 256][4];
@@ -961,7 +963,10 @@
   const int64_t base = (int64_t)blockIdx.x * FM_PER_BLOCK;
   fp.N = gnx_dd_n(fp.dd, fp.N);
   fp.step = gnx_dd_step(fp.dd, fp.step);
-  if (base >= fp.N) return;
+  if (base >= fp.N) {
+    if (kcnt && tid == 0) kcnt[blockIdx.x] = 0;
+    return;
+  }
   constexpr int ROUNDS = FM_PER_BLOCK / 256;
   bool okr[ROUNDS];
   unsigned long long balr[ROUNDS];
@@ -991,11 +996,14 @@
   for (int round = 0; round < ROUNDS; ++round) {
     int off = n_list;
     for (int w = 0; w < wave; ++w) off += wcnt[round][w];
-    if (okr[round])
-      list[off + __popcll(balr[round] & ((1ull << lane) - 1ull))] =
-          (int32_t)(base + round * 256 + tid);
+    if (okr[round]) {
+      const int pos = off + __popcll(balr[round] & ((1ull << lane) - 1ull));
+      list[pos] = (int32_t)(base + round * 256 + tid);
+      if (klist) klist[base + pos] = (int32_t)(base + round * 256 + tid);
+    }
     n_list += wcnt[round][0] + wcnt[round][1] + wcnt[round][2] + wcnt[round][3];
   }
+  if (kcnt && tid == 0) kcnt[blockIdx.x] = n_list;
   __syncthreads();
   if (MODE != GNX_MATE_NEAREST) {
     constexpr bool WT = MODE == GNX_MATE_INVERSE;
@@ -1486,8 +1494,10 @@
   return ok && (s.age[fo] >= P.ra_f) && (s.age[m] >= P.ra_m);
 }
 
+template <bool LISTED>
 __global__ void __launch_bounds__(256)
-k_pair_flags(PairP P, GnxSoA s, int32_t* flag2, int32_t* cnt, GnxVtOut vt) {
+k_pair_flags(PairP P, GnxSoA s, const int32_t* __restrict__ klist, const int32_t* __restrict__ kcnt,
+             int32_t* flag2, int32_t* cnt, GnxVtOut vt) {
   __shared__ int lds[16];
   __shared__ int vtot[GNX_VTN];
   if (vt.scls && threadIdx.x < GNX_VTN) vtot[threadIdx.x] = 0;
@@ -1496,29 +1506,81 @@
   P.step = gnx_dd_step(P.dd, P.step);
   bool f[4];
   float px[4] = {0.f, 0.f, 0.f, 0.f}, py[4] = {0.f, 0.f, 0.f, 0.f};
-  if (vt.scls) {
+  if (LISTED) {
+    const int tid = threadIdx.x, wbase = tid & ~63;
+    int li[4] = {base + tid < P.N ? klist[base + tid] : -1, -1, -1, -1};
+    const int n_l = base < P.N ? kcnt[blockIdx.x] : 0;
+    if (tid >= n_l) li[0] = -1;
+#pragma unroll
+    for (int r = 1; r < 4; ++r)
+      if (r * 256 + wbase < n_l) {
+        const int t = r * 256 + tid;
+        li[r] = t < n_l ? klist[base + t] : -1;
+      }
+    int m4[4] = {-1, -1, -1, -1}, agei[4], mm[4], agem[4];
+    int64_t idi[4], idm[4];
+    uint8_t sexi[4], gh[4], sexm[4];
+#pragma unroll
+    for (int r = 0; r < 4; ++r)
+      if (r * 256 + wbase < n_l) {
+        const int i = max(li[r], 0);
+        m4[r] = li[r] >= 0 ? P.mate[i] : -1;
+        idi[r] = s.id[i];
+        agei[r] = s.age[i];
+        sexi[r] = s.sex[i];
+        gh[r] = s.ghost[i];
+        if (vt.scls) {
+          px[r] = s.x[i];
+          py[r] = s.y[i];
+        }
+      }
+#pragma unroll
+    for (int r = 0; r < 4; ++r)
+      if (r * 256 + wbase < n_l) {
+        const int m = max(m4[r], 0);
+        agem[r] = s.age[m];
+        sexm[r] = s.sex[m];
+        mm[r] = P.mate[m];
+        idm[r] = s.id[m];
+      }
+#pragma unroll
+    for (int r = 0; r < 4; ++r) {
+      f[r] = false;
+      if (r * 256 + wbase < n_l) {
+        bool ok = m4[r] >= 0 && (!P.sexed || sexm[r] == 1) && agem[r] >= P.ra_m;
+        if (ok && P.dedup && mm[r] == li[r] && idm[r] < idi[r] &&
+            (!P.sexed || sexi[r] == 1) && agei[r] >= P.ra_m)
+          ok = false;
+        if (gh[r]) ok = false;
+        f[r] = ok;
+        if (li[r] >= 0) flag2[base + r * 256 + tid] = ok ? m4[r] : -1;
+      }
+    }
+  } else {
+    if (vt.scls) {
+#pragma unroll
+      for (int r = 0; r < 4; ++r) {
+        const int64_t i = base + r * 256 + threadIdx.x;
+        if (i < P.N) {
+          px[r] = s.x[i];
+          py[r] = s.y[i];
+        }
+      }
+    }
 #pragma unroll
     for (int r = 0; r < 4; ++r) {
       const int64_t i = base + r * 256 + threadIdx.x;
+      f[r] = false;
       if (i < P.N) {
-        px[r] = s.x[i];
-        py[r] = s.y[i];
-      }
-    }
-  }
-#pragma unroll
-  for (int r = 0; r < 4; ++r) {
-    const int64_t i = base + r * 256 + threadIdx.x;
-    f[r] = false;
-    if (i < P.N) {
-      bool ok = pair_ok(P, s, i);
-      if (ok && P.dedup) {
-        const int m = P.mate[i];
-        if (P.mate[m] == (int32_t)i && s.id[m] < s.id[i] && pair_ok(P, s, m)) ok = false;
-      }
-      if (s.ghost[P.focal ? P.focal[i] : (int)i]) ok = false;
-      f[r] = ok;
-      flag2[i] = ok ? 1 : 0;
+        bool ok = pair_ok(P, s, i);
+        if (ok && P.dedup) {
+          const int m = P.mate[i];
+          if (P.mate[m] == (int32_t)i && s.id[m] < s.id[i] && pair_ok(P, s, m)) ok = false;
+        }
+        if (s.ghost[P.focal ? P.focal[i] : (int)i]) ok = false;
+        f[r] = ok;
+        flag2[i] = ok ? 1 : 0;
+      }
     }
   }
   int rank[4], tot;
@@ -1553,8 +1615,10 @@
   }
 }
 
+template <bool LISTED>
 __global__ void __launch_bounds__(256)
 k_pair_compact(int64_t N, const int32_t* focal, const int32_t* mate, const int32_t* flag2,
+               const int32_t* __restrict__ klist, const int32_t* __restrict__ kcnt,
                const int32_t* blk_off, const float* x, const float* y, const uint64_t* popkey,
                int idbits, int32_t* pairs, float* mid_x, float* mid_y, uint64_t* key,
                const int32_t* __restrict__ cnt, int32_t* __restrict__ total_dev,
@@ -1565,6 +1629,8 @@
   __shared__ int vcnt[16][GNX_VTN];
   __shared__ int vpre[GNX_VTN];
   if (dd) N = dd->N;
+  const int64_t base = (int64_t)blockIdx.x * GNX_CB;
+  const int n_l = LISTED && base < N ? kcnt[blockIdx.x] : 0;
   if (vt.cls) {
     for (int k = threadIdx.x; k < 16 * GNX_VTN; k += 256) (&vcnt[0][0])[k] = 0;
     const int lane = threadIdx.x & 63, wave = threadIdx.x >> 6;
@@ -1624,26 +1690,42 @@
       }
     }
   }
-  const int64_t base = (int64_t)blockIdx.x * GNX_CB;
   bool f[4];
   int sc[4] = {0, 0, 0, 0};
+  int fo4[4] = {0, 0, 0, 0}, m4[4] = {0, 0, 0, 0};
 #pragma unroll
   for (int r = 0; r < 4; ++r) {
-    const int64_t i = base + r * 256 + threadIdx.x;
-    f[r] = i < N && flag2[i] != 0;
-    if (vt.cls && i < N) sc[r] = vt.scls[i];
+    const int t = r * 256 + threadIdx.x;
+    const int64_t i = base + t;
+    if (LISTED) {
+      f[r] = false;
+      if (t < n_l) {
+        fo4[r] = klist[i];
+        m4[r] = flag2[i];
+        if (vt.cls) sc[r] = vt.scls[i];
+        f[r] = m4[r] >= 0;
+      }
+    } else {
+      f[r] = i < N && flag2[i] != 0;
+      if (vt.cls && i < N) sc[r] = vt.scls[i];
+    }
   }
   int rank[4], tot;
   gnx_block_ranks(f, rank, tot, lds);
   int vc[4] = {0, 0, 0, 0}, vrw[4] = {0, 0, 0, 0};
-  float fx[4], fy[4];
-  int fo4[4];
+  float fx[4], fy[4], gx[4] = {0.f, 0.f, 0.f, 0.f}, gy[4] = {0.f, 0.f, 0.f, 0.f};
+  uint64_t pk[4] = {0, 0, 0, 0};
 #pragma unroll
   for (int r = 0; r < 4; ++r) {
     const int64_t i = base + r * 256 + threadIdx.x;
-    fo4[r] = f[r] ? (focal ? focal[i] : (int)i) : 0;
+    if (!LISTED) fo4[r] = f[r] ? (focal ? focal[i] : (int)i) : 0;
     fx[r] = f[r] ? x[fo4[r]] : 0.f;
     fy[r] = f[r] ? y[fo4[r]] : 0.f;
+    if (LISTED && f[r]) {
+      gx[r] = x[m4[r]];
+      gy[r] = y[m4[r]];
+      if (key) pk[r] = popkey[fo4[r]];
+    }
   }
   if (vt.cls) {
     const int lane = threadIdx.x & 63, wave = threadIdx.x >> 6;
@@ -1661,15 +1743,18 @@
     int bin = 0;
     if (f[r]) {
       const int p = bo + rank[r];
-      const int m = mate[i];
+      const int m = LISTED ? m4[r] : mate[i];
       const int fo = fo4[r];
       pairs[2 * p] = fo;
       pairs[2 * p + 1] = m;
-      const float mx = (fx[r] + x[m]) / 2.0f, my = (fy[r] + y[m]) / 2.0f;
+      const float mx = (fx[r] + (LISTED ? gx[r] : x[m])) / 2.0f;
+      const float my = (fy[r] + (LISTED ? gy[r] : y[m])) / 2.0f;
       mid_x[p] = mx;
       mid_y[p] = my;
-      const uint64_t k = popkey[i];
-      key[p] = ((k >> idbits) << 40) | (k & ((1ull << idbits) - 1ull));
+      if (key) {
+        const uint64_t k = LISTED ? pk[r] : popkey[i];
+        key[p] = ((k >> idbits) << 40) | (k & ((1ull << idbits) - 1ull));
+      }
       if (bins.bins) bin = gnx_bin_of(bins, mx, my);
       if (vt.cls) {
         const int wave = threadIdx.x >> 6;
@@ -1709,11 +1794,14 @@
   int64_t N = h->N;
   h->n_pairs = 0;
   h->pairs_wait = false;
+  h->pairs_keyed = h->pair_keys;
   if (N == 0) return 0;
   const gnx_species_params& sp = h->sp;
   GnxSoA s = h->soa[h->cur];
   int sexed = sp.sexed;
   const int32_t* focal = nullptr;
+  const bool lists = h->pair_lists && sp.mating_radius >= 0;
+  if (lists) ++h->pc[GNX_PC_PAIR_LISTS];
   gnx_time_begin(h);
   if (sp.mating_radius < 0) {
     focal = h->off_pair;
@@ -1724,16 +1812,17 @@
     float r2 = r * r;
     FocalP fp{N, d_keep, (float)sp.b, sexed, sp.repro_age[0], h->step, h->cfg.seed};
     dim3 grid(gnx_grid(N, FM_PER_BLOCK)), blk(256);
+    int32_t *kl = lists ? h->off_pair : nullptr, *kc = lists ? h->kcnt : nullptr;
     const uint4* cd = (const uint4*)h->cand;
     if (sp.mate_mode == GNX_MATE_NEAREST)
       hipLaunchKernelGGL(k_find_mates<GNX_MATE_NEAREST>, grid, blk, 0, h->stream, fp, s, cd,
-                         h->inv_cs, h->cell_start, h->ncx, h->ncy, h->cell_ref, r, r2, GNX_FM_EASY_ROUNDS, h->mate);
+                         h->inv_cs, h->cell_start, h->ncx, h->ncy, h->cell_ref, r, r2, GNX_FM_EASY_ROUNDS, h->mate, kl, kc);
     else if (sp.mate_mode == GNX_MATE_INVERSE)
       hipLaunchKernelGGL(k_find_mates<GNX_MATE_INVERSE>, grid, blk, 0, h->stream, fp, s, cd,
-                         h->inv_cs, h->cell_start, h->ncx, h->ncy, h->cell_ref, r, r2, GNX_FM_EASY_ROUNDS, h->mate);
+                         h->inv_cs, h->cell_start, h->ncx, h->ncy, h->cell_ref, r, r2, GNX_FM_EASY_ROUNDS, h->mate, kl, kc);
     else
       hipLaunchKernelGGL(k_find_mates<GNX_MATE_UNIFORM>, grid, blk, 0, h->stream, fp, s, cd,
-                         h->inv_cs, h->cell_start, h->ncx, h->ncy, h->cell_ref, r, r2, GNX_FM_EASY_ROUNDS, h->mate);
+                         h->inv_cs, h->cell_start, h->ncx, h->ncy, h->cell_ref, r, r2, GNX_FM_EASY_ROUNDS, h->mate, kl, kc);
   }
   gnx_time_end(h, GNX_K_FIND_MATES, (double)N * 16.0);
   GNXCHK(gnx_permute_rest_launch(h));
@@ -1744,12 +1833,18 @@
            h->step, h->cfg.seed};
   GnxVtOut vto;
   GNXCHK(gnx_vt_out(h, &vto));
-  hipLaunchKernelGGL(k_pair_flags, dim3(nb), dim3(256), 0, h->stream, pp, s, h->flag2, h->blk_cnt, vto);
+  if (lists)
+    hipLaunchKernelGGL(k_pair_flags<true>, dim3(nb), dim3(256), 0, h->stream, pp, s,
+                       (const int32_t*)h->off_pair, (const int32_t*)h->kcnt, h->flag2, h->blk_cnt, vto);
+  else
+    hipLaunchKernelGGL(k_pair_flags<false>, dim3(nb), dim3(256), 0, h->stream, pp, s,
+                       (const int32_t*)nullptr, (const int32_t*)nullptr, h->flag2, h->blk_cnt, vto);
   const int64_t seq = ++h->pin_seq;
   const bool with_top = h->half_top && h->genomes_assigned;
-  hipLaunchKernelGGL(k_pair_compact, dim3(nb), dim3(256), 0, h->stream, N, focal, h->mate,
-                     h->flag2, h->blk_off, s.x, s.y, h->key64[1], gnx_id_bits(h), h->pairs,
-                     h->mid_x, h->mid_y, h->key64[0],
+  hipLaunchKernelGGL(lists ? k_pair_compact<true> : k_pair_compact<false>, dim3(nb), dim3(256), 0,
+                     h->stream, N, focal, h->mate, h->flag2, (const int32_t*)h->off_pair,
+                     (const int32_t*)h->kcnt, h->blk_off, s.x, s.y, h->key64[1], gnx_id_bits(h), h->pairs,
+                     h->mid_x, h->mid_y, h->pair_keys ? h->key64[0] : (uint64_t*)nullptr,
                      (const int32_t*)h->blk_cnt, h->cnt_dev,
                      h->h_pin_dev + 4, (long long)seq,
                      with_top ? (const int32_t*)h->half_top : (const int32_t*)nullptr,
@@ -2204,7 +2299,8 @@
   const int64_t wipe_words = (int64_t)gnx_os_words_used((size_t)n_fixed, h->key_bits);
   hipLaunchKernelGGL(k_permute, dim3(gnx_grid(n_fixed, 256)), dim3(256), 0, st, n_fixed, c.cap_inds,
                      h->valk[1], a, b, c.n_layers, c.n_traits, a.tb ? 2 * h->TW : 0,
-                     (unsigned long long)c.seed, h->tag, (uint4*)h->cand, h->key64[1], 40,
+                     (unsigned long long)c.seed, h->tag, (uint4*)h->cand,
+                     h->pair_keys ? h->key64[1] : (uint64_t*)nullptr, 40,
                      h->cell_start, h->ncx * h->ncy, h->keyk[1], h->ord[h->ord_cur], (int64_t)0,
                      h->ord[h->ord_cur ^ 1], h->perm[1], (uint4*)h->os_scratch, (wipe_words + 3) / 4,
                      0, (const GnxDD*)h->dd,
@@ -2224,25 +2320,33 @@
   FocalP fp{cap, nullptr, (float)sp.b, sp.sexed, sp.repro_age[0], 0, h->cfg.seed, h->dd};
   dim3 grid(gnx_grid(cap, FM_PER_BLOCK)), blk(256);
   const uint4* cd = (const uint4*)h->cand;
+  const bool lists = h->pair_lists;
+  int32_t *kl = lists ? h->off_pair : nullptr, *kc = lists ? h->kcnt : nullptr;
   if (sp.mate_mode == GNX_MATE_NEAREST)
     hipLaunchKernelGGL(k_find_mates<GNX_MATE_NEAREST>, grid, blk, 0, st, fp, s, cd, h->inv_cs,
-                       h->cell_start, h->ncx, h->ncy, h->cell_ref, r, r2, GNX_FM_EASY_ROUNDS, h->mate);
+                       h->cell_start, h->ncx, h->ncy, h->cell_ref, r, r2, GNX_FM_EASY_ROUNDS, h->mate, kl, kc);
   else if (sp.mate_mode == GNX_MATE_INVERSE)
     hipLaunchKernelGGL(k_find_mates<GNX_MATE_INVERSE>, grid, blk, 0, st, fp, s, cd, h->inv_cs,
-                       h->cell_start, h->ncx, h->ncy, h->cell_ref, r, r2, GNX_FM_EASY_ROUNDS, h->mate);
+                       h->cell_start, h->ncx, h->ncy, h->cell_ref, r, r2, GNX_FM_EASY_ROUNDS, h->mate, kl, kc);
   else
     hipLaunchKernelGGL(k_find_mates<GNX_MATE_UNIFORM>, grid, blk, 0, st, fp, s, cd, h->inv_cs,
-                       h->cell_start, h->ncx, h->ncy, h->cell_ref, r, r2, GNX_FM_EASY_ROUNDS, h->mate);
+                       h->cell_start, h->ncx, h->ncy, h->cell_ref, r, r2, GNX_FM_EASY_ROUNDS, h->mate, kl, kc);
   const int nb = (int)((cap + GNX_CB - 1) / GNX_CB);
   PairP pp{cap, nullptr, h->mate, nullptr, (float)sp.b, sp.sexed, sp.repro_age[0], sp.repro_age[1],
            sp.sexed ? 0 : 1, 0, h->cfg.seed, h->dd};
   GnxVtOut vto;
   GNXCHK(gnx_vt_out(h, &vto));
-  hipLaunchKernelGGL(k_pair_flags, dim3(nb), dim3(256), 0, st, pp, s, h->flag2, h->blk_cnt, vto);
-  hipLaunchKernelGGL(k_pair_compact, dim3(nb), dim3(256), 0, st, cap, (const int32_t*)nullptr,
-                     h->mate, h->flag2, h->blk_off, s.x, s.y, h->key64[1], 40, h->pairs, h->mid_x,
-                     h->mid_y, h->key64[0], (const int32_t*)h->blk_cnt, h->cnt_dev,
-                     (int64_t*)nullptr, 0ll, (const int32_t*)nullptr, h->dd,
+  if (lists)
+    hipLaunchKernelGGL(k_pair_flags<true>, dim3(nb), dim3(256), 0, st, pp, s, (const int32_t*)kl,
+                       (const int32_t*)kc, h->flag2, h->blk_cnt, vto);
+  else
+    hipLaunchKernelGGL(k_pair_flags<false>, dim3(nb), dim3(256), 0, st, pp, s, (const int32_t*)nullptr,
+                       (const int32_t*)nullptr, h->flag2, h->blk_cnt, vto);
+  hipLaunchKernelGGL(lists ? k_pair_compact<true> : k_pair_compact<false>, dim3(nb), dim3(256), 0, st,
+                     cap, (const int32_t*)nullptr, h->mate, h->flag2, (const int32_t*)kl,
+                     (const int32_t*)kc, h->blk_off, s.x, s.y, h->key64[1], 40, h->pairs, h->mid_x,
+                     h->mid_y, h->pair_keys ? h->key64[0] : (uint64_t*)nullptr,
+                     (const int32_t*)h->blk_cnt, h->cnt_dev, (int64_t*)nullptr, 0ll, (const int32_t*)nullptr, h->dd,
                      (int)sp.n_births_lambda, (int64_t)cap,
                      GnxBinP{d_bins, 1.0 / h->lat.hww, h->lat.nbx, h->lat.nby}, vto);
   if (vto.cls) {
diff --git a/geonomics_amd/csrc/gnx_tile.hip b/geonomics_amd/csrc/gnx_tile.hip
--- a/geonomics_amd/csrc/gnx_tile.hip
+++ b/geonomics_amd/csrc/gnx_tile.hip
@@ -36,6 +36,7 @@
   h->tile_r = r;
   h->tile_c = c;
   h->tiled = R * C > 1;
+  h->pair_keys = true;
   return 0;
 }
 
@@ -301,12 +302,19 @@
   return import_common(h, n, rec, nullptr, nullptr, 1);
 }
 
+static int pairs_keyed(const gnx_state* h) {
+  if (h->pairs_keyed) return 0;
+  gnx_set_error("the pair list was made without its order keys (no tile protocol on this handle yet)");
+  return 1;
+}
+
 extern "C" int gnx_tile_pairs(gnx_state* h, int32_t burn, int64_t* n_pairs, int64_t* n_births) {
   if (!h->have_sp) {
     gnx_set_error("species parameters not set");
     return 1;
   }
   int64_t P = 0, B = 0;
+  h->pair_keys = true;
   GNXCHK(gnx_l_sort_by_cell(h));
   GNXCHK(gnx_l_find_pairs(h, nullptr, &P));
   GNXCHK(gnx_l_bins(h, P, h->mid_x, h->mid_y, nullptr, h->bins_P));
@@ -319,6 +327,7 @@
 extern "C" int gnx_tile_pair_info(gnx_state* h, int64_t* focal_ids, int32_t* n_births) {
   int64_t P = h->n_pairs;
   if (P == 0) return 0;
+  GNXCHK(pairs_keyed(h));
   GNXCHK(gnx_d2h(h, focal_ids, h->key64[0], P * sizeof(int64_t)));
   if (h->sp.n_births_fixed)
     for (int64_t p = 0; p < P; ++p) n_births[p] = (int32_t)h->sp.n_births_lambda;
@@ -879,6 +888,7 @@
   *focal_ids = nullptr;
   *n_births = nullptr;
   if (P == 0) return 0;
+  GNXCHK(pairs_keyed(h));
   HIPCHK(hipStreamSynchronize(h->stream));
   *focal_ids = h->key64[0];
   if (!h->sp.n_births_fixed) *n_births = h->nbirths;
@@ -1205,6 +1215,7 @@
 #define GNX_REQ_CNT(h) ((h)->route_cnt + 4 * n_tiles(h) + 8)
 static int tile2_buffers(gnx_state* h) {
   h->tile2_mode = true;
+  h->pair_keys = true;
   if (!h->route_cnt) {
     GNXCHK(dalloc_t(&h->route_cnt, (size_t)5 * GNX_MAX_TILES + 8));
     HIPCHK(hipMemset(h->route_cnt, 0, ((size_t)5 * GNX_MAX_TILES + 8) * sizeof(int32_t)));
@@ -1810,6 +1821,7 @@
 extern "C" int gnx_tile_pair_ptrs_nosync(gnx_state* h, int64_t* n_pairs, void** focal_ids,
                                          void** n_births) {
   const int64_t P = h->n_pairs;
+  if (P) GNXCHK(pairs_keyed(h));
   *n_pairs = P;
   *focal_ids = P ? (void*)h->key64[0] : nullptr;
   *n_births = (P && !h->sp.n_births_fixed) ? (void*)h->nbirths : nullptr;
```

Result: faster. 2.585 billion, median of 6 (+1.8%).
